# 10258392511/InverseProblemWithDiffusionModel

Measured on AMD Instinct MI355X. Metric: ALD reconstructions/sec (128x128 complex, R=40, 4-coil), higher is better.
Workload: dtype f32 (convolutions: operands as two fp16 pieces = 22 significand bits + 2 signs, three fp16 MFMAs per product, fp32 accumulate; every image scaled into fp16's range by an exact power of two from its producer's per-image maxima: any fp32 input, DESIGN.md 4.2); 1 GPU; ACDC-style 128x128 complex SENSE R=40 4-coil ALD reconstruction, NCSNv2Deepest ngf=128 (94.1M params, seeded random init), sigma 348->0.01 x 2311 levels x 3 steps, L2Penalty, denoise; 14 posterior samples = 14 on rank 0 + 13 per further rank (the 105-sample / 8-GPU partition of BASELINE config 3); samples_total=14, samples_this_rank=14, parallelism=sample-sharded x1, hip_graph=True, state_finite=True

## Files before the change

include/ipdm.h:

```cpp
#ifndef IPDM_H
#define IPDM_H

#include <stddef.h>
#include <stdint.h>

#ifdef __cplusplus
extern "C" {
#endif

#define IPDM_OK 0
#define IPDM_EINVAL (-1)
#define IPDM_EUNSUPPORTED (-2)

#define IPDM_ACT_NONE 0
#define IPDM_ACT_ELU 1
#define IPDM_ACT_RELU 2
#define IPDM_ACT_LRELU02 3
#define IPDM_ACT_SWISH 4
#define IPDM_ACT_COPY 5

#define IPDM_AMAX_WAYS 8
#define IPDM_AMAX_SLOT 128

#define IPDM_ABI_VERSION 4
// ... 106 lines not shown
                                   int32_t* iters_out, int B, int n_coils, int H, int W, void* stream);

int ipdm_sense_forward_sets_c64(const float* x, const float* sens, int sens_complex, int sens_sets, const uint8_t* mask,
                                int mask_t, float* y, int B, int n_coils, int H, int W, void* stream);
int ipdm_sense_adjoint_sets_c64(const float* s, const float* sens, int sens_complex, int sens_sets, const uint8_t* mask,
                                int mask_t, int apply_mask, float* x, float* workspace, int B, int n_coils, int H, int W,
                                void* stream);
int ipdm_sense_l2prox_sets_f32(const float* z_re, const float* z_im, const float* y, const float* sens, int sens_complex,
                               int sens_sets, const uint8_t* mask, int mask_t, float coef, float* out_re, float* out_im,
                               float* work, int B, int n_coils, int H, int W, void* stream);
int ipdm_ald_sense_step_sets_f32(float* x_re, float* x_im, const float* g_re, const float* g_im,
                                 const float* noise_re, const float* noise_im,
                                 float step, float noise_scale, uint64_t seed, int64_t sample_offset, int64_t step_id,
                                 const ipdm_sched_t* dev_sched, const float* y, const float* sens, int sens_complex,
                                 int sens_sets, const uint8_t* mask, int mask_t, float coef, float* work, int B, int n_coils,
                                 int H, int W, void* stream);
int ipdm_sense_cgprox_sets_f32(const float* z_re, const float* z_im, const float* y, const float* sens, int sens_complex,
                               int sens_sets, const uint8_t* mask, int mask_t, float a, const float* ahy, int max_iter,
                               float tol, float* out_re, float* out_im, float* work, int32_t* iters_out, int B, int n_coils,
                               int H, int W, void* stream);
int ipdm_ald_sense_cg_step_sets_f32(float* x_re, float* x_im, const float* g_re, const float* g_im,
                                    const float* noise_re, const float* noise_im,
                                    float step, float noise_scale, uint64_t seed, int64_t sample_offset, int64_t step_id,
                                    const ipdm_sched_t* dev_sched, const float* y, const float* sens, int sens_complex,
                                    int sens_sets, const uint8_t* mask, int mask_t, float coef, float* work,
                                    const float* ahy, int max_iter, float tol, int32_t* iters_out, int B, int n_coils,
                                    int H, int W, void* stream);

size_t ipdm_csm_workspace_bytes(int B, int n_coils, int H, int W);
int ipdm_csm_supported(int n_coils, int radius, int H, int W);
int ipdm_csm_calib_images_c64(const float* y, int ah, int aw, float* calib, int B, int n_coils, int H, int W, void* stream);
int ipdm_csm_walsh_c64(const float* y, int ah, int aw, int radius, int power_iters, float thresh,
                       float* maps , float* rss ,
                       float* rss_max , float* work , int B,
                       int n_coils, int H, int W, void* stream);

int ipdm_coilcomp_supported(int n_coils, int n_virtual);
size_t ipdm_coilcomp_workspace_bytes(int B, int n_coils);
int ipdm_coil_gram_c64(const float* y, int ah, int aw, float* gram, int B, int n_coils, int H, int W, void* stream);
int ipdm_coilcomp_matrix_c64(const float* gram, const float* noise_cov, int n_virtual, float* A, float* eig, int32_t* status,
                             int B, int n_coils, void* stream);
int ipdm_coil_apply_c64(const float* y, const float* A, int per_image, float* out, int B, int n_coils, int n_virtual,
                        int64_t P, void* stream);
int ipdm_coil_compress_c64(const float* y, int ah, int aw, int n_virtual, const float* noise_cov, float* A, float* eig,
                           int32_t* status, float* out, float* work, int B, int n_coils, int H, int W, void* stream);

int ipdm_gcc_supported(int n_coils, int n_virtual, int H, int W, int win);
size_t ipdm_gcc_workspace_bytes(int B, int n_coils, int n_virtual, int H, int W);
int ipdm_readout_fft_c64(const float* in, float* out, int inverse, int64_t planes, int H, int W, void* stream);
int ipdm_gcc_gram_c64(const float* h, int aw, int win, float* gram, int B, int n_coils, int H, int W, void* stream);
int ipdm_gcc_align_c64(const float* Ahat, const float* noise_cov, float* A, int32_t* status, int32_t* work, int B, int H,
                       int n_coils, int n_virtual, void* stream);
int ipdm_coil_apply_rows_c64(const float* y, const float* A, int per_image, float* out, int B, int n_coils, int n_virtual, int H,
                             int W, void* stream);
int ipdm_gcc_compress_c64(const float* y, int aw, int win, int n_virtual, const float* noise_cov, float* A, float* eig,
                          int32_t* status, float* out, float* work, int B, int n_coils, int H, int W, void* stream);

int ipdm_espirit_supported(int n_coils, int ksize, int H, int W);
size_t ipdm_espirit_workspace_bytes(int B, int n_coils, int ksize);
int ipdm_espirit_gram_c64(const float* y, int ah, int aw, int ksize, double* gram, int B, int n_coils, int H, int W, void* stream);
int ipdm_espirit_kernels_c64(const float* y, int ah, int aw, int ksize, double sv_thresh, float* K, double* lam, int32_t* rank,
                             int32_t* status, int32_t* sweeps, double* work, int B, int n_coils, int H, int W, void* stream);
int ipdm_espirit_pixel_c64(const float* K, const int32_t* status, int ksize, float crop, int power_iters, float* maps,
                           float* eigval, int B, int n_coils, int H, int W, void* stream);
int ipdm_espirit_c64(const float* y, int ah, int aw, int ksize, double sv_thresh, float crop, int power_iters, float* maps,
                     float* eigval, float* K, double* lam, int32_t* rank, int32_t* status, double* work, int B, int n_coils,
                     int H, int W, void* stream);

int ipdm_kspace_tavg_c64(const float* y, const uint8_t* mask, int mask_t, float* ybar, int32_t* count, int B, int T,
                         int n_coils, int H, int W, void* stream);

int ipdm_singlecoil_prox_f32(const float* z_re, const float* z_im, const float* y, const uint8_t* mask, int mask_t,
                             float coef, int mode, float* out_re, float* out_im,
                             float* workspace ,
                             int B, int H, int W, void* stream);

int ipdm_ald_singlecoil_step_f32(float* x_re, float* x_im, const float* g_re, const float* g_im,
                                 const float* noise_re, const float* noise_im,
                                 float step, float noise_scale, uint64_t seed, int64_t sample_offset, int64_t step_id,
                                 const ipdm_sched_t* dev_sched, const float* y, const uint8_t* mask, int mask_t,
                                 float coef, int mode, float* workspace , int B, int H,
                                 int W, void* stream);

int64_t ipdm_pc_langevin_coef_workspace_bytes(int B);
int ipdm_pc_langevin_coef_f32(const float* g_re, const float* g_im, const float* noise_re, const float* noise_im,
                              double snr, double alpha, uint64_t seed, int64_t sample_offset, int64_t step_id,
                              const ipdm_sched_t* dev_sched, float coef, float sigma, ipdm_sched_t* sample_sched,
                              double* work, int B, int64_t sample_elems, void* stream);
int ipdm_pc_sense_step_f32(float* x_re, float* x_im, const float* g_re, const float* g_im,
                           const float* noise_re, const float* noise_im,
                           float step, float noise_scale, uint64_t seed, int64_t sample_offset, int64_t step_id,
                           const ipdm_sched_t* dev_sched, int sched_stride, const float* y, const float* sens,
                           int sens_complex, int sens_sets, const uint8_t* mask, int mask_t, float coef, float* work, int B,
                           int n_coils, int H, int W, void* stream);
int ipdm_pc_sense_cg_step_f32(float* x_re, float* x_im, const float* g_re, const float* g_im,
                              const float* noise_re, const float* noise_im,
                              float step, float noise_scale, uint64_t seed, int64_t sample_offset, int64_t step_id,
                              const ipdm_sched_t* dev_sched, int sched_stride, const float* y, const float* sens,
                              int sens_complex, int sens_sets, const uint8_t* mask, int mask_t, float coef, float* work,
                              const float* ahy, int max_iter, float tol, int32_t* iters_out, int B, int n_coils, int H,
                              int W, void* stream);
int ipdm_pc_singlecoil_step_f32(float* x_re, float* x_im, const float* g_re, const float* g_im,
                                const float* noise_re, const float* noise_im,
                                float step, float noise_scale, uint64_t seed, int64_t sample_offset, int64_t step_id,
                                const ipdm_sched_t* dev_sched, int sched_stride, const float* y, const uint8_t* mask,
                                int mask_t, float coef, int mode, float* workspace, int B, int H, int W, void* stream);

int ipdm_nc_supported(int H, int W);
int64_t ipdm_ndft_workspace_bytes(int M, int H, int W);
int ipdm_ndft_forward_c64(const float* x, const float* sens, const double* traj, float* y,
                          float* work , int B, int n_coils, int M, int H, int W, void* stream);
int ipdm_ndft_adjoint_c64(const float* y, const float* sens, const double* traj, const float* weights, float* x,
                          float* work , int B, int n_coils, int M, int H, int W, void* stream);
int64_t ipdm_toeplitz_psf_workspace_bytes(int M, int H, int W);
int ipdm_toeplitz_psf_f32(const double* traj, const float* weights, float* psf,
                          float* work , int M, int H, int W, void* stream);
int64_t ipdm_toeplitz_workspace_bytes(int B, int n_coils, int H, int W);
int ipdm_toeplitz_normal_c64(const float* v, const float* sens, const float* psf, float* out,
                             float* work , int B, int n_coils, int H, int W, void* stream);
int64_t ipdm_nc_sense_cg_workspace_bytes(int B, int n_coils, int H, int W);
int ipdm_nc_sense_cgprox_f32(const float* z_re, const float* z_im, const float* sens, const float* psf, float a,
                             const float* ahy, int max_iter, float tol, float* out_re, float* out_im, float* work,
                             int32_t* iters_out, int B, int n_coils, int H, int W, void* stream);
int ipdm_ald_nc_sense_cg_step_f32(float* x_re, float* x_im, const float* g_re, const float* g_im,
                                  const float* noise_re, const float* noise_im,
                                  float step, float noise_scale, uint64_t seed, int64_t sample_offset, int64_t step_id,
                                  const ipdm_sched_t* dev_sched, int sched_stride, const float* sens, const float* psf,
                                  float coef, float* work, const float* ahy, int max_iter, float tol, int32_t* iters_out,
                                  int B, int n_coils, int H, int W, void* stream);
int ipdm_ndft_forward_sets_c64(const float* x, const float* sens, const double* traj, int traj_sets, float* y, float* work,
                               int B, int n_coils, int M, int H, int W, void* stream);
int ipdm_ndft_adjoint_sets_c64(const float* y, const float* sens, const double* traj, int traj_sets, const float* weights,
                               float* x, float* work, int B, int n_coils, int M, int H, int W, void* stream);
int ipdm_toeplitz_psf_sets_f32(const double* traj, int traj_sets, const float* weights, float* psf, float* work, int M, int H,
                               int W, void* stream);
int ipdm_toeplitz_normal_sets_c64(const float* v, const float* sens, const float* psf, int psf_sets, float* out, float* work,
                                  int B, int n_coils, int H, int W, void* stream);
int ipdm_nc_sense_cgprox_sets_f32(const float* z_re, const float* z_im, const float* sens, const float* psf, int psf_sets,
                                  float a, const float* ahy, int max_iter, float tol, float* out_re, float* out_im,
                                  float* work, int32_t* iters_out, int B, int n_coils, int H, int W, void* stream);
int ipdm_ald_nc_sense_cg_step_sets_f32(float* x_re, float* x_im, const float* g_re, const float* g_im,
                                       const float* noise_re, const float* noise_im,
                                       float step, float noise_scale, uint64_t seed, int64_t sample_offset, int64_t step_id,
                                       const ipdm_sched_t* dev_sched, int sched_stride, const float* sens, const float* psf,
                                       int psf_sets, float coef, float* work, const float* ahy, int max_iter, float tol,
                                       int32_t* iters_out, int B, int n_coils, int H, int W, void* stream);

size_t ipdm_nc_coil_gram_workspace_bytes(int B, int n_coils, int M);
int ipdm_nc_coil_gram_c64(const float* y, const float* weights, float* gram, float* work, int B, int n_coils, int M, void* stream);

int ipdm_langevin_step_f32(float* x, const float* g, const float* noise, float step, float noise_scale,
                           uint64_t seed, int64_t sample_offset, int64_t step_id, const ipdm_sched_t* dev_sched,
                           int64_t n_samples, int64_t sample_elems, void* stream);

int ipdm_philox_normal_f32(float* out, uint64_t seed, int64_t sample_offset, int64_t step_id, int plane,
                           int64_t n_samples, int64_t sample_elems, void* stream);

int ipdm_philox_block_host(uint64_t seed, int64_t sample, int64_t step_id, int plane, uint32_t quad, uint32_t* out4);


int ipdm_instnorm_plus_coef_f32(const float* x, const float* alpha, const float* gamma, const float* beta,
                                float* coef, int B, int C, int HW,
                                float* amax_bound ,
                                void* stream);
int ipdm_cond_instnorm_plus_coef_f32(const float* x, const float* embed, const int64_t* labels, int num_classes, int bias,
                                     float* coef, int B, int C, int HW, float* amax_bound, void* stream);
int ipdm_affine_act_f32(const float* x, const float* coef, float* y, int B, int C, int HW, int act, void* stream);
int ipdm_act_f32(const float* x, float* y, int64_t n, int act, void* stream);
int ipdm_scale_shift_f32(const float* x, float* y, int64_t n, float a, float b, void* stream);
int ipdm_add_f32(const float* x, const float* y, float* out, int64_t n, void* stream);
int ipdm_div_sigma_f32(const float* x, const float* sigmas, const int64_t* labels, float* out,
                       int B, int64_t sample_elems, void* stream);
int ipdm_conv3x3_thin_supported(int Cin, int Cout, int H, int W);
int ipdm_conv3x3_thin_f32(const float* x, const float* w, const float* bias,
                          const float* coef ,
                          float* out, int B, int Cin, int Cout, int H, int W, void* stream);
int ipdm_conv3x3_thin_stats_partials(int Cin, int Cout, int H, int W);
int ipdm_conv3x3_thin_stats_f32(const float* x, const float* w, const float* bias, const float* coef, float* out, float* part,
                                int B, int Cin, int Cout, int H, int W, void* stream);
int ipdm_conv3x3_fewout_fin_supported(int Cin, int Cout, int H, int W);
int ipdm_conv3x3_fewout_fin_f32(const float* x, const float* w, const float* bias, const float* coef, int act, float* out,
                                int B, int Cin, int Cout, int H, int W, void* stream);
int ipdm_maxpool5_f32(const float* x, float* y, int planes, int H, int W, void* stream);
int ipdm_affine_avgpool5_f32(const float* x, const float* coef, float* y, int planes, int H, int W, void* stream);
int ipdm_meanpool2_f32(const float* x, float* y, int planes, int H, int W, void* stream);
int ipdm_bilinear_f32(const float* x, float* out, int planes, int in_h, int in_w, int out_h, int out_w,
                      int accumulate, int act ,
                      int planes_per_image, float* amax_out ,
                      void* stream);
int ipdm_trilinear_f32(const float* x, float* out, int planes, int in_d, int in_h, int in_w, int out_d, int out_h,
                       int out_w, int accumulate, int act, int planes_per_image, float* amax_out, void* stream);

int ipdm_groupnorm_coef_f32(const float* x, const float* weight, const float* bias, float* coef,
                            int B, int C, int HW, int G, float eps,
                            float* plane_amax ,
                            void* stream);
int ipdm_groupnorm_coef_partials_f32(const float* part1, int C1, const float* part2, int C2, int P, const float* weight,
                                     const float* bias, float* coef , int B, int G, float eps, void* stream);
int ipdm_groupnorm_coef_cat_f32(const float* x1, int C1, const float* x2, int C2, const float* weight, const float* bias,
                                float* coef, int B, int HW, int G, float eps, float* plane_amax ,
                                void* stream);
int ipdm_affine_act_cat_f32(const float* x1, int C1, const float* x2, int C2, const float* coef, float* y, int B, int HW,
                            int act, void* stream);
int ipdm_linear_f32(const float* x, const float* W, const float* bias, float* y, int B, int In, int Out,
                    int act, void* stream);
int ipdm_attention_f32(const float* q, const float* k, const float* v, float* out, int B, int C, int N,
                       float scale, void* stream);
int ipdm_axpby_f32(const float* x, const float* y, float* out, int64_t n, float a, float b, void* stream);
int ipdm_sample_axpy2_f32(const float* x, const float* y, const float* z, const float* a, const float* c,
                          float* out, int n_samples, int64_t sample_elems, void* stream);
int ipdm_sample_norm_f32(const float* x, float* norms, int n_samples, int64_t sample_elems, void* stream);

int ipdm_conv_pack_weight_f32(const float* w , float* wt, int Cout, int Cin, int k, void* stream);
int ipdm_conv2d_f32(const float* x, const float* wt, const float* bias, const float* coef, int act,
                    const float* residual, float* out, float* out_act, int act_out,
                    int B, int Cin, int Cout, int H, int W, int k, int dilation, int pool2, void* stream);

int ipdm_conv_wino_weight_f32(const float* w , float* U, int Cout, int Cin, void* stream);
int ipdm_conv2d_wino_supported(int Cin, int Cout, int H, int W, int dilation);
int ipdm_conv2d_wino_f32(const float* x, const float* U, const float* bias, const float* residual, float* out,
                         float* out_act, int act_out, int B, int Cin, int Cout, int H, int W, int dilation,
                         void* stream);

int ipdm_debug_set_stamp_buffer(void* buf);
int64_t ipdm_debug_lds_optin_count(void);

int ipdm_conv3d_f32(const float* x, const float* wt, const float* bias, const float* coef, int act,
                    const float* residual, float* out, float* out_act, int act_out,
                    int B, int Cin, int Cout, int D, int H, int W, int k, int dilation, void* stream);

int ipdm_maxpool3d5_f32(const float* x, float* y, int planes, int D, int H, int W, void* stream);
int ipdm_temporal_taps_f32(const float* x, float* out, int planes, int S, int T_in, int T_out, int mode, void* stream);

typedef struct {
  const float* in_amax;
  int bias_bstride;
  float out_scale;
  int res_second;
  float* out_amax;
  float* act_amax;
} ipdm_conv_ext_t;

int64_t ipdm_conv_bx3_weight_bytes(int Cout, int Cin, int k);
int ipdm_conv_bx3_pack_weight(const float* w , void* packed, int Cout,
                              int Cin, int k, void* stream);
int ipdm_conv2d_bx3_f32(const float* x, const void* packed, const float* bias, const float* coef, int act,
                        const float* residual, float* out, float* out_act, int act_out,
                        int B, int Cin, int Cout, int H, int W, int k, int dilation, const ipdm_conv_ext_t* ext, void* stream);
int ipdm_conv3d_bx3_f32(const float* x, const void* packed, const float* bias, const float* coef, int act,
                        const float* residual, float* out, float* out_act, int act_out,
                        int B, int Cin, int Cout, int D, int H, int W, int k, int dilation, const ipdm_conv_ext_t* ext, void* stream);

int ipdm_conv_bx3_splitk(int B, int D, int Cin, int Cout, int H, int W, int k, int dilation);
int ipdm_conv_bx3_splitk_f32(const float* x, const void* packed, const float* bias, const float* coef, int act,
                             const float* residual, float* out, float* out_act, int act_out,
                             int B, int Cin, int Cout, int D, int H, int W, int k, int dilation, int volume, int ksplit,
                             float* work, const ipdm_conv_ext_t* ext, void* stream);

int ipdm_adam_ascent_f32(float* x, const float* g, float* m, float* v, int64_t n, float lr, float beta1, float beta2,
                         float eps, int step, void* stream);

int64_t ipdm_conv_wino_bx3_weight_bytes(int Cout, int Cin);
int ipdm_conv_wino_bx3_pack_weight(const float* w , void* U, int Cout, int Cin, void* stream);
int ipdm_conv2d_wino_bx3_supported(int Cin, int Cout, int H, int W, int dilation);
int ipdm_conv2d_wino_bx3_f32(const float* x, const void* U, const float* bias, const float* residual, float* out,
                             float* out_act, int act_out, int B, int Cin, int Cout, int H, int W, int dilation,
                             int pool2, const ipdm_conv_ext_t* ext, void* stream);
int ipdm_conv2d_wino_bx3_splitk(int Cin, int Cout, int H, int W, int dilation);
int ipdm_conv2d_wino_bx3_splitk_f32(const float* x, const void* U, const float* bias, const float* residual, float* out,
                                    float* out_act, int act_out, int B, int Cin, int Cout, int H, int W, int dilation,
                                    int ksplit, float* work, const ipdm_conv_ext_t* ext, void* stream);
int ipdm_conv2d_wino_bx3_stats_partials(int Cin, int Cout, int H, int W, int dilation, int pool2);
int ipdm_conv2d_wino_bx3_stats_f32(const float* x, const void* U, const float* bias, const float* residual, float* out,
                                   float* out_act, int act_out, int B, int Cin, int Cout, int H, int W, int dilation,
                                   int pool2, float* stats, const ipdm_conv_ext_t* ext, void* stream);
int ipdm_absmax_f32(const float* x, float* amax , int n_images,
                    int64_t per_image, void* stream);
int64_t ipdm_conv_hx2_weight_bytes(int Cout, int Cin, int k);
int ipdm_conv_hx2_pack_weight(const float* w , void* packed, int Cout,
                              int Cin, int k, void* stream);
int ipdm_conv2d_hx2_f32(const float* x, const void* packed, const float* bias, const float* coef, int act,
                        const float* residual, float* out, float* out_act, int act_out,
                        int B, int Cin, int Cout, int H, int W, int k, int dilation, const ipdm_conv_ext_t* ext, void* stream);
int ipdm_conv3d_hx2_f32(const float* x, const void* packed, const float* bias, const float* coef, int act,
                        const float* residual, float* out, float* out_act, int act_out,
                        int B, int Cin, int Cout, int D, int H, int W, int k, int dilation, const ipdm_conv_ext_t* ext, void* stream);
int ipdm_conv_hx2_splitk_f32(const float* x, const void* packed, const float* bias, const float* coef, int act,
                             const float* residual, float* out, float* out_act, int act_out,
                             int B, int Cin, int Cout, int D, int H, int W, int k, int dilation, int volume, int ksplit,
                             float* work, const ipdm_conv_ext_t* ext, void* stream);
int64_t ipdm_conv_wino_hx2_weight_bytes(int Cout, int Cin);
int ipdm_conv_wino_hx2_pack_weight(const float* w , void* U, int Cout, int Cin, void* stream);
int ipdm_conv2d_wino_hx2_f32(const float* x, const void* U, const float* bias, const float* residual, float* out,
                             float* out_act, int act_out, int B, int Cin, int Cout, int H, int W, int dilation,
                             int pool2, const ipdm_conv_ext_t* ext, void* stream);
#define IPDM_WINO_FORM_OTHER 0
#define IPDM_WINO_FORM_CO32 1
#define IPDM_WINO_FORM_HALF 2
#define IPDM_WINO_FORM_POLY 3
int ipdm_conv2d_wino_hx2_form(int Cin, int Cout, int H, int W, int dilation);
int64_t ipdm_conv_wino1d_weight_bytes(int Cout, int Cin);
int ipdm_conv_wino1d_pack_weight(const float* w , void* U, int Cout, int Cin, void* stream);
int ipdm_conv2d_wino1d_supported(int Cin, int Cout, int H, int W);
int64_t ipdm_conv_wino1d_weight_bytes3d(int Cout, int Cin);
int ipdm_conv_wino1d_pack_weight3d(const float* w, void* U, int Cout, int Cin, void* stream);
int ipdm_conv3d_wino1d_supported(int Cin, int Cout, int D, int H, int W);
int ipdm_conv3d_wino1d_f32(const float* x, const void* U, const float* bias, const float* residual, float* out,
                           float* out_act, int act_out, int B, int Cin, int Cout, int D, int H, int W,
                           const ipdm_conv_ext_t* ext, void* stream);
int ipdm_conv2d_wino1d_f32(const float* x, const void* U, const float* bias, const float* coef, int act,
                           const float* residual, float* out, float* out_act, int act_out, int B, int Cin, int Cout, int H,
                           int W, int pool2, const ipdm_conv_ext_t* ext, void* stream);
int ipdm_conv2d_wino1d_stats_partials(int Cin, int Cout, int H, int W);
int ipdm_conv2d_wino1d_stats_f32(const float* x, const void* U, const float* bias, const float* coef, int act,
                                 const float* residual, float* out, float* out_act, int act_out, int B, int Cin, int Cout,
                                 int H, int W, int pool2, float* stats, const ipdm_conv_ext_t* ext, void* stream);
int ipdm_conv2d_wino_hx2_splitk_f32(const float* x, const void* U, const float* bias, const float* residual, float* out,
                                    float* out_act, int act_out, int B, int Cin, int Cout, int H, int W, int dilation,
                                    int ksplit, float* work, const ipdm_conv_ext_t* ext, void* stream);
int ipdm_conv2d_wino_hx2_stats_f32(const float* x, const void* U, const float* bias, const float* residual, float* out,
                                   float* out_act, int act_out, int B, int Cin, int Cout, int H, int W, int dilation,
                                   int pool2, float* stats, const ipdm_conv_ext_t* ext, void* stream);
int ipdm_instnorm_plus_coef_partials_f32(const float* partials, int P, const float* alpha, const float* gamma,
                                         const float* beta , float* coef , int B, int C,
                                         int HW , float* amax_bound ,
                                         void* stream);

int ipdm_cond_instnorm_plus_coef_partials_f32(const float* partials, int P, const float* embed, const int64_t* labels,
                                              int num_classes, int bias, float* coef, int B, int C, int HW, float* amax_bound,
                                              void* stream);

int ipdm_conv1d_hx2_supported(int Cin, int Cout, int L, int k, int dilation);
int64_t ipdm_conv1d_hx2_weight_bytes(int Cout, int Cin, int k);
int ipdm_conv1d_hx2_pack_weight(const float* w , void* packed, int Cout, int Cin, int k, void* stream);
int ipdm_conv1d_hx2_f32(const float* x, const void* packed, const float* bias, const float* residual, float* out,
                        float* out_act, int act_out, int N, int Cin, int Cout, int L, int k, int dilation, int pool2,
                        const ipdm_conv_ext_t* ext, void* stream);
int ipdm_meanpool1d2_f32(const float* x, float* y, int rows, int L, void* stream);
int ipdm_scale_shift_amax_f32(const float* x, float* y, float* amax_out, int n_images, int64_t per_image, float a, float b,
                              void* stream);


int ipdm_zero_insert2_f32(const float* x, float* out, int planes, int H, int W, void* stream);
int ipdm_subsample2_f32(const float* x, float* out, int planes, int H, int W, int oy, int ox, int Ho, int Wo, void* stream);
int ipdm_in_prelu_fwd_f32(const float* x, const float* slope, float* xhat, float* y, float* rstd, int planes, int HW,
                          float eps, void* stream);
int ipdm_in_prelu_bwd_f32(const float* gy, const float* xhat, const float* rstd, const float* slope, float* gx, int planes,
                          int HW, void* stream);
int ipdm_in_prelu_bwd_eps_f32(const float* gy, const float* xhat, const float* rstd, const float* slope, float* gx, int planes,
                              int HW, float eps, void* stream);
int ipdm_seg_loglh_grad_f32(const float* logits, const int64_t* label, float* g, int B, int C, int64_t HW, void* stream);
int ipdm_axpy_sched_f32(float* y, const float* x, const int64_t* mask, int64_t mask_period, const ipdm_sched_t* dev_sched,
                        float scale, int64_t n, void* stream);


int ipdm_magnitude_c64(const float* x , float* out, int64_t n, void* stream);
int ipdm_posterior_moments_c64(const float* samples, double* planes, int n_samples, int64_t HW, void* stream);
int ipdm_nrmse_f32(const float* img, const float* ref, double* out, int n_images, int64_t elems, int ref_broadcast,
                   void* stream);
int ipdm_ssim_f32(const float* img, const float* ref, double* out, int n_images, int H, int W, int ref_broadcast,
                  double data_range, void* stream);

int ipdm_tv_c64(const float* x, double* out, int n_images, int H, int W, void* stream);
int ipdm_tv_grad_c64(const float* x, float* g, int n_images, int H, int W, void* stream);

#ifdef __cplusplus
}
#endif
#endif
```

inverseproblemwithdiffusionmodel_amd/_lib.py:

```python
import ctypes
import os

import torch
from ctypes import c_char_p, c_double, c_float, c_int, c_int64, c_uint64, c_void_p


class ConvExt(ctypes.Structure):
    _fields_ = [("in_amax", c_void_p), ("bias_bstride", c_int), ("out_scale", c_float), ("res_second", c_int),
                ("out_amax", c_void_p), ("act_amax", c_void_p)]


_HERE = os.path.dirname(os.path.abspath(__file__))
LIB_PATH = os.environ.get("IPDM_LIB") or os.path.join(_HERE, "libipdm.so")

P = c_void_p

SIGNATURES = {
    "ipdm_abi_version": [],
    "ipdm_build_arch": [],
    "ipdm_upfirdn2d_f32": [P, P, P] + [c_int] * 14 + [P],
    "ipdm_fused_bias_act_f32": [P, P, P, P, c_int64, c_int, c_int, c_int, c_int, c_float, c_float, P],
    "ipdm_upfirdn2d_f16": [P, P, P] + [c_int] * 14 + [P],
    "ipdm_upfirdn2d_f64": [P, P, P] + [c_int] * 14 + [P],
    "ipdm_fused_bias_act_f16": [P, P, P, P, c_int64, c_int, c_int, c_int, c_int, c_float, c_float, P],
    "ipdm_fused_bias_act_f64": [P, P, P, P, c_int64, c_int, c_int, c_int, c_int, c_float, c_float, P],
    "ipdm_fft2c_c64": [P, P, c_int, c_int, c_int, c_int, P, P],
    "ipdm_fft2c_workspace_bytes": [c_int, c_int, c_int],
    "ipdm_mask_layouts": [],
    "ipdm_kspace_size_class": [c_int, c_int],
    "ipdm_sense_forward_c64": [P, P, P, c_int, P, c_int, c_int, c_int, c_int, P],
    "ipdm_sense_workspace_bytes": [c_int, c_int, c_int, c_int],
    "ipdm_sense_adjoint_c64": [P, P, P, c_int, c_int, P, P, c_int, c_int, c_int, c_int, P],
    "ipdm_sense_ssos_c64": [P, P, P, c_int, c_int, c_int, c_int, P],
    "ipdm_sense_l2prox_f32": [P, P, P, P, P, c_int, c_float, P, P, P, c_int, c_int, c_int, c_int, P],
    "ipdm_ald_sense_step_f32": [P, P, P, P, P, P, c_float, c_float, c_uint64, c_int64, c_int64, P,
                                P, P, P, c_int, c_float, P, c_int, c_int, c_int, c_int, P],
    "ipdm_sense_forward_csm_c64": [P, P, P, c_int, P, c_int, c_int, c_int, c_int, P],
    "ipdm_sense_adjoint_csm_c64": [P, P, P, c_int, c_int, P, P, c_int, c_int, c_int, c_int, P],
    "ipdm_sense_l2prox_csm_f32": [P, P, P, P, P, c_int, c_float, P, P, P, c_int, c_int, c_int, c_int, P],
    "ipdm_ald_sense_step_csm_f32": [P, P, P, P, P, P, c_float, c_float, c_uint64, c_int64, c_int64, P,
                                    P, P, P, c_int, c_float, P, c_int, c_int, c_int, c_int, P],
    "ipdm_sense_cg_workspace_bytes": [c_int, c_int, c_int, c_int],
    "ipdm_sense_cgprox_f32": [P, P, P, P, P, c_int, c_float, P, c_int, c_float, P, P, P, P, c_int, c_int, c_int, c_int, P],
    "ipdm_sense_cgprox_csm_f32": [P, P, P, P, P, c_int, c_float, P, c_int, c_float, P, P, P, P, c_int, c_int, c_int, c_int, P],
    "ipdm_ald_sense_cg_step_f32": [P, P, P, P, P, P, c_float, c_float, c_uint64, c_int64, c_int64, P,
                                   P, P, P, c_int, c_float, P, P, c_int, c_float, P, c_int, c_int, c_int, c_int, P],
    "ipdm_ald_sense_cg_step_csm_f32": [P, P, P, P, P, P, c_float, c_float, c_uint64, c_int64, c_int64, P,
                                       P, P, P, c_int, c_float, P, P, c_int, c_float, P, c_int, c_int, c_int, c_int, P],
    "ipdm_sense_forward_sets_c64": [P, P, c_int, c_int, P, c_int, P, c_int, c_int, c_int, c_int, P],
    "ipdm_sense_adjoint_sets_c64": [P, P, c_int, c_int, P, c_int, c_int, P, P, c_int, c_int, c_int, c_int, P],
    "ipdm_sense_l2prox_sets_f32": [P, P, P, P, c_int, c_int, P, c_int, c_float, P, P, P, c_int, c_int, c_int, c_int, P],
    "ipdm_ald_sense_step_sets_f32": [P, P, P, P, P, P, c_float, c_float, c_uint64, c_int64, c_int64, P,
                                     P, P, c_int, c_int, P, c_int, c_float, P, c_int, c_int, c_int, c_int, P],
    "ipdm_sense_cgprox_sets_f32": [P, P, P, P, c_int, c_int, P, c_int, c_float, P, c_int, c_float, P, P, P, P,
                                   c_int, c_int, c_int, c_int, P],
    "ipdm_ald_sense_cg_step_sets_f32": [P, P, P, P, P, P, c_float, c_float, c_uint64, c_int64, c_int64, P,
                                        P, P, c_int, c_int, P, c_int, c_float, P, P, c_int, c_float, P,
                                        c_int, c_int, c_int, c_int, P],
    "ipdm_csm_workspace_bytes": [c_int, c_int, c_int, c_int],
    "ipdm_csm_supported": [c_int, c_int, c_int, c_int],
    "ipdm_csm_calib_images_c64": [P, c_int, c_int, P, c_int, c_int, c_int, c_int, P],
    "ipdm_csm_walsh_c64": [P, c_int, c_int, c_int, c_int, c_float, P, P, P, P, c_int, c_int, c_int, c_int, P],
    "ipdm_coilcomp_supported": [c_int, c_int],
    "ipdm_coilcomp_workspace_bytes": [c_int, c_int],
    "ipdm_coil_gram_c64": [P, c_int, c_int, P, c_int, c_int, c_int, c_int, P],
    "ipdm_coilcomp_matrix_c64": [P, P, c_int, P, P, P, c_int, c_int, P],
    "ipdm_coil_apply_c64": [P, P, c_int, P, c_int, c_int, c_int, c_int64, P],
    "ipdm_coil_compress_c64": [P, c_int, c_int, c_int, P, P, P, P, P, P, c_int, c_int, c_int, c_int, P],
    "ipdm_gcc_supported": [c_int, c_int, c_int, c_int, c_int],
    "ipdm_gcc_workspace_bytes": [c_int, c_int, c_int, c_int, c_int],
    "ipdm_readout_fft_c64": [P, P, c_int, c_int64, c_int, c_int, P],
    "ipdm_gcc_gram_c64": [P, c_int, c_int, P, c_int, c_int, c_int, c_int, P],
    "ipdm_gcc_align_c64": [P, P, P, P, P, c_int, c_int, c_int, c_int, P],
    "ipdm_coil_apply_rows_c64": [P, P, c_int, P, c_int, c_int, c_int, c_int, c_int, P],
    "ipdm_gcc_compress_c64": [P, c_int, c_int, c_int, P, P, P, P, P, P, c_int, c_int, c_int, c_int, P],
    "ipdm_espirit_supported": [c_int, c_int, c_int, c_int],
    "ipdm_espirit_workspace_bytes": [c_int, c_int, c_int],
    "ipdm_espirit_gram_c64": [P, c_int, c_int, c_int, P, c_int, c_int, c_int, c_int, P],
    "ipdm_espirit_kernels_c64": [P, c_int, c_int, c_int, c_double, P, P, P, P, P, P, c_int, c_int, c_int, c_int, P],
    "ipdm_espirit_pixel_c64": [P, P, c_int, c_float, c_int, P, P, c_int, c_int, c_int, c_int, P],
    "ipdm_espirit_c64": [P, c_int, c_int, c_int, c_double, c_float, c_int, P, P, P, P, P, P, P, c_int, c_int, c_int, c_int, P],
    "ipdm_kspace_tavg_c64": [P, P, c_int, P, P, c_int, c_int, c_int, c_int, c_int, P],
    "ipdm_singlecoil_prox_f32": [P, P, P, P, c_int, c_float, c_int, P, P, P, c_int, c_int, c_int, P],
    "ipdm_ald_singlecoil_step_f32": [P, P, P, P, P, P, c_float, c_float, c_uint64, c_int64, c_int64, P,
                                     P, P, c_int, c_float, c_int, P, c_int, c_int, c_int, P],
    "ipdm_pc_langevin_coef_workspace_bytes": [c_int],
    "ipdm_pc_langevin_coef_f32": [P, P, P, P, c_double, c_double, c_uint64, c_int64, c_int64, P, c_float, c_float, P, P,
                                  c_int, c_int64, P],
    "ipdm_pc_sense_step_f32": [P, P, P, P, P, P, c_float, c_float, c_uint64, c_int64, c_int64, P, c_int,
                               P, P, c_int, c_int, P, c_int, c_float, P, c_int, c_int, c_int, c_int, P],
    "ipdm_pc_sense_cg_step_f32": [P, P, P, P, P, P, c_float, c_float, c_uint64, c_int64, c_int64, P, c_int,
                                  P, P, c_int, c_int, P, c_int, c_float, P, P, c_int, c_float, P,
                                  c_int, c_int, c_int, c_int, P],
    "ipdm_pc_singlecoil_step_f32": [P, P, P, P, P, P, c_float, c_float, c_uint64, c_int64, c_int64, P, c_int,
                                    P, P, c_int, c_float, c_int, P, c_int, c_int, c_int, P],
    "ipdm_nc_supported": [c_int, c_int],
    "ipdm_ndft_workspace_bytes": [c_int, c_int, c_int],
    "ipdm_ndft_forward_c64": [P, P, P, P, P, c_int, c_int, c_int, c_int, c_int, P],
    "ipdm_ndft_adjoint_c64": [P, P, P, P, P, P, c_int, c_int, c_int, c_int, c_int, P],
    "ipdm_toeplitz_psf_workspace_bytes": [c_int, c_int, c_int],
    "ipdm_toeplitz_psf_f32": [P, P, P, P, c_int, c_int, c_int, P],
    "ipdm_toeplitz_workspace_bytes": [c_int, c_int, c_int, c_int],
    "ipdm_toeplitz_normal_c64": [P, P, P, P, P, c_int, c_int, c_int, c_int, P],
    "ipdm_nc_sense_cg_workspace_bytes": [c_int, c_int, c_int, c_int],
    "ipdm_nc_sense_cgprox_f32": [P, P, P, P, c_float, P, c_int, c_float, P, P, P, P, c_int, c_int, c_int, c_int, P],
    "ipdm_ald_nc_sense_cg_step_f32": [P, P, P, P, P, P, c_float, c_float, c_uint64, c_int64, c_int64, P, c_int,
                                      P, P, c_float, P, P, c_int, c_float, P, c_int, c_int, c_int, c_int, P],
    "ipdm_ndft_forward_sets_c64": [P, P, P, c_int, P, P, c_int, c_int, c_int, c_int, c_int, P],
    "ipdm_ndft_adjoint_sets_c64": [P, P, P, c_int, P, P, P, c_int, c_int, c_int, c_int, c_int, P],
    "ipdm_toeplitz_psf_sets_f32": [P, c_int, P, P, P, c_int, c_int, c_int, P],
    "ipdm_toeplitz_normal_sets_c64": [P, P, P, c_int, P, P, c_int, c_int, c_int, c_int, P],
    "ipdm_nc_sense_cgprox_sets_f32": [P, P, P, P, c_int, c_float, P, c_int, c_float, P, P, P, P, c_int, c_int, c_int, c_int, P],
    "ipdm_ald_nc_sense_cg_step_sets_f32": [P, P, P, P, P, P, c_float, c_float, c_uint64, c_int64, c_int64, P, c_int,
                                           P, P, c_int, c_float, P, P, c_int, c_float, P, c_int, c_int, c_int, c_int, P],
    "ipdm_nc_coil_gram_workspace_bytes": [c_int, c_int, c_int],
    "ipdm_nc_coil_gram_c64": [P, P, P, P, c_int, c_int, c_int, P],
    "ipdm_langevin_step_f32": [P, P, P, c_float, c_float, c_uint64, c_int64, c_int64, P, c_int64, c_int64, P],
    "ipdm_philox_normal_f32": [P, c_uint64, c_int64, c_int64, c_int, c_int64, c_int64, P],
    "ipdm_philox_block_host": [c_uint64, c_int64, c_int64, c_int, ctypes.c_uint32, P],
    "ipdm_instnorm_plus_coef_f32": [P, P, P, P, P, c_int, c_int, c_int, P, P],
    "ipdm_cond_instnorm_plus_coef_f32": [P, P, P, c_int, c_int, P, c_int, c_int, c_int, P, P],
    "ipdm_affine_act_f32": [P, P, P, c_int, c_int, c_int, c_int, P],
    "ipdm_act_f32": [P, P, c_int64, c_int, P],
    "ipdm_scale_shift_f32": [P, P, c_int64, c_float, c_float, P],
    "ipdm_add_f32": [P, P, P, c_int64, P],
    "ipdm_div_sigma_f32": [P, P, P, P, c_int, c_int64, P],
    "ipdm_maxpool5_f32": [P, P, c_int, c_int, c_int, P],
    "ipdm_affine_avgpool5_f32": [P, P, P, c_int, c_int, c_int, P],
    "ipdm_meanpool2_f32": [P, P, c_int, c_int, c_int, P],
    "ipdm_bilinear_f32": [P, P, c_int, c_int, c_int, c_int, c_int, c_int, c_int, c_int, P, P],
    "ipdm_conv3x3_thin_supported": [c_int, c_int, c_int, c_int],
    "ipdm_conv3x3_thin_f32": [P, P, P, P, P, c_int, c_int, c_int, c_int, c_int, P],
    "ipdm_conv3x3_thin_stats_partials": [c_int, c_int, c_int, c_int],
    "ipdm_conv3x3_thin_stats_f32": [P, P, P, P, P, P, c_int, c_int, c_int, c_int, c_int, P],
    "ipdm_conv3x3_fewout_fin_supported": [c_int, c_int, c_int, c_int],
    "ipdm_conv3x3_fewout_fin_f32": [P, P, P, P, c_int, P, c_int, c_int, c_int, c_int, c_int, P],
    "ipdm_trilinear_f32": [P, P, c_int, c_int, c_int, c_int, c_int, c_int, c_int, c_int, c_int, c_int, P, P],
    "ipdm_groupnorm_coef_f32": [P, P, P, P, c_int, c_int, c_int, c_int, c_float, P, P],
    "ipdm_groupnorm_coef_partials_f32": [P, c_int, P, c_int, c_int, P, P, P, c_int, c_int, c_float, P],
    "ipdm_groupnorm_coef_cat_f32": [P, c_int, P, c_int, P, P, P, c_int, c_int, c_int, c_float, P, P],
    "ipdm_affine_act_cat_f32": [P, c_int, P, c_int, P, P, c_int, c_int, c_int, P],
    "ipdm_linear_f32": [P, P, P, P, c_int, c_int, c_int, c_int, P],
    "ipdm_attention_f32": [P, P, P, P, c_int, c_int, c_int, c_float, P],
    "ipdm_axpby_f32": [P, P, P, c_int64, c_float, c_float, P],
    "ipdm_sample_axpy2_f32": [P, P, P, P, P, P, c_int, c_int64, P],
    "ipdm_sample_norm_f32": [P, P, c_int, c_int64, P],
    "ipdm_conv_pack_weight_f32": [P, P, c_int, c_int, c_int, P],
    "ipdm_conv2d_f32": [P, P, P, P, c_int, P, P, P, c_int] + [c_int] * 8 + [P],
    "ipdm_conv_wino_weight_f32": [P, P, c_int, c_int, P],
    "ipdm_conv2d_wino_supported": [c_int, c_int, c_int, c_int, c_int],
    "ipdm_conv2d_wino_f32": [P, P, P, P, P, P, c_int, c_int, c_int, c_int, c_int, c_int, c_int, P],
    "ipdm_debug_set_stamp_buffer": [P],
    "ipdm_debug_lds_optin_count": [],
    "ipdm_conv3d_f32": [P, P, P, P, c_int, P, P, P, c_int] + [c_int] * 8 + [P],
    "ipdm_maxpool3d5_f32": [P, P, c_int, c_int, c_int, c_int, P],
    "ipdm_temporal_taps_f32": [P, P, c_int, c_int, c_int, c_int, c_int, P],
    "ipdm_conv_bx3_weight_bytes": [c_int, c_int, c_int],
    "ipdm_conv_bx3_pack_weight": [P, P, c_int, c_int, c_int, P],
    "ipdm_conv2d_bx3_f32": [P, P, P, P, c_int, P, P, P, c_int] + [c_int] * 7 + [P, P],
    "ipdm_conv3d_bx3_f32": [P, P, P, P, c_int, P, P, P, c_int] + [c_int] * 8 + [P, P],
    "ipdm_conv_bx3_splitk": [c_int] * 8,
    "ipdm_conv_bx3_splitk_f32": [P, P, P, P, c_int, P, P, P, c_int] + [c_int] * 10 + [P, P, P],
    "ipdm_adam_ascent_f32": [P, P, P, P, c_int64, c_float, c_float, c_float, c_float, c_int, P],
    "ipdm_conv_wino_bx3_weight_bytes": [c_int, c_int],
    "ipdm_conv_wino_bx3_pack_weight": [P, P, c_int, c_int, P],
    "ipdm_conv2d_wino_bx3_supported": [c_int, c_int, c_int, c_int, c_int],
    "ipdm_conv2d_wino_bx3_f32": [P, P, P, P, P, P, c_int, c_int, c_int, c_int, c_int, c_int, c_int, c_int, P, P],
    "ipdm_conv2d_wino_bx3_stats_partials": [c_int, c_int, c_int, c_int, c_int, c_int],
    "ipdm_conv2d_wino_bx3_splitk": [c_int, c_int, c_int, c_int, c_int],
    "ipdm_conv2d_wino_bx3_splitk_f32": [P, P, P, P, P, P, c_int, c_int, c_int, c_int, c_int, c_int, c_int, c_int, P, P, P],
    "ipdm_conv2d_wino_bx3_stats_f32": [P, P, P, P, P, P, c_int, c_int, c_int, c_int, c_int, c_int, c_int, c_int, P, P, P],
    "ipdm_conv_hx2_weight_bytes": [c_int, c_int, c_int],
    "ipdm_conv_hx2_pack_weight": [P, P, c_int, c_int, c_int, P],
    "ipdm_absmax_f32": [P, P, c_int, c_int64, P],
    "ipdm_conv2d_hx2_f32": [P, P, P, P, c_int, P, P, P, c_int] + [c_int] * 7 + [P, P],
    "ipdm_conv3d_hx2_f32": [P, P, P, P, c_int, P, P, P, c_int] + [c_int] * 8 + [P, P],
    "ipdm_conv_hx2_splitk_f32": [P, P, P, P, c_int, P, P, P, c_int] + [c_int] * 10 + [P, P, P],
    "ipdm_conv_wino_hx2_weight_bytes": [c_int, c_int],
    "ipdm_conv_wino1d_weight_bytes": [c_int, c_int],
    "ipdm_conv_wino1d_pack_weight": [P, P, c_int, c_int, P],
    "ipdm_conv2d_wino1d_supported": [c_int, c_int, c_int, c_int],
    "ipdm_conv_wino1d_weight_bytes3d": [c_int, c_int],
    "ipdm_conv_wino1d_pack_weight3d": [P, P, c_int, c_int, P],
    "ipdm_conv3d_wino1d_supported": [c_int, c_int, c_int, c_int, c_int],
    "ipdm_conv3d_wino1d_f32": [P, P, P, P, P, P, c_int, c_int, c_int, c_int, c_int, c_int, c_int, P, P],
    "ipdm_conv2d_wino1d_f32": [P, P, P, P, c_int, P, P, P, c_int, c_int, c_int, c_int, c_int, c_int, c_int, P, P],
    "ipdm_conv2d_wino1d_stats_partials": [c_int, c_int, c_int, c_int],
    "ipdm_conv2d_wino1d_stats_f32": [P, P, P, P, c_int, P, P, P, c_int, c_int, c_int, c_int, c_int, c_int, c_int, P, P, P],
    "ipdm_conv_wino_hx2_pack_weight": [P, P, c_int, c_int, P],
    "ipdm_conv2d_wino_hx2_f32": [P, P, P, P, P, P, c_int, c_int, c_int, c_int, c_int, c_int, c_int, c_int, P, P],
    "ipdm_conv2d_wino_hx2_form": [c_int] * 5,
    "ipdm_conv2d_wino_hx2_splitk_f32": [P, P, P, P, P, P, c_int, c_int, c_int, c_int, c_int, c_int, c_int, c_int, P, P, P],
    "ipdm_conv2d_wino_hx2_stats_f32": [P, P, P, P, P, P, c_int, c_int, c_int, c_int, c_int, c_int, c_int, c_int, P, P, P],
    "ipdm_instnorm_plus_coef_partials_f32": [P, c_int, P, P, P, P, c_int, c_int, c_int, P, P],
    "ipdm_cond_instnorm_plus_coef_partials_f32": [P, c_int, P, P, c_int, c_int, P, c_int, c_int, c_int, P, P],
    "ipdm_conv1d_hx2_supported": [c_int] * 5,
    "ipdm_conv1d_hx2_weight_bytes": [c_int, c_int, c_int],
    "ipdm_conv1d_hx2_pack_weight": [P, P, c_int, c_int, c_int, P],
    "ipdm_conv1d_hx2_f32": [P, P, P, P, P, P, c_int] + [c_int] * 7 + [P, P],
    "ipdm_meanpool1d2_f32": [P, P, c_int, c_int, P],
    "ipdm_scale_shift_amax_f32": [P, P, P, c_int, c_int64, c_float, c_float, P],
    "ipdm_zero_insert2_f32": [P, P, c_int, c_int, c_int, P],
    "ipdm_subsample2_f32": [P, P, c_int, c_int, c_int, c_int, c_int, c_int, c_int, P],
    "ipdm_in_prelu_fwd_f32": [P, P, P, P, P, c_int, c_int, c_float, P],
    "ipdm_in_prelu_bwd_f32": [P, P, P, P, P, c_int, c_int, P],
    "ipdm_in_prelu_bwd_eps_f32": [P, P, P, P, P, c_int, c_int, c_float, P],
    "ipdm_seg_loglh_grad_f32": [P, P, P, c_int, c_int, c_int64, P],
    "ipdm_axpy_sched_f32": [P, P, P, c_int64, P, c_float, c_int64, P],
    "ipdm_magnitude_c64": [P, P, c_int64, P],
    "ipdm_posterior_moments_c64": [P, P, c_int, c_int64, P],
    "ipdm_tv_c64": [P, P, c_int, c_int, c_int, P],
    "ipdm_tv_grad_c64": [P, P, c_int, c_int, c_int, P],
    "ipdm_nrmse_f32": [P, P, P, c_int, c_int64, c_int, P],
    "ipdm_ssim_f32": [P, P, P, c_int, c_int, c_int, c_int, ctypes.c_double, P],
}
_RESTYPES = {"ipdm_build_arch": c_char_p, "ipdm_debug_lds_optin_count": c_int64, "ipdm_fft2c_workspace_bytes": c_int64, "ipdm_sense_workspace_bytes": c_int64, "ipdm_sense_cg_workspace_bytes": c_int64,
             "ipdm_pc_langevin_coef_workspace_bytes": c_int64,
             "ipdm_ndft_workspace_bytes": c_int64, "ipdm_toeplitz_psf_workspace_bytes": c_int64,
             "ipdm_toeplitz_workspace_bytes": c_int64, "ipdm_nc_sense_cg_workspace_bytes": c_int64,
             "ipdm_conv_bx3_weight_bytes": c_int64,
             "ipdm_conv_wino_bx3_weight_bytes": c_int64, "ipdm_conv_hx2_weight_bytes": c_int64,
             "ipdm_conv_wino_hx2_weight_bytes": c_int64, "ipdm_conv_wino1d_weight_bytes": c_int64, "ipdm_conv_wino1d_weight_bytes3d": c_int64,
             "ipdm_conv1d_hx2_weight_bytes": c_int64, "ipdm_csm_workspace_bytes": ctypes.c_size_t,
             "ipdm_coilcomp_workspace_bytes": ctypes.c_size_t, "ipdm_gcc_workspace_bytes": ctypes.c_size_t,
             "ipdm_espirit_workspace_bytes": ctypes.c_size_t, "ipdm_nc_coil_gram_workspace_bytes": ctypes.c_size_t}

IPDM_EINVAL = -1
IPDM_EUNSUPPORTED = -2


class IpdmError(RuntimeError):
    pass


class IpdmUnsupported(IpdmError, NotImplementedError):
    pass


def _load():
    if not os.path.exists(LIB_PATH):
        raise ImportError(
            f"{LIB_PATH} is missing: the HIP kernels are not built. Run `python -c 'import __graft_entry__ as g; "
            "g.build()'` (or inverseproblemwithdiffusionmodel_amd/csrc/build.py). There is no CPU fallback.")
    lib = ctypes.CDLL(LIB_PATH)
    for name, argtypes in SIGNATURES.items():
        fn = getattr(lib, name)
        fn.argtypes = argtypes
        fn.restype = _RESTYPES.get(name, c_int)
    return lib


lib = _load()


def check(rc, what):
    if rc == 0:
        return
    if rc == IPDM_EUNSUPPORTED:
        raise IpdmUnsupported(f"{what}: no gfx950 kernel for this size/combination (IPDM_EUNSUPPORTED)")
    if rc == IPDM_EINVAL:
        raise IpdmError(f"{what}: invalid argument (IPDM_EINVAL)")
    raise IpdmError(f"{what}: HIP error {rc}")


def call(name, *args):
    check(getattr(lib, name)(*args), name)
```

inverseproblemwithdiffusionmodel_amd/csrc/conv_wino1d.hip:

```cpp
#include "conv_kernel.h"

namespace ipdm_conv {

namespace {

constexpr int Y_KC = 16;
constexpr int Y_CO = 128;
constexpr int Y_ROWS = 8, Y_TX = 16;
constexpr int Y_VROWS = 12;
constexpr int Y_RS = 1040;
constexpr int Y_STAGE = Y_VROWS * Y_RS;
constexpr int Y_RAW = 8 * 1024;
constexpr int Y_M = 4 * 64 * 32;
constexpr int Y_S1 = Y_STAGE + Y_RAW;
constexpr size_t Y_LDS_BYTES = ((size_t)Y_S1 + 2 * Y_M + 2 * Y_CO) * 4;
static_assert(Y_STAGE <= 2 * Y_M && Y_LDS_BYTES <= 160 * 1024, "LDS budget");
constexpr float HX1_PRESCALE = 0.5f;
constexpr int Y_QC = 10, Y_RC4 = 40, Y_QN = 100;

__device__ __forceinline__ float wino1d_U(const float* g, int p) {
  g += (p / 12) * 9;
  p %= 12;
  const float G[4][3] = {{1.f, 0.f, 0.f}, {0.5f, 0.5f, 0.5f}, {0.5f, -0.5f, 0.5f}, {0.f, 0.f, 1.f}};
  const int ky = p >> 2, xi = p & 3;
  return G[xi][0] * g[ky * 3 + 0] + G[xi][1] * g[ky * 3 + 1] + G[xi][2] * g[ky * 3 + 2];
}

__global__ __launch_bounds__(256) void wino1d_scale_kernel(const float* __restrict__ w, float* __restrict__ inv_scale, int Cout,
                                                           int Cin, int n_co_pad, int npos) {
  __shared__ float red[256];
  const int co = blockIdx.x;
  float m = 0.f;
  if (co < Cout)
    for (int i = threadIdx.x; i < Cin * npos; i += 256)
      m = fmaxf(m, fabsf(wino1d_U(w + ((size_t)co * Cin + i / npos) * (npos / 12 * 9), i % npos)));
  red[threadIdx.x] = m;
  __syncthreads();
  for (int st = 128; st > 0; st >>= 1) {
    if ((int)threadIdx.x < st) red[threadIdx.x] = fmaxf(red[threadIdx.x], red[threadIdx.x + st]);
    __syncthreads();
  }
  if (threadIdx.x == 0 && co < n_co_pad) {
    int e = 0;
    const float mx = red[0];
    if (mx > 0.f && mx < INFINITY) (void)frexpf(mx, &e);
    inv_scale[co] = (mx > 0.f && mx < INFINITY ? ldexpf(1.f, e - 14) : 1.f) / HX1_PRESCALE;
  }
}

__global__ __launch_bounds__(256) void wino1d_weight_kernel(const float* __restrict__ w, unsigned short* __restrict__ out,
                                                            const float* __restrict__ inv_scale, int Cout, int Cin, int n_cc,
                                                            int n_ct, int npos) {
  const int64_t total = (int64_t)npos * n_cc * n_ct * 512;
  for (int64_t i = (int64_t)blockIdx.x * 256 + threadIdx.x; i < total; i += (int64_t)gridDim.x * 256) {
    const int q = (int)(i & 7), r = (int)((i >> 3) & 31), h = (int)((i >> 8) & 1);
    const int64_t rest = i >> 9;
    const int ct = (int)(rest % n_ct);
    const int cc = (int)((rest / n_ct) % n_cc);
    const int p = (int)(rest / ((int64_t)n_ct * n_cc));
    const int co = ct * 32 + r, ci = cc * 16 + 8 * h + q;
    float v = 0.f;
    if (co < Cout && ci < Cin) v = wino1d_U(w + ((size_t)co * Cin + ci) * (npos / 12 * 9), p) * (1.f / (inv_scale[co] * HX1_PRESCALE));
    const _Float16 hi = (_Float16)v;
    const _Float16 lo = (_Float16)(v - (float)hi);
    const int64_t base = rest * 2 * 512 + h * 256 + r * 8 + q;
    out[base] = __builtin_bit_cast(unsigned short, hi);
    out[base + 512] = __builtin_bit_cast(unsigned short, lo);
  }
}

template <int OUTS, bool STATS = false, bool POOL = false, bool FIN = false, bool VOL = false, int NBU = 4>
__global__ __launch_bounds__(512) void conv_wino1d_kernel(ConvArgs a, int total_tiles) {
  extern __shared__ __align__(16) float lds[];
  unsigned* const ldsw = reinterpret_cast<unsigned*>(lds);
  const int tid = threadIdx.x;
  const int lane = tid & 63;
  const int wave = __builtin_amdgcn_readfirstlane(tid >> 6);
  const int h = lane >> 5, j = lane & 31;
  const int xi = wave & 3, chh = wave >> 2;
  const int HW = a.H * a.W;
  const int n_cc = a.Cin / Y_KC, n_ct = a.Cout / 32;
  static_assert(!VOL || (!STATS && !POOL && !FIN), "VOL: plain epilogues");
  static_assert(NBU == 4 || (NBU == 3 && VOL), "compact columns: the volume form");
  const int n_chunks = VOL ? 3 * n_cc : n_cc;
  const int CS = VOL ? a.D * HW : HW;
  const bool pack = VOL && a.W <= 12;
  const int seam = a.W >> 1;
  unsigned long long t0 = 0, t1 = 0, t_loop = 0, t_epi = 0, tq = 0;
#ifdef IPDM_W1D_TRACE
  unsigned long long te[4] = {0, 0, 0, 0};
#endif
  if (a.dbg) t0 = __builtin_amdgcn_s_memtime();

  const int S = gridDim.x / 8;
  const int xcd = blockIdx.x % 8, slot = blockIdx.x / 8;
  const int q8 = total_tiles / 8, r8 = total_tiles % 8;
  const int x_start = xcd < r8 ? xcd * (q8 + 1) : r8 * (q8 + 1) + (xcd - r8) * q8;
  const int t_end = x_start + q8 + (xcd < r8 ? 1 : 0);
  int tile = x_start + slot;
  if (tile >= t_end) return;
  if (a.phase_step > 0) {
    const int g = slot & a.phase_mask;
    for (int i = 0; i < g * a.phase_step; ++i) __builtin_amdgcn_s_sleep(8);
  }

  struct Geo { int b, y0, x0, cob, z; };
  auto geo_of = [&](int L) {
    Geo g;
    g.cob = L % a.co_tiles;
    int t = L / a.co_tiles;
    const int tx = t % a.tiles_x;
    t /= a.tiles_x;
    g.y0 = (t % a.tiles_y) * Y_ROWS;
    g.x0 = tx * (2 * Y_TX);
    t /= a.tiles_y;
    g.z = 0;
    if constexpr (VOL) {
      const int nz = pack ? (a.D + 1) >> 1 : a.D;
      g.z = (t % nz) * (pack ? 2 : 1);
      t /= nz;
    }
    g.b = t;
    return g;
  };

  const __amdgpu_buffer_rsrc_t x_rsrc = __builtin_amdgcn_make_buffer_rsrc(
      const_cast<float*>(a.x), 0, (int)((size_t)a.B * a.Cin * CS * 4), 0x00020000);
  float* const rs = lds + Y_STAGE;

  int dma_off[4];
  int dma_b = 0;
  [[maybe_unused]] int dma_z = 0, dma_isb = 0;
  auto set_dma_geo = [&](const Geo& g) {
    dma_b = g.b;
    if constexpr (VOL) {
      dma_z = g.z;
      dma_isb = 0;
    }
#pragma unroll
    for (int k = 0; k < 4; ++k) {
      const int e = k * 64 + lane;
      const int cl = e / Y_QN, qq = e - cl * Y_QN;
      const int cin = 2 * wave + cl;
      const int rr = qq / Y_QC, qc = qq - rr * Y_QC;
      const int gy = g.y0 - 1 + rr;
      int gx0 = g.x0 - 4 + 4 * qc;
      bool okx = gx0 >= 0 && gx0 < a.W;
      if constexpr (VOL) {
        if (pack) {
          const bool in_b = gx0 >= a.W && gx0 < 2 * a.W;
          okx = okx || in_b;
          gx0 -= in_b ? a.W : 0;
          dma_isb |= in_b ? 1 << k : 0;
        }
      }
      const bool ok = e < 2 * Y_QN && gy >= 0 && gy < a.H && okx;
      dma_off[k] = ok ? (cin * CS + gy * a.W + gx0) * 4 : 0x40000000;
    }
  };
  auto issue_dma = [&](int chunk) {
    int cc = chunk;
    [[maybe_unused]] int off_a = 0, off_b = 0;
    [[maybe_unused]] bool ok_a = true, ok_b = false;
    if constexpr (VOL) {
      const int kz = chunk / n_cc;
      cc = chunk - kz * n_cc;
      const int za = dma_z + kz - 1, zb = za + 1;
      ok_a = (unsigned)za < (unsigned)a.D;
      ok_b = pack && (unsigned)zb < (unsigned)a.D && dma_z + 1 < a.D;
      off_a = za * HW * 4;
      off_b = zb * HW * 4;
    }
    [[maybe_unused]] const int soff = (int)(((size_t)dma_b * a.Cin + cc * Y_KC) * CS * 4);
#pragma unroll
    for (int k = 0; k < 4; ++k) {
      int off = dma_off[k];
      if constexpr (VOL) {
        const bool isb = (dma_isb >> k) & 1;
        const bool ok = off != 0x40000000 && (isb ? ok_b : ok_a);
        off = ok ? off + (isb ? off_b : off_a) : 0x40000000;
      }
#if defined(__HIP_DEVICE_COMPILE__)
      __builtin_amdgcn_raw_ptr_buffer_load_lds(x_rsrc, (__attribute__((address_space(3))) void*)(rs + (wave * 4 + k) * 256), 16,
                                               off, soff, 0, 0);
#endif
    }
  };

  const int pt = lane & 15, rsub = lane >> 4;
  const bool pfirst = pt == 0, plast = pt == Y_TX - 1;
  struct Raw { float2 qa, qb; float ea, eb; };
  Raw raw[3];
  auto read_items = [&]() {
    const float* rp = rs + wave * 1024 + rsub * Y_RC4 + 2 * pt + 2;
    const int edge = pfirst ? 1 : 4;
#pragma unroll
    for (int it = 0; it < 3; ++it) {
      raw[it].qa = *reinterpret_cast<const float2*>(rp + it * 4 * Y_RC4 + 2);
      raw[it].ea = rp[it * 4 * Y_RC4 + edge];
      raw[it].qb = *reinterpret_cast<const float2*>(rp + Y_QN * 4 + it * 4 * Y_RC4 + 2);
      raw[it].eb = rp[Y_QN * 4 + it * 4 * Y_RC4 + edge];
    }
  };
  [[maybe_unused]] float hx_in = HX1_PRESCALE, hx_out = 1.f;
  auto hx_scales_of = [&](int b, float& s_in, float& s_out) {
    s_in = HX1_PRESCALE;
    s_out = 1.f;
    if (a.in_amax) {
      float sd, si;
      hx_dynamic_scale(ipdm_amax_read(a.in_amax + (size_t)b * IPDM_AMAX_SLOT), sd, si);
      s_in = HX1_PRESCALE * sd;
      s_out = si;
    }
  };
  const int v_st = ((wave & 3) >> 1) * 64 + (wave >> 2) * 32 + (wave & 1) * 16 + pt;
  [[maybe_unused]] float fin_mu[2] = {0.f, 0.f}, fin_sc[2] = {1.f, 1.f}, fin_sh[2] = {0.f, 0.f};
  [[maybe_unused]] int fin_row = 0;
  [[maybe_unused]] bool fin_pair = true, fin_edge = true;
  [[maybe_unused]] auto set_fin = [&](int b, int chunk, int y0, int x0) {
    if constexpr (FIN) {
      const float* cf = a.coef + ((size_t)b * a.Cin + chunk * Y_KC + 2 * wave) * 3;
#pragma unroll
      for (int cl = 0; cl < 2; ++cl) {
        fin_mu[cl] = cf[cl * 3];
        fin_sc[cl] = cf[cl * 3 + 1];
        fin_sh[cl] = cf[cl * 3 + 2];
      }
      fin_row = y0 - 1 + rsub;
      fin_pair = x0 + 2 * pt < a.W;
      fin_edge = pfirst ? x0 > 0 : x0 + 2 * Y_TX < a.W;
    }
  };
  auto xform_item = [&](auto itc, float (&va)[4], float (&vb)[4]) {
    constexpr int it = decltype(itc)::value;
    Raw r = raw[it];
    if constexpr (FIN) {
      const bool rok = (unsigned)(fin_row + 4 * it) < (unsigned)a.H;
      const bool pok = rok && fin_pair, eok = rok && fin_edge;
      auto fin = [&](float v, int cl, bool ok) {
        const float t = fast_elu((v - fin_mu[cl]) * fin_sc[cl] + fin_sh[cl]);
        return ok ? t : 0.f;
      };
      r.qa.x = fin(r.qa.x, 0, pok); r.qa.y = fin(r.qa.y, 0, pok); r.ea = fin(r.ea, 0, eok);
      r.qb.x = fin(r.qb.x, 1, pok); r.qb.y = fin(r.qb.y, 1, pok); r.eb = fin(r.eb, 1, eok);
    }
    const float la = __builtin_bit_cast(float, __builtin_amdgcn_mov_dpp(__builtin_bit_cast(int, r.qa.y), 0x111, 0xf, 0xf, true));
    const float ra = __builtin_bit_cast(float, __builtin_amdgcn_mov_dpp(__builtin_bit_cast(int, r.qa.x), 0x101, 0xf, 0xf, true));
    const float lb = __builtin_bit_cast(float, __builtin_amdgcn_mov_dpp(__builtin_bit_cast(int, r.qb.y), 0x111, 0xf, 0xf, true));
    const float rb = __builtin_bit_cast(float, __builtin_amdgcn_mov_dpp(__builtin_bit_cast(int, r.qb.x), 0x101, 0xf, 0xf, true));
    float a0 = pfirst ? r.ea : la, a3 = plast ? r.ea : ra;
    float b0 = pfirst ? r.eb : lb, b3 = plast ? r.eb : rb;
    if constexpr (VOL) {
      if (pack) {
        const bool s_l = pt == seam, s_r = pt == seam - 1;
        a0 = s_l ? 0.f : a0; b0 = s_l ? 0.f : b0;
        a3 = s_r ? 0.f : a3; b3 = s_r ? 0.f : b3;
      }
    }
    va[0] = a0 - r.qa.y; va[1] = r.qa.x + r.qa.y; va[2] = r.qa.y - r.qa.x; va[3] = r.qa.x - a3;
    vb[0] = b0 - r.qb.y; vb[1] = r.qb.x + r.qb.y; vb[2] = r.qb.y - r.qb.x; vb[3] = r.qb.x - b3;
  };
  auto store_item = [&](unsigned* st, auto itc, const float (&va)[4], const float (&vb)[4], auto lo_c, auto hi_c) {
    constexpr int it = decltype(itc)::value;
    unsigned* vs = st + (it * 4 + rsub) * Y_RS + v_st;
#pragma unroll
    for (int x = decltype(lo_c)::value; x < decltype(hi_c)::value; ++x) {
      unsigned hp, lp;
      split2_pk_scaled(va[x], vb[x], hx_in, hp, lp);
      vs[(x * 2 + 0) * 128] = hp;
      vs[(x * 2 + 1) * 128] = lp;
    }
  };

  const uint4* wq = reinterpret_cast<const uint4*>(a.wt);
  const size_t pos_stride = (size_t)n_cc * n_ct * 128;
  auto load_A = [&](uint4 (&fr)[2][2], int ky, int chunk, int cob) {
    int cc = chunk, kz = 0;
    if constexpr (VOL) {
      kz = chunk / n_cc;
      cc = chunk - kz * n_cc;
    }
    const uint4* base = wq + (size_t)((kz * 3 + ky) * 4 + xi) * pos_stride + ((size_t)cc * n_ct + cob * 4 + chh * 2) * 128 + lane;
#pragma unroll
    for (int c = 0; c < 2; ++c)
#pragma unroll
      for (int s = 0; s < 2; ++s) fr[c][s] = base[c * 128 + s * 64];
  };
  const int b_lane = (j >> 4) * Y_RS + xi * 256 + h * 32 + (j & 15);
  [[maybe_unused]] int b_cmp[3] = {0, 0, 0};
  if constexpr (NBU == 3) {
#pragma unroll
    for (int nb = 0; nb < 3; ++nb) {
      const int n = 32 * nb + j;
      b_cmp[nb] = (n / 12) * Y_RS + xi * 256 + h * 32 + n % 12;
    }
  }
  auto load_B = [&](uint4 (&fr)[2], const unsigned* cur, auto kyc, auto nbc) {
    constexpr int ky = decltype(kyc)::value, nb = decltype(nbc)::value;
    const unsigned* bp = NBU == 3 ? cur + ky * Y_RS + b_cmp[nb < 3 ? nb : 0] : cur + (2 * nb + ky) * Y_RS + b_lane;
#pragma unroll
    for (int s = 0; s < 2; ++s) fr[s] = make_uint4(bp[s * 128], bp[s * 128 + 16], bp[s * 128 + 64], bp[s * 128 + 80]);
  };

  f32x16 acc[2][NBU];
#pragma unroll
  for (int i = 0; i < 2 * NBU; ++i)
#pragma unroll
    for (int rr = 0; rr < 16; ++rr) acc[i / NBU][i % NBU][rr] = 0.f;

  auto lds_barrier = [&]() {
    __builtin_amdgcn_sched_barrier(0);
    __builtin_amdgcn_s_waitcnt(0xC07F);
    __builtin_amdgcn_s_barrier();
    asm volatile("" ::: "memory");
    __builtin_amdgcn_sched_barrier(0);
  };

  Geo cur_g = geo_of(tile);
  uint4 afr[2][2][2];
  load_A(afr[0], 0, 0, cur_g.cob);
  load_A(afr[1], 1, 0, cur_g.cob);
  hx_scales_of(cur_g.b, hx_in, hx_out);
  set_dma_geo(cur_g);
  issue_dma(0);
  __builtin_amdgcn_s_waitcnt(0);
  set_fin(cur_g.b, 0, cur_g.y0, cur_g.x0);
  read_items();
  __builtin_amdgcn_sched_barrier(0);
  __builtin_amdgcn_s_waitcnt(0xC07F);
  issue_dma(1);
  __builtin_amdgcn_sched_barrier(0);
  static_for<3>([&](auto itc) {
    float va[4], vb[4];
    xform_item(itc, va, vb);
    store_item(ldsw, itc, va, vb, std::integral_constant<int, 0>{}, std::integral_constant<int, 4>{});
  });
  __builtin_amdgcn_s_waitcnt(0);
  __syncthreads();

  if (a.dbg) t1 = tq = __builtin_amdgcn_s_memtime();
  [[maybe_unused]] int pend_b = cur_g.b;
  [[maybe_unused]] unsigned pend_o = 0u, pend_a = 0u;
  auto flush_amax = [&]() {
    if (lane == 0) {
      if (a.amax_out) ipdm_amax_atomic(a.amax_out + (size_t)pend_b * IPDM_AMAX_SLOT, wave, __builtin_bit_cast(float, pend_o));
      if (a.amax_act) ipdm_amax_atomic(a.amax_act + (size_t)pend_b * IPDM_AMAX_SLOT, wave, __builtin_bit_cast(float, pend_a));
    }
  };

  while (true) {
    const int next_tile = tile + S;
    const bool has_next = next_tile < t_end;
    const Geo next_g = geo_of(has_next ? next_tile : tile);
    for (int ch2 = 0; ch2 < n_chunks; ch2 += 2) {
      static_for<2>([&](auto cpc) {
        constexpr int cpar = decltype(cpc)::value;
        const int ch = ch2 + cpar;
        const unsigned* cur = ldsw + cpar * Y_S1;
        unsigned* nxt = ldsw + (1 - cpar) * Y_S1;
        const bool dma_next = ch + 2 >= n_chunks;
        const int dma_chunk = dma_next ? ch + 2 - n_chunks : ch + 2;
        if (ch + 2 == n_chunks) set_dma_geo(next_g);
        const bool a_next = ch + 1 >= n_chunks;
        const int a_chunk = a_next ? 0 : ch + 1;
        const int a_cob = a_next ? next_g.cob : cur_g.cob;
        if (a_next && next_g.b != cur_g.b) {
          [[maybe_unused]] float unused_out;
          hx_scales_of(next_g.b, hx_in, unused_out);
        }
        if constexpr (FIN) {
          if (a_next) set_fin(next_g.b, 0, next_g.y0, next_g.x0);
          else set_fin(cur_g.b, ch + 1, cur_g.y0, cur_g.x0);
        }
        uint4 bsh[2][2];
        __builtin_amdgcn_s_waitcnt(0x0F78);
        read_items();
        load_B(bsh[0], cur, std::integral_constant<int, 0>{}, std::integral_constant<int, 0>{});
        __builtin_amdgcn_sched_barrier(0);
        __builtin_amdgcn_s_waitcnt(0xC07F);
        issue_dma(dma_chunk);
        __builtin_amdgcn_sched_barrier(0);
        float va[4], vb[4];
        static_for<3 * NBU>([&](auto ssc) {
          constexpr int ss = decltype(ssc)::value;
          constexpr int ky = ss / NBU, nb = ss % NBU;
          constexpr int aslot = (cpar * 3 + ky) & 1;
          if constexpr (ss < 3 * NBU - 1)
            load_B(bsh[(ss + 1) & 1], cur, std::integral_constant<int, (ss + 1) / NBU>{}, std::integral_constant<int, (ss + 1) % NBU>{});
          constexpr int it = ky;
          if constexpr (nb == 0) xform_item(std::integral_constant<int, it>{}, va, vb);
          if constexpr (nb == 1) store_item(nxt, std::integral_constant<int, it>{}, va, vb, std::integral_constant<int, 0>{}, std::integral_constant<int, 2>{});
          if constexpr (nb == 2) store_item(nxt, std::integral_constant<int, it>{}, va, vb, std::integral_constant<int, 2>{}, std::integral_constant<int, 4>{});
          const f16x8 bh = __builtin_bit_cast(f16x8, bsh[ss & 1][0]), bl = __builtin_bit_cast(f16x8, bsh[ss & 1][1]);
#pragma unroll
          for (int c = 0; c < 2; ++c) {
            f32x16 v = acc[c][nb];
            v = __builtin_amdgcn_mfma_f32_32x32x16_f16(__builtin_bit_cast(f16x8, afr[aslot][c][1]), bh, v, 0, 0, 0);
            v = __builtin_amdgcn_mfma_f32_32x32x16_f16(__builtin_bit_cast(f16x8, afr[aslot][c][0]), bl, v, 0, 0, 0);
            v = __builtin_amdgcn_mfma_f32_32x32x16_f16(__builtin_bit_cast(f16x8, afr[aslot][c][0]), bh, v, 0, 0, 0);
            acc[c][nb] = v;
          }
          if constexpr (nb == NBU - 1) {
            if constexpr (ky == 0) load_A(afr[aslot], 2, ch, cur_g.cob);
            if constexpr (ky == 1) load_A(afr[aslot], 0, a_chunk, a_cob);
            if constexpr (ky == 2) load_A(afr[aslot], 1, a_chunk, a_cob);
          }
          if constexpr (ss < 3 * NBU - 1) __builtin_amdgcn_sched_group_barrier(0x100, 8, 0);
#pragma unroll
          for (int i = 0; i < 6; ++i) {
            __builtin_amdgcn_sched_group_barrier(0x008, 1, 0);
            __builtin_amdgcn_sched_group_barrier(0x006, 4, 0);
            if constexpr (nb == 1 || nb == 2) __builtin_amdgcn_sched_group_barrier(0x200, 1, 0);
          }
          __builtin_amdgcn_sched_barrier(0);
        });
        lds_barrier();
      });
    }

    if (a.dbg) {
      const unsigned long long t = __builtin_amdgcn_s_memtime();
      t_loop += t - tq;
      tq = t;
    }
    constexpr bool W_OUT = (OUTS & 1) != 0, W_ACT = (OUTS & 2) != 0;
    float* const ms = lds + Y_S1;
    const int ecol = tid & 31, ecg = tid >> 5;
    const int co0 = cur_g.cob * Y_CO;
    const float* const scale_p = reinterpret_cast<const float*>(wq + (VOL ? 36 : 12) * pos_stride);
    const int oHW = POOL ? HW >> 2 : (VOL ? CS : HW), oW = POOL ? a.W >> 1 : a.W;
    const size_t tile_base = (((size_t)cur_g.b * a.Cout + co0) * oHW + (size_t)cur_g.z * HW + (size_t)(POOL ? cur_g.y0 >> 1 : cur_g.y0) * oW +
                              (POOL ? cur_g.x0 >> 1 : cur_g.x0)) * 4;
    const bool e_isb = pack && (ecol & 15) >= seam;
    const int e_pair = e_isb ? (ecol & 15) - seam : (ecol & 15);
    unsigned eoff4 = 4u * (unsigned)(ecg * oHW + (POOL ? (ecol & 15) : (ecol >> 4) * oW + 2 * e_pair + (e_isb ? HW : 0)));
    asm volatile("" : "+v"(eoff4));
    [[maybe_unused]] auto cmp_off = [&](int nb) -> unsigned {
      const int n = 32 * nb + ecol, row = n / 12, pr = n % 12;
      const bool isb = pack && pr >= 6;
      return 4u * (unsigned)(ecg * oHW + row * oW + 2 * (isb ? pr - 6 : pr) + (isb ? HW : 0));
    };
    auto boff = [&](int c, int nb, int k) -> unsigned {
      if constexpr (NBU == 3) return 4u * (unsigned)((((k >> 1) * 2 + c) * 32 + (k & 1) * 16) * oHW) + cmp_off(nb);
      return 4u * (unsigned)((((k >> 1) * 2 + c) * 32 + (k & 1) * 16) * oHW + (POOL ? nb : 2 * nb) * oW) + eoff4;
    };
    auto in_range = [&](int nb) {
      if constexpr (NBU == 3) return !(pack && (32 * nb + ecol) % 12 >= 6) || cur_g.z + 1 < a.D;
      const bool row_ok = cur_g.y0 + 2 * nb + (ecol >> 4) < a.H;
      if constexpr (VOL) {
        if (pack) return row_ok && (ecol & 15) < 2 * seam && (!e_isb || cur_g.z + 1 < a.D);
      }
      return row_ok && cur_g.x0 + 2 * (ecol & 15) < a.W;
    };
    const bool has_res = a.residual != nullptr, has_bias = a.bias != nullptr;
    const bool elu = a.act_out == IPDM_ACT_ELU;
    const float* const res_p = has_res ? a.residual : a.wt;
    const float* const bias_p = has_bias ? a.bias : a.wt;
    const char* const res_b = reinterpret_cast<const char*>(res_p) + (has_res ? tile_base : 0);
    [[maybe_unused]] char* const out_b = reinterpret_cast<char*>(a.out) + tile_base;
    [[maybe_unused]] char* const act_b = reinterpret_cast<char*>(a.out_act) + tile_base;
    constexpr int NV = POOL ? 1 : 2;
    typedef float vecv __attribute__((ext_vector_type(NV)));
    vecv resv[2][4];
    auto prefetch = [&](auto rc) {
      constexpr int rnd = decltype(rc)::value;
      constexpr int c = rnd / NBU, nb = rnd % NBU, bf = rnd & 1;
      const bool res_ok = has_res && in_range(nb) && (!POOL || (ecol >> 4) == 0);
#pragma unroll
      for (int k = 0; k < 4; ++k) {
        const unsigned ob = res_ok ? boff(c, nb, k) : 0u;
        resv[bf][k] = *reinterpret_cast<const vecv*>(res_b + ob);
      }
    };
    if (cur_g.b != pend_b) {
      flush_amax();
      pend_b = cur_g.b;
      pend_o = pend_a = 0u;
    }
    float* const es = lds + Y_S1 + 2 * Y_M;
    if (tid < Y_CO) {
      es[tid] = scale_p[co0 + tid] * hx_out;
      es[Y_CO + tid] = has_bias ? bias_p[cur_g.b * a.bias_bstride + co0 + tid] : 0.f;
    }
    prefetch(std::integral_constant<int, 0>{});
    float amx_o = 0.f, amx_a = 0.f;
    [[maybe_unused]] float st_k[4], st_s1[4], st_s2[4];
    [[maybe_unused]] int st_c0 = 0, st_c1 = 0;
#ifdef IPDM_W1D_TRACE
#define W1D_TE(k) if (a.dbg) { const unsigned long long t_ = __builtin_amdgcn_s_memtime(); te[k] += t_ - tl; tl = t_; }
    unsigned long long tl = a.dbg ? __builtin_amdgcn_s_memtime() : 0;
#else
#define W1D_TE(k)
#endif
    static_for<2 * NBU>([&](auto rc) {
      constexpr int rnd = decltype(rc)::value;
      constexpr int c = rnd / NBU, nb = rnd % NBU, bf = rnd & 1;
      float* const mw = ms + (rnd & 1) * Y_M;
#pragma unroll
      for (int rr = 0; rr < 16; ++rr) {
        const int col = (rr & 3) + 8 * (rr >> 2) + 4 * h;
        mw[(xi * 64 + chh * 32 + col) * 32 + j] = acc[c][nb][rr];
        acc[c][nb][rr] = 0.f;
      }
      W1D_TE(0);
      __syncthreads();
      W1D_TE(1);
      if constexpr (rnd < 2 * NBU - 1) prefetch(std::integral_constant<int, rnd + 1>{});
      const bool inr = in_range(nb) && (!POOL || (ecol >> 4) == 0);
#pragma unroll
      for (int half = 0; half < 2; ++half) {
        float m[2][4], sc[2], bi[2];
#pragma unroll
        for (int kk = 0; kk < 2; ++kk) {
          const int k = half * 2 + kk;
          const int cidx = ((k >> 1) * 2 + c) * 32 + (k & 1) * 16 + ecg;
          sc[kk] = es[cidx];
          bi[kk] = es[Y_CO + cidx];
#pragma unroll
          for (int x = 0; x < 4; ++x) m[kk][x] = mw[(x * 64 + k * 16 + ecg) * 32 + ecol];
        }
        vecv ov[2], ev[2];
#pragma unroll
        for (int kk = 0; kk < 2; ++kk) {
          const int k = half * 2 + kk;
          float yv[2];
          yv[0] = __builtin_fmaf(m[kk][0] + m[kk][1] + m[kk][2], sc[kk], bi[kk]);
          yv[1] = __builtin_fmaf(m[kk][1] - m[kk][2] - m[kk][3], sc[kk], bi[kk]);
          if constexpr (POOL) {
            const float p0 = __shfl_xor(yv[0], 16, 64), p1 = __shfl_xor(yv[1], 16, 64);
            yv[0] = (((yv[0] + p0) + yv[1]) + p1) * 0.25f;
          }
#pragma unroll
          for (int v = 0; v < NV; ++v) {
            float y = yv[v], rv = yv[v];
            y += has_res ? resv[bf][k][v] : 0.f;
            rv = a.res_second ? rv : y;
            y *= a.out_scale;
            rv *= a.out_scale;
            ov[kk][v] = rv;
            if constexpr (STATS) {
              if constexpr (nb == 0) {
                if (v == 0) {
                  const float k0 = __builtin_bit_cast(float, __builtin_amdgcn_readlane(__builtin_bit_cast(int, rv), 0));
                  const float k1 = __builtin_bit_cast(float, __builtin_amdgcn_readlane(__builtin_bit_cast(int, rv), 32));
                  st_k[k] = h ? k1 : k0;
                  st_s1[k] = st_s2[k] = 0.f;
                }
              }
              const float d = inr ? rv - st_k[k] : 0.f;
              st_s1[k] += d;
              st_s2[k] = __builtin_fmaf(d, d, st_s2[k]);
            }
            if constexpr (W_OUT) amx_o = fmaxf(amx_o, inr ? fabsf(rv) : 0.f);
            if constexpr (W_ACT) {
              const float e = elu ? fast_elu(y) : y;
              ev[kk][v] = e;
              amx_a = fmaxf(amx_a, inr ? fabsf(e) : 0.f);
            }
          }
        }
        if (inr) {
#pragma unroll
          for (int kk = 0; kk < 2; ++kk) {
            const unsigned ob = boff(c, nb, half * 2 + kk);
#if defined(IPDM_W1D_NO_NT)
            if constexpr (W_OUT) *reinterpret_cast<vecv*>(out_b + ob) = ov[kk];
#elif defined(IPDM_W1D_NT_BIG)
            if constexpr (W_OUT) {
              if ((size_t)a.B * a.Cout * HW > (size_t)IPDM_W1D_NT_BIG * 262144) __builtin_nontemporal_store(ov[kk], reinterpret_cast<vecv*>(out_b + ob));
              else *reinterpret_cast<vecv*>(out_b + ob) = ov[kk];
            }
#else
            if constexpr (W_OUT) __builtin_nontemporal_store(ov[kk], reinterpret_cast<vecv*>(out_b + ob));
#endif
#ifdef IPDM_W1D_ACT_NT
            if constexpr (W_ACT) __builtin_nontemporal_store(ev[kk], reinterpret_cast<vecv*>(act_b + ob));
#else
            if constexpr (W_ACT) *reinterpret_cast<vecv*>(act_b + ob) = ev[kk];
#endif
          }
        }
      }
      if constexpr (STATS) {
        const unsigned long long bal = __ballot(inr);
        if constexpr (nb == 0) st_c0 = st_c1 = 0;
        st_c0 += NV * __popcll(bal & 0xffffffffull);
        st_c1 += NV * __popcll(bal >> 32);
        if constexpr (nb == NBU - 1) {
          const float cnt = (float)(h ? st_c1 : st_c0);
          const int tb = (cur_g.y0 / Y_ROWS) * a.tiles_x + cur_g.x0 / (2 * Y_TX);
          const int n_tb = a.tiles_x * a.tiles_y;
#pragma unroll
          for (int k = 0; k < 4; ++k) {
            const float s1 = half_wave_sum(st_s1[k]), s2 = half_wave_sum(st_s2[k]);
            if (ecol == 0) {
              const int co = co0 + ((k >> 1) * 2 + c) * 32 + (k & 1) * 16 + ecg;
              float* sp = a.stats + (((size_t)cur_g.b * a.Cout + co) * n_tb + tb) * 3;
              const float dm = cnt > 0.f ? s1 / cnt : 0.f;
              sp[0] = cnt; sp[1] = st_k[k] + dm; sp[2] = fmaxf(s2 - s1 * dm, 0.f);
            }
          }
        }
      }
      W1D_TE(2);
    });
    __syncthreads();
    W1D_TE(3);
    if (a.amax_out || a.amax_act) {
      const unsigned mo = __builtin_bit_cast(unsigned, ipdm_wave_max(amx_o)), ma = __builtin_bit_cast(unsigned, ipdm_wave_max(amx_a));
      const unsigned uo = __builtin_amdgcn_readfirstlane(mo), ua = __builtin_amdgcn_readfirstlane(ma);
      pend_o = pend_o > uo ? pend_o : uo;
      pend_a = pend_a > ua ? pend_a : ua;
    }
    if (a.dbg) {
      const unsigned long long t = __builtin_amdgcn_s_memtime();
      t_epi += t - tq;
      tq = t;
    }
    if (!has_next) break;
    tile = next_tile;
    if (next_g.b != cur_g.b) hx_scales_of(next_g.b, hx_in, hx_out);
    cur_g = next_g;
  }
  flush_amax();
  if (a.dbg && tid == 0) {
    unsigned long long* d4 = a.dbg + (size_t)blockIdx.x * 4;
    d4[0] = tq - t0; d4[1] = t1 - t0; d4[2] = t_loop; d4[3] = t_epi;
#ifdef IPDM_W1D_TRACE
    unsigned long long* d8 = a.dbg + (size_t)gridDim.x * 4 + (size_t)blockIdx.x * 4;
    d8[0] = te[0]; d8[1] = te[1]; d8[2] = te[2]; d8[3] = te[3];
#endif
  }
}

}

bool wino1d_ok(const ConvArgs& a) {
  if (!(a.D == 1 && a.dil == 1 && a.Cin % (2 * Y_KC) == 0 && a.Cout % Y_CO == 0)) return false;
  if (a.coef ? a.act != IPDM_ACT_ELU : a.act != IPDM_ACT_NONE) return false;
  if (a.out_act && a.act_out != IPDM_ACT_ELU && a.act_out != IPDM_ACT_COPY) return false;
  if ((size_t)a.B * a.Cin * a.H * a.W * 4 >= 0x3fffffffull) return false;
  if (a.stats && !a.out) return false;
  return a.H % 2 == 0 && a.W % 4 == 0 && a.H >= 8 && a.W >= 32 && (reinterpret_cast<uintptr_t>(a.x) & 15) == 0;
}

struct W1dStagger {
  int step = 0, groups = 4, minpass = 0;
};
static W1dStagger w1d_stagger_parse(const char* e) {
  W1dStagger st;
  if (e) {
    int c = 0, g = 4, m = 0;
    const int n = sscanf(e, "%d:%d:%d", &c, &g, &m);
    if (n >= 1) st.step = c / 512;
    if (n >= 2 && (g == 2 || g == 4 || g == 8)) st.groups = g;
    if (n >= 3) st.minpass = m;
  }
  return st;
}

int conv_wino1d_launch(ConvArgs a, hipStream_t s) {
  static const W1dStagger st = w1d_stagger_parse(getenv("IPDM_W1D_STAGGER"));
  a.tiles_x = (a.W + 2 * Y_TX - 1) / (2 * Y_TX);
  a.tiles_y = (a.H + Y_ROWS - 1) / Y_ROWS;
  a.co_tiles = a.Cout / Y_CO;
  const int64_t nblk = (int64_t)a.B * a.tiles_x * a.tiles_y * a.co_tiles;
  if (nblk > 0x7fffffff) return IPDM_EUNSUPPORTED;
  a.phase_step = st.step > 0 && nblk >= (int64_t)st.minpass * 256 ? st.step : 0;
  a.phase_mask = st.groups - 1;
  const dim3 grid(ipdm_persistent_grid(nblk));
  const int outs = (a.out ? 1 : 0) | (a.out_act ? 2 : 0);
#define W1D_LAUNCH(O, S_, P_)                                                                                            \
  return a.coef ? ipdm_launch_lds(conv_wino1d_kernel<O, S_, P_, true>, grid, dim3(512), Y_LDS_BYTES, s, a, (int)nblk)   \
                : ipdm_launch_lds(conv_wino1d_kernel<O, S_, P_, false>, grid, dim3(512), Y_LDS_BYTES, s, a, (int)nblk)
  if (a.pool2) {
    if (a.stats) { if (outs == 3) W1D_LAUNCH(3, true, true); else W1D_LAUNCH(1, true, true); }
    else if (outs == 3) W1D_LAUNCH(3, false, true);
    else if (outs == 1) W1D_LAUNCH(1, false, true);
    else W1D_LAUNCH(2, false, true);
  } else if (a.stats) {
    if (outs == 3) W1D_LAUNCH(3, true, false); else W1D_LAUNCH(1, true, false);
  } else if (outs == 3) W1D_LAUNCH(3, false, false);
  else if (outs == 1) W1D_LAUNCH(1, false, false);
  else W1D_LAUNCH(2, false, false);
#undef W1D_LAUNCH
}

int conv_wino1d_weights(const float* w, void* U, int Cout, int Cin, int npos, hipStream_t s) {
  const int n_cc = (Cin + 15) / 16, n_ct = (Cout + 31) / 32;
  const int64_t total = (int64_t)npos * n_cc * n_ct * 512;
  float* inv_scale = reinterpret_cast<float*>(static_cast<char*>(U) + total * 2 * 2);
  hipLaunchKernelGGL(wino1d_scale_kernel, dim3(n_ct * 32), dim3(256), 0, s, w, inv_scale, Cout, Cin, n_ct * 32, npos);
  hipLaunchKernelGGL(wino1d_weight_kernel, dim3(ipdm_ew_grid(total, 256)), dim3(256), 0, s, w, (unsigned short*)U, inv_scale, Cout,
                     Cin, n_cc, n_ct, npos);
  return ipdm_launch_status();
}

}

using namespace ipdm_conv;

extern "C" int64_t ipdm_conv_wino1d_weight_bytes(int Cout, int Cin) {
  if (Cout <= 0 || Cin <= 0) return -1;
  return (int64_t)12 * ((Cin + 15) / 16) * ((Cout + 31) / 32) * 2048 + (int64_t)((Cout + 31) / 32) * 32 * 4;
}

extern "C" int ipdm_conv_wino1d_pack_weight(const float* w, void* U, int Cout, int Cin, void* stream) {
  IPDM_REQUIRE(w && U && Cout > 0 && Cin > 0);
  return conv_wino1d_weights(w, U, Cout, Cin, 12, ipdm_stream(stream));
}

extern "C" int ipdm_conv2d_wino1d_supported(int Cin, int Cout, int H, int W) {
  return wino1d_ok(conv_query_args(Cin, Cout, 1, H, W, 1)) ? 1 : 0;
}

static int wino1d_entry(const float* x, const void* U, const float* bias, const float* coef, int act, const float* residual,
                        float* out, float* out_act, int act_out, int B, int Cin, int Cout, int H, int W, int pool2, float* stats, const ipdm_conv_ext_t* ext,
                        void* stream) {
  IPDM_REQUIRE(B >= 0 && Cin > 0 && Cout > 0 && H > 0 && W > 0);
  if (B == 0) return IPDM_OK;
  IPDM_REQUIRE(x && U && (out || out_act) && x != out && x != out_act);
  ConvArgs a = conv_launch_args(x, U, bias, residual, out, out_act, act_out, B, Cin, Cout, 1, H, W, 3, 1, 1, ext, conv_debug_stamps());
  a.coef = coef; a.act = coef ? act : IPDM_ACT_NONE;
  a.stats = stats;
  a.pool2 = pool2 ? 1 : 0;
  if (!wino1d_ok(a) || !wino_pairs_aligned(a)) return IPDM_EUNSUPPORTED;
  return conv_wino1d_launch(a, ipdm_stream(stream));
}

extern "C" int ipdm_conv2d_wino1d_f32(const float* x, const void* U, const float* bias, const float* coef, int act,
                                      const float* residual, float* out, float* out_act, int act_out, int B, int Cin, int Cout,
                                      int H, int W, int pool2, const ipdm_conv_ext_t* ext, void* stream) {
  IPDM_REQUIRE(coef || act == IPDM_ACT_NONE);
  return wino1d_entry(x, U, bias, coef, act, residual, out, out_act, act_out, B, Cin, Cout, H, W, pool2, nullptr, ext, stream);
}

extern "C" int ipdm_conv2d_wino1d_stats_partials(int Cin, int Cout, int H, int W) {
  if (!ipdm_conv2d_wino1d_supported(Cin, Cout, H, W)) return 0;
  return ((W + 2 * Y_TX - 1) / (2 * Y_TX)) * ((H + Y_ROWS - 1) / Y_ROWS);
}

extern "C" int ipdm_conv2d_wino1d_stats_f32(const float* x, const void* U, const float* bias, const float* coef, int act,
                                            const float* residual, float* out, float* out_act, int act_out, int B, int Cin,
                                            int Cout, int H, int W, int pool2, float* stats, const ipdm_conv_ext_t* ext,
                                            void* stream) {
  IPDM_REQUIRE(stats != nullptr && out != nullptr && (coef || act == IPDM_ACT_NONE));
  return wino1d_entry(x, U, bias, coef, act, residual, out, out_act, act_out, B, Cin, Cout, H, W, pool2, stats, ext, stream);
}

namespace ipdm_conv {
bool wino1d_vol_ok(const ConvArgs& a) {
  if (!(a.D >= 1 && a.dil == 1 && a.Cin % (2 * Y_KC) == 0 && a.Cout % Y_CO == 0 && !a.coef && a.act == IPDM_ACT_NONE)) return false;
  if (a.out_act && a.act_out != IPDM_ACT_ELU && a.act_out != IPDM_ACT_COPY) return false;
  if (a.pool2 || a.stats) return false;
  if ((size_t)a.B * a.Cin * a.D * a.H * a.W * 4 >= 0x3fffffffull) return false;
  if ((size_t)a.D * a.H * a.W * Y_CO * 4 >= 0xffffffffull) return false;
  return a.H >= 2 && a.W % 4 == 0 && (a.W <= 12 || a.W >= 16) && (reinterpret_cast<uintptr_t>(a.x) & 15) == 0;
}

int conv_wino1d_vol_launch(ConvArgs a, hipStream_t s) {
  const bool pack = a.W <= 12;
  a.tiles_x = pack ? 1 : (a.W + 2 * Y_TX - 1) / (2 * Y_TX);
  a.tiles_y = (a.H + Y_ROWS - 1) / Y_ROWS;
  a.co_tiles = a.Cout / Y_CO;
  const int64_t nblk = (int64_t)a.B * (pack ? (a.D + 1) / 2 : a.D) * a.tiles_x * a.tiles_y * a.co_tiles;
  if (nblk > 0x7fffffff) return IPDM_EUNSUPPORTED;
  static const int compact = ipdm_env_int("IPDM_W1D_COMPACT", 1);
  const bool nbu3 = compact && a.H % Y_ROWS == 0 && (pack ? a.W == 12 : a.W == 24);
  const dim3 grid(ipdm_persistent_grid(nblk));
  const int outs = (a.out ? 1 : 0) | (a.out_act ? 2 : 0);
  if (nbu3) {
    if (outs == 3) return ipdm_launch_lds(conv_wino1d_kernel<3, false, false, false, true, 3>, grid, dim3(512), Y_LDS_BYTES, s, a, (int)nblk);
    if (outs == 1) return ipdm_launch_lds(conv_wino1d_kernel<1, false, false, false, true, 3>, grid, dim3(512), Y_LDS_BYTES, s, a, (int)nblk);
    return ipdm_launch_lds(conv_wino1d_kernel<2, false, false, false, true, 3>, grid, dim3(512), Y_LDS_BYTES, s, a, (int)nblk);
  }
  if (outs == 3) return ipdm_launch_lds(conv_wino1d_kernel<3, false, false, false, true>, grid, dim3(512), Y_LDS_BYTES, s, a, (int)nblk);
  if (outs == 1) return ipdm_launch_lds(conv_wino1d_kernel<1, false, false, false, true>, grid, dim3(512), Y_LDS_BYTES, s, a, (int)nblk);
  return ipdm_launch_lds(conv_wino1d_kernel<2, false, false, false, true>, grid, dim3(512), Y_LDS_BYTES, s, a, (int)nblk);
}
}

extern "C" int64_t ipdm_conv_wino1d_weight_bytes3d(int Cout, int Cin) {
  if (Cout <= 0 || Cin <= 0) return -1;
  return (int64_t)36 * ((Cin + 15) / 16) * ((Cout + 31) / 32) * 2048 + (int64_t)((Cout + 31) / 32) * 32 * 4;
}

extern "C" int ipdm_conv_wino1d_pack_weight3d(const float* w, void* U, int Cout, int Cin, void* stream) {
  IPDM_REQUIRE(w && U && Cout > 0 && Cin > 0);
  return conv_wino1d_weights(w, U, Cout, Cin, 36, ipdm_stream(stream));
}

extern "C" int ipdm_conv3d_wino1d_supported(int Cin, int Cout, int D, int H, int W) {
  return wino1d_vol_ok(conv_query_args(Cin, Cout, D, H, W, 1)) ? 1 : 0;
}

extern "C" int ipdm_conv3d_wino1d_f32(const float* x, const void* U, const float* bias, const float* residual, float* out,
                                      float* out_act, int act_out, int B, int Cin, int Cout, int D, int H, int W,
                                      const ipdm_conv_ext_t* ext, void* stream) {
  IPDM_REQUIRE(B >= 0 && Cin > 0 && Cout > 0 && D > 0 && H > 0 && W > 0);
  if (B == 0) return IPDM_OK;
  IPDM_REQUIRE(x && U && (out || out_act) && x != out && x != out_act);
  ConvArgs a = conv_launch_args(x, U, bias, residual, out, out_act, act_out, B, Cin, Cout, D, H, W, 3, 1, 1, ext, conv_debug_stamps());
  a.kd = 3;
  if (!wino1d_vol_ok(a) || !wino_pairs_aligned(a)) return IPDM_EUNSUPPORTED;
  return conv_wino1d_vol_launch(a, ipdm_stream(stream));
}
```

inverseproblemwithdiffusionmodel_amd/ncsn/models/layers.py:

```python
import os
from functools import partial

import torch
import torch.nn as nn

from ... import ops, _lib
from .normalization import InstanceNorm2dPlus, ConditionalInstanceNorm2dPlus, get_normalization


class _Act:

    def __init__(self, name):
        self.name = name
        self.code = ops.ACT_CODES[name]

    def __call__(self, x):
        return ops.act(x, self.code)


USE_WINOGRAD = os.environ.get("IPDM_WINOGRAD", "1") != "0"
FUSE_POOL = os.environ.get("IPDM_FUSE_POOL", "1") != "0"


def get_act(config):
    name = config.model.nonlinearity.lower()
    if name not in ("elu", "relu", "lrelu", "swish"):
        raise NotImplementedError("activation function does not exist!")
    return _Act(name)


def _act_code(act):
    if act is None:
        return ops.ACT_NONE
    if isinstance(act, _Act):
        return act.code
    if isinstance(act, nn.ELU):
        return ops.ACT_ELU
    if isinstance(act, nn.ReLU):
        return ops.ACT_RELU
    raise NotImplementedError(f"no kernel code for activation {act!r}")


class Conv2d(ops.PackedWeightMixin, nn.Module):

    def __init__(self, in_planes, out_planes, kernel_size=3, dilation=1, bias=True, ndim=2, full_range=False):
        super().__init__()
        assert kernel_size in (1, 3) and ndim in (1, 2, 3)
        self.in_planes, self.out_planes, self.kernel_size, self.dilation = in_planes, out_planes, kernel_size, dilation
        self.ndim = ndim
        self.full_range = full_range
        self.weight = nn.Parameter(torch.empty(out_planes, in_planes, *([kernel_size] * ndim)))
        self.bias = nn.Parameter(torch.empty(out_planes)) if bias else None
        bound = 1.0 / (in_planes * kernel_size ** ndim) ** 0.5
        nn.init.uniform_(self.weight, -bound, bound)
        if bias:
            nn.init.uniform_(self.bias, -bound, bound)
        self._cache = ops.PackedWeightCache()

    def _cached(self, kind, build):
        return self._cache.get(self.weight, kind, build)

    def packed_wino(self):
        return self._cached("wino_f32", ops.conv_wino_weight)

    def packed_wino_bx3(self):
        return self._cached("wino_" + ops.CONV_IMPL, ops.conv_wino_split_weight)

    def packed_wino1d(self):
        return self._cached("wino1d", ops.conv_wino1d_weight)

    def route(self, x, site="ncsn", coef=None, **call):
        return ops.conv_route(site, self.ndim, self.kernel_size, self.dilation, self.in_planes, self.out_planes, tuple(x.shape[2:]),
                              x.data_ptr() % 16 == 0, ops.CONV_IMPL, winograd=USE_WINOGRAD, fuse_pool=FUSE_POOL,
                              full_range=self.full_range, coef=coef is not None,
                              coef_bound=getattr(coef, "_ipdm_amax_bound", None) is not None, **call)

    def fuses_input(self, x, coef):
        return self.route(x, coef=coef, act=ops.ACT_ELU) == ops.ROUTE_WINO1D

    def streams_norm_input(self, x, act):
        return (self.ndim == 2 and self.kernel_size == 3 and self.dilation == 1 and x.dim() == 4
                and ops.conv3x3_fewout_fin_ok(self.in_planes, self.out_planes, x.shape[2], x.shape[3], x, act))

    def stream_norm_input(self, x, coef, act):
        return ops.conv3x3_fewout_fin(x, self.weight.data, None if self.bias is None else self.bias.data, coef, act)

    def packed_conv1d(self):
        return self._cached("conv1d", ops.conv1d_weight)

    def packed_rows(self):
        if self.full_range and ops.CONV_IMPL == "hx2":
            return self._cached("rows_bx3", lambda w: ops.conv1d_rows_weight(w, impl="bx3"))
        return self._cached("rows_" + ops.CONV_IMPL, ops.conv1d_rows_weight)

    def conv1d_ok(self, x):
        return self.ndim == 1 and self.route(x) == ops.ROUTE_SEQ

    def packed(self):
        if self.full_range and ops.CONV_IMPL == "hx2":
            return self._cached("direct_bx3", lambda w: ops.conv_weight(w, impl="bx3"))
        return self._cached("direct_" + ops.CONV_IMPL, ops.conv_weight)

    def forward(self, x, coef=None, act=ops.ACT_NONE, residual=None, out=None, act_out=ops.ACT_NONE, raw=True,
                want_stats=False, in_amax=None, feeds_conv=True, res_second=False, thin_stats=False):
        bias = None if self.bias is None else self.bias.data
        dyn = ops.dynamic_range()
        produce = dyn and feeds_conv
        if in_amax is None and dyn and coef is None and act == ops.ACT_NONE:
            in_amax = ops.in_amax_for(x)
        if self.ndim == 1 and out is not None:
            raise NotImplementedError("Conv2d(ndim=1): no `out=` form")
        route = self.route(x, coef=coef, act=act, residual=residual is not None, out=out is not None, act_out=act_out, raw=raw,
                           want_stats=want_stats)
        tail = dict(act_out=act_out, raw=raw, in_amax=in_amax, want_amax=produce, res_second=res_second)
        if route == ops.ROUTE_SEQ:
            return ops.conv1d(x, self.packed_conv1d(), bias, residual, self.dilation, **tail)
        if route == ops.ROUTE_ROWS:
            return ops.conv1d_rows(x, self.packed_rows(), bias, coef, act, residual, self.dilation, **tail)
        if route == ops.ROUTE_WINO1D and coef is not None:
            return ops.conv2d_wino_bx3(x, self.packed_wino1d(), bias, residual, act_out=act_out, raw=raw, want_stats=want_stats,
                                       in_amax=getattr(coef, "_ipdm_amax_bound", None) if dyn else None, want_amax=produce,
                                       res_second=res_second, coef=coef, act=act)
        if route == ops.ROUTE_THIN:
            if thin_stats:
                return ops.conv3x3_thin(x, self.weight.data, bias, coef, want_stats=True)
            return ops.conv3x3_thin(x, self.weight.data, bias, coef)
        if route == ops.ROUTE_WINO_F32:
            return ops.conv2d_wino(x, self.packed_wino(), bias, residual, act_out=act_out, raw=raw,
                                   dilation=self.dilation)
        if route in (ops.ROUTE_WINO1D, ops.ROUTE_WINO_SPLIT):
            return ops.conv2d_wino_bx3(x, self.packed_wino1d() if route == ops.ROUTE_WINO1D else self.packed_wino_bx3(), bias, residual,
                                       act_out=act_out, raw=raw, dilation=self.dilation, want_stats=want_stats, in_amax=in_amax,
                                       want_amax=produce, res_second=res_second)
        if route == ops.ROUTE_WINO1D_VOL:
            return ops.conv3d(x, self._cached("wino1d_vol", ops.conv_wino1d_weight3d), bias, residual=residual, **tail)
        if route == ops.ROUTE_DIRECT3D:
            return ops.conv3d(x, self.packed(), bias, coef, act, residual, self.dilation, **tail)
        return ops.conv2d(x, self.packed(), bias, coef, act, residual, self.dilation, out=out, **tail)


def conv1x1(in_planes, out_planes, stride=1, bias=True, spec_norm=False, ndim=2):
    assert stride == 1 and not spec_norm
    return Conv2d(in_planes, out_planes, 1, bias=bias, ndim=ndim)


def conv3x3(in_planes, out_planes, stride=1, bias=True, spec_norm=False, ndim=2):
    assert stride == 1 and not spec_norm
    return Conv2d(in_planes, out_planes, 3, bias=bias, ndim=ndim)


def dilated_conv3x3(in_planes, out_planes, dilation, bias=True, spec_norm=False, ndim=2):
    assert not spec_norm
    return Conv2d(in_planes, out_planes, 3, dilation=dilation, bias=bias, ndim=ndim)


def _maxpool(x):
    if x.dim() == 3:
        return ops.maxpool1d5(x)
    return ops.maxpool3d5(x) if x.dim() == 5 else ops.maxpool5(x)


class ConvMeanPool(nn.Module):
    def __init__(self, input_dim, output_dim, kernel_size=3, biases=True, adjust_padding=False, spec_norm=False, ndim=2):
        super().__init__()
        if adjust_padding or spec_norm:
            raise NotImplementedError("adjust_padding / spec_norm are unused by every shipped config")
        if ndim == 3:
            raise NotImplementedError("the 8-way 3-D ConvMeanPool is unused by NCSN3DShallow (all its stages are dilated)")
        self.conv = Conv2d(input_dim, output_dim, kernel_size, bias=biases, ndim=ndim)

    def forward(self, inputs, feeds_conv=True):
        if self.conv.ndim == 1:
            if self.conv.kernel_size == 1:
                return self.conv(ops.meanpool1d2(inputs), feeds_conv=feeds_conv)
            return ops.meanpool1d2(self.conv(inputs, feeds_conv=feeds_conv))
        if self.conv.kernel_size == 1:
            return self.conv(ops.meanpool2(inputs), feeds_conv=feeds_conv)
        return ops.meanpool2(self.conv(inputs, feeds_conv=feeds_conv))

    def fused(self, inputs, residual=None, act_out=ops.ACT_NONE, feeds_conv=True, coef=None, act=ops.ACT_NONE):
        c = self.conv
        route = c.route(inputs, site="pool", coef=coef, act=act, act_out=act_out)
        bias, dyn = None if c.bias is None else c.bias.data, ops.dynamic_range()
        if route is None:
            return None
        if route == ops.ROUTE_SEQ:
            return ops.conv1d(inputs, c.packed_conv1d(), bias, residual, c.dilation,
                              act_out=act_out, in_amax=ops.in_amax_for(inputs) if dyn else None, want_amax=dyn and feeds_conv,
                              pool2=True)
        try:
            if coef is not None:
                return ops.conv2d_wino_bx3(inputs, c.packed_wino1d(), bias, residual,
                                           act_out=act_out, pool2=True, want_stats=True,
                                           in_amax=getattr(coef, "_ipdm_amax_bound", None) if dyn else None,
                                           want_amax=dyn and feeds_conv, coef=coef, act=act)
            return ops.conv2d_wino_bx3(inputs, c.packed_wino1d() if route == ops.ROUTE_WINO1D else c.packed_wino_bx3(), bias, residual,
                                       act_out=act_out, pool2=True, want_stats=True,
                                       in_amax=ops.in_amax_for(inputs), want_amax=dyn and feeds_conv)
        except _lib.IpdmUnsupported:
            return None


class CRPBlock(nn.Module):
    def __init__(self, features, n_stages, act=None, maxpool=True, spec_norm=False, ndim=2):
        super().__init__()
        if not maxpool:
            raise NotImplementedError("average-pool CRP is unused by every shipped config")
        self.convs = nn.ModuleList([conv3x3(features, features, bias=False, spec_norm=spec_norm, ndim=ndim)
                                    for _ in range(n_stages)])
        self.n_stages = n_stages
        self.act = act

    def forward(self, x, x_act=None, want_act=False):
        code = _act_code(self.act)
        x = x_act if x_act is not None else ops.act(x, code)
        path, out_act = x, None
        for i in range(self.n_stages):
            pooled = _maxpool(path)
            if i == self.n_stages - 1:
                if want_act:
                    x, out_act = self.convs[i](pooled, residual=x, act_out=code)
                else:
                    x = self.convs[i](pooled, residual=x)
            elif ops.split_impl():
                path, x = self.convs[i](pooled, residual=x, res_second=True, act_out=ops.ACT_COPY)
            else:
                path = self.convs[i](pooled)
                x = ops.add(path, x)
        return x, out_act


class RCUBlock(nn.Module):
    def __init__(self, features, n_blocks, n_stages, act=None, spec_norm=False, ndim=2):
        super().__init__()
        for i in range(n_blocks):
            for j in range(n_stages):
                setattr(self, '{}_{}_conv'.format(i + 1, j + 1), conv3x3(features, features, bias=False,
                                                                         spec_norm=spec_norm, ndim=ndim))
        self.stride = 1
        self.n_blocks = n_blocks
        self.n_stages = n_stages
        self.act = act

    def forward(self, x, x_act=None, want_act=False, feeds_conv=True, want_stats=False):
        code = _act_code(self.act)
        for i in range(self.n_blocks):
            residual = x
            a = x_act if x_act is not None else ops.act(x, code)
            for j in range(self.n_stages):
                conv = getattr(self, '{}_{}_conv'.format(i + 1, j + 1))
                if j < self.n_stages - 1:
                    _, a = conv(a, act_out=code, raw=False)
                elif i < self.n_blocks - 1 or want_act:
                    x, x_act = conv(a, residual=residual, act_out=code)
                elif want_stats:
                    x, x_act = conv(a, residual=residual, feeds_conv=feeds_conv, want_stats=True), None
                else:
                    x, x_act = conv(a, residual=residual, feeds_conv=feeds_conv), None
        return x, x_act


class MSFBlock(nn.Module):
    def __init__(self, in_planes, features, spec_norm=False, ndim=2):
        super().__init__()
        assert isinstance(in_planes, (list, tuple))
        self.convs = nn.ModuleList([conv3x3(p, features, bias=True, spec_norm=spec_norm, ndim=ndim) for p in in_planes])
        self.features = features

    def forward(self, xs, shape, act_out=ops.ACT_NONE):
        shape = tuple(int(s) for s in shape)
        sums = None
        n = len(self.convs)
        for i, conv in enumerate(self.convs):
            last_act = act_out if i == n - 1 else ops.ACT_NONE
            if tuple(xs[i].shape[2:]) == shape:
                if last_act != ops.ACT_NONE:
                    _, sums = conv(xs[i], residual=sums, act_out=last_act, raw=False)
                else:
                    sums = conv(xs[i], residual=sums, feeds_conv=False)
            else:
                h = conv(xs[i], feeds_conv=False)
                resize = ops.trilinear if h.dim() == 5 else ops.bilinear
                size = shape
                if h.dim() == 3:
                    resize, size = ops.linear1d, shape[0]
                sums = resize(h, size, out=sums, accumulate=sums is not None, act=last_act,
                              want_amax=i == n - 1 and ops.dynamic_range())
        return sums


class RefineBlock(nn.Module):
    def __init__(self, in_planes, features, act=None, start=False, end=False, maxpool=True, spec_norm=False, ndim=2):
        super().__init__()
        assert isinstance(in_planes, (tuple, list))
        self.n_blocks = n_blocks = len(in_planes)
        self.adapt_convs = nn.ModuleList([RCUBlock(in_planes[i], 2, 2, act, spec_norm=spec_norm, ndim=ndim)
                                          for i in range(n_blocks)])
        self.output_convs = RCUBlock(features, 3 if end else 1, 2, act, spec_norm=spec_norm, ndim=ndim)
        if not start:
            self.msf = MSFBlock(in_planes, features, spec_norm=spec_norm, ndim=ndim)
        self.crp = CRPBlock(features, 2, act, maxpool=maxpool, spec_norm=spec_norm, ndim=ndim)
        self.act = act

    def forward(self, xs, output_shape, xs_act=None, want_act=False, feeds_conv=None, want_stats=False):
        assert isinstance(xs, (tuple, list))
        code = _act_code(self.act)
        xs_act = [None] * len(xs) if xs_act is None else xs_act
        single = self.n_blocks == 1
        hs = [self.adapt_convs[i](xs[i], xs_act[i], want_act=single) for i in range(len(xs))]
        if single:
            h, h_act = self.crp(hs[0][0], hs[0][1], want_act=True)
        else:
            a = self.msf([h[0] for h in hs], output_shape, act_out=code)
            h, h_act = self.crp(None, a, want_act=True)
        out, out_act = self.output_convs(h, h_act, want_act=want_act, feeds_conv=want_act if feeds_conv is None else feeds_conv,
                                         want_stats=want_stats and not want_act)
        return (out, out_act) if want_act else out


class ResidualBlock(nn.Module):
    def __init__(self, input_dim, output_dim, resample=None, act=None, normalization=InstanceNorm2dPlus,
                 adjust_padding=False, dilation=None, spec_norm=False, ndim=2):
        super().__init__()
        conv3x3_ = partial(conv3x3, ndim=ndim)
        conv1x1_ = partial(conv1x1, ndim=ndim)
        dilated_conv3x3_ = partial(dilated_conv3x3, ndim=ndim)
        ConvMeanPool_ = partial(ConvMeanPool, ndim=ndim)
        self.non_linearity = act
        self.input_dim = input_dim
        self.output_dim = output_dim
        self.resample = resample
        self.normalization = normalization
        if resample == 'down':
            if dilation is not None:
                self.conv1 = dilated_conv3x3_(input_dim, input_dim, dilation=dilation, spec_norm=spec_norm)
                self.normalize2 = normalization(input_dim)
                self.conv2 = dilated_conv3x3_(input_dim, output_dim, dilation=dilation, spec_norm=spec_norm)
                conv_shortcut = partial(dilated_conv3x3_, dilation=dilation, spec_norm=spec_norm)
            else:
                self.conv1 = conv3x3_(input_dim, input_dim, spec_norm=spec_norm)
                self.normalize2 = normalization(input_dim)
                self.conv2 = ConvMeanPool_(input_dim, output_dim, 3, adjust_padding=adjust_padding, spec_norm=spec_norm)
                conv_shortcut = partial(ConvMeanPool_, kernel_size=1, adjust_padding=adjust_padding,
                                        spec_norm=spec_norm)
        elif resample is None:
            if dilation is not None:
                conv_shortcut = partial(dilated_conv3x3_, dilation=dilation, spec_norm=spec_norm)
                self.conv1 = dilated_conv3x3_(input_dim, output_dim, dilation=dilation, spec_norm=spec_norm)
                self.normalize2 = normalization(output_dim)
                self.conv2 = dilated_conv3x3_(output_dim, output_dim, dilation=dilation, spec_norm=spec_norm)
            else:
                conv_shortcut = partial(conv1x1_, spec_norm=spec_norm)
                self.conv1 = conv3x3_(input_dim, output_dim, spec_norm=spec_norm)
                self.normalize2 = normalization(output_dim)
                self.conv2 = conv3x3_(output_dim, output_dim, spec_norm=spec_norm)
        else:
            raise Exception('invalid resample value')
        if output_dim != input_dim or resample is not None:
            self.shortcut = conv_shortcut(input_dim, output_dim)
        self.normalize1 = normalization(input_dim)

    def forward(self, x, want_act=False):
        code = _act_code(self.non_linearity)
        h = self._norm_act_conv(self.normalize1, self.conv1, x, code, want_stats=True, feeds_conv=False)
        a2 = None
        if self.output_dim == self.input_dim and self.resample is None:
            shortcut = x
        else:
            shortcut = self.shortcut(x, feeds_conv=False)
        if isinstance(self.conv2, ConvMeanPool):
            plain_norm = isinstance(self.normalize2, InstanceNorm2dPlus) and self.conv2.conv.ndim == 2
            coef2 = self.normalize2.coef(h) if plain_norm else None
            fin = plain_norm and code == ops.ACT_ELU and self.conv2.conv.fuses_input(h, coef2)
            a2 = h if fin else (ops.affine_act(h, coef2, code) if plain_norm else self.normalize2(h, code))
            fused = self.conv2.fused(a2, residual=shortcut, act_out=code if want_act else ops.ACT_NONE, feeds_conv=want_act,
                                     coef=coef2 if fin else None, act=code if fin else ops.ACT_NONE)
            if fused is not None:
                return fused
            if fin:
                a2 = ops.affine_act(h, coef2, code)
            out = ops.add(shortcut, self.conv2(a2))
            return (out, ops.act(out, code)) if want_act else out
        if want_act:
            return self._norm_act_conv(self.normalize2, self.conv2, h, code, residual=shortcut, act_out=code, want_stats=True)
        return self._norm_act_conv(self.normalize2, self.conv2, h, code, residual=shortcut, want_stats=True, feeds_conv=False)

    @staticmethod
    def _norm_act_conv(norm, conv, x, code, **kw):
        if code == ops.ACT_ELU and isinstance(conv, Conv2d) and conv.ndim == 2 and isinstance(norm, InstanceNorm2dPlus):
            coef = norm.coef(x)
            if conv.fuses_input(x, coef):
                return conv(x, coef=coef, act=code, **kw)
            return conv(ops.affine_act(x, coef, code), **kw)
        return conv(norm(x, code), **kw)



def _cond_norm_act_conv(coef, conv, x, code, **kw):
    if code == ops.ACT_ELU and isinstance(conv, Conv2d) and conv.fuses_input(x, coef):
        return conv(x, coef=coef, act=code, **kw)
    return conv(ops.affine_act(x, coef, code), **kw)


class ConditionalResidualBlock(nn.Module):
    def __init__(self, input_dim, output_dim, num_classes, resample=None, act=None,
                 normalization=ConditionalInstanceNorm2dPlus, adjust_padding=False, dilation=None, spec_norm=False):
        super().__init__()
        self.non_linearity = act
        self.input_dim = input_dim
        self.output_dim = output_dim
        self.resample = resample
        self.normalization = normalization
        if resample == 'down':
            if dilation is not None:
                self.conv1 = dilated_conv3x3(input_dim, input_dim, dilation=dilation, spec_norm=spec_norm)
                self.normalize2 = normalization(input_dim, num_classes)
                self.conv2 = dilated_conv3x3(input_dim, output_dim, dilation=dilation, spec_norm=spec_norm)
                conv_shortcut = partial(dilated_conv3x3, dilation=dilation, spec_norm=spec_norm)
            else:
                self.conv1 = conv3x3(input_dim, input_dim, spec_norm=spec_norm)
                self.normalize2 = normalization(input_dim, num_classes)
                self.conv2 = ConvMeanPool(input_dim, output_dim, 3, adjust_padding=adjust_padding, spec_norm=spec_norm)
                conv_shortcut = partial(ConvMeanPool, kernel_size=1, adjust_padding=adjust_padding, spec_norm=spec_norm)
        elif resample is None:
            if dilation is not None:
                conv_shortcut = partial(dilated_conv3x3, dilation=dilation, spec_norm=spec_norm)
                self.conv1 = dilated_conv3x3(input_dim, output_dim, dilation=dilation, spec_norm=spec_norm)
                self.normalize2 = normalization(output_dim, num_classes)
                self.conv2 = dilated_conv3x3(output_dim, output_dim, dilation=dilation, spec_norm=spec_norm)
            else:
                conv_shortcut = nn.Conv2d
                self.conv1 = conv3x3(input_dim, output_dim, spec_norm=spec_norm)
                self.normalize2 = normalization(output_dim, num_classes)
                self.conv2 = conv3x3(output_dim, output_dim, spec_norm=spec_norm)
        else:
            raise Exception('invalid resample value')
        if output_dim != input_dim or resample is not None:
            self.shortcut = conv_shortcut(input_dim, output_dim)
        self.normalize1 = normalization(input_dim, num_classes)

    def forward(self, x, y, feeds_conv=False):
        code = _act_code(self.non_linearity)
        h = _cond_norm_act_conv(self.normalize1.coef(x, y), self.conv1, x, code, want_stats=True, feeds_conv=False)
        if self.output_dim == self.input_dim and self.resample is None:
            shortcut = x
        else:
            shortcut = self.shortcut(x, feeds_conv=False)
        coef2 = self.normalize2.coef(h, y)
        if isinstance(self.conv2, ConvMeanPool):
            fin = code == ops.ACT_ELU and self.conv2.conv.fuses_input(h, coef2)
            a2 = h if fin else ops.affine_act(h, coef2, code)
            fused = self.conv2.fused(a2, residual=shortcut, feeds_conv=feeds_conv, coef=coef2 if fin else None,
                                     act=code if fin else ops.ACT_NONE)
            if fused is not None:
                return fused
            if fin:
                a2 = ops.affine_act(h, coef2, code)
            return ops.add(shortcut, self.conv2(a2))
        return _cond_norm_act_conv(coef2, self.conv2, h, code, residual=shortcut, want_stats=True, feeds_conv=feeds_conv)


class CondRCUBlock(nn.Module):
    def __init__(self, features, n_blocks, n_stages, num_classes, normalizer, act=None, spec_norm=False):
        super().__init__()
        for i in range(n_blocks):
            for j in range(n_stages):
                setattr(self, '{}_{}_norm'.format(i + 1, j + 1), normalizer(features, num_classes, bias=True))
                setattr(self, '{}_{}_conv'.format(i + 1, j + 1), conv3x3(features, features, bias=False, spec_norm=spec_norm))
        self.stride = 1
        self.n_blocks = n_blocks
        self.n_stages = n_stages
        self.act = act
        self.normalizer = normalizer

    def forward(self, x, y, want_act=False):
        code = _act_code(self.act)
        x_act = None
        for i in range(self.n_blocks):
            residual = x
            for j in range(self.n_stages):
                norm = getattr(self, '{}_{}_norm'.format(i + 1, j + 1))
                conv = getattr(self, '{}_{}_conv'.format(i + 1, j + 1))
                kw = dict(want_stats=True, feeds_conv=False)
                if j == self.n_stages - 1:
                    kw["residual"] = residual
                    if want_act and i == self.n_blocks - 1:
                        kw["act_out"] = code
                out = _cond_norm_act_conv(norm.coef(x, y), conv, x, code, **kw)
                x, x_act = out if "act_out" in kw else (out, None)
        return (x, x_act) if want_act else x


class CondMSFBlock(nn.Module):
    def __init__(self, in_planes, features, num_classes, normalizer, spec_norm=False):
        super().__init__()
        assert isinstance(in_planes, (list, tuple))
        self.convs = nn.ModuleList()
        self.norms = nn.ModuleList()
        self.features = features
        self.normalizer = normalizer
        for i in range(len(in_planes)):
# ... 74 lines not shown
```

inverseproblemwithdiffusionmodel_amd/ops.py:

```python
import ctypes
import os

import torch

from . import _lib
from ._lib import call, P

ACT_NONE, ACT_ELU, ACT_RELU, ACT_LRELU02, ACT_SWISH = 0, 1, 2, 3, 4
ACT_COPY = 5
CONV_TRACE = None

ACT_CODES = {"none": ACT_NONE, None: ACT_NONE, "elu": ACT_ELU, "relu": ACT_RELU, "lrelu": ACT_LRELU02,
             "swish": ACT_SWISH}


def _gpu(t, dtype=None, name="tensor"):
    if not isinstance(t, torch.Tensor) or not t.is_cuda:
        raise RuntimeError(f"ipdm: {name} must be a GPU tensor (the HIP path has no CPU fallback); got "
                           f"{getattr(t, 'device', type(t))}")
    if dtype is not None and t.dtype != dtype:
        raise TypeError(f"ipdm: {name} must be {dtype}, got {t.dtype}")
    return t if t.is_contiguous() else t.contiguous()


def _ptr(t):
    return P(t.data_ptr()) if t is not None else P(0)


def _inplace_operand(t, dtype, name):
    if not isinstance(t, torch.Tensor) or not t.is_cuda:
        raise RuntimeError(f"ipdm: {name} must be a GPU tensor (the HIP path has no CPU fallback)")
    if t.dtype != dtype:
        raise TypeError(f"ipdm: {name} must be {dtype}, got {t.dtype}")
    if not t.is_contiguous():
        raise ValueError(f"ipdm: {name} must be contiguous (in-place kernel operand; call .contiguous() yourself and "
                         "keep the result)")
    return t


_STREAM_OF_DEVICE = {}


def _written(*tensors):
    for t in tensors:
        if t is not None:
            torch.autograd.graph.increment_version(t)


def _stream():
    st = torch.cuda.current_stream()
    h = st.cuda_stream
    if _STREAM_OF_DEVICE.get(st.device_index, h) != h or st.device_index not in _STREAM_OF_DEVICE:
        _note_stream(st.device_index, h)
    return P(h)


def _note_stream(dev, h):
    if torch.cuda.is_current_stream_capturing():
        return
    first = _STREAM_OF_DEVICE.setdefault(dev, h)
    if first != h and os.environ.get("IPDM_ALLOW_MULTI_STREAM", "0") != "1":
        raise RuntimeError(
            f"ipdm: kernels were launched on stream {first:#x} of cuda:{dev} and now on stream {h:#x}: this library runs on ONE "
            "stream per device (two queues on one MI355X silently corrupt packed-fp32 results, "
            "profiles/r03_shared_card_probe.txt). Use one stream, or set IPDM_ALLOW_MULTI_STREAM=1 to take the risk.")


def _c64_as_f32(t):
    return torch.view_as_real(t)


_FLOAT_SUFFIX = {torch.float32: "f32", torch.float16: "f16", torch.float64: "f64"}


def _float_suffix(t, what):
    try:
        return _FLOAT_SUFFIX[t.dtype]
    except KeyError:
        raise TypeError(f"ipdm {what}: dtype {t.dtype} (float32 / float16 / float64, as the reference's "
                        "AT_DISPATCH_FLOATING_TYPES_AND_HALF)") from None


def upfirdn2d_raw(x, kernel, up_x, up_y, down_x, down_y, pad_x0, pad_x1, pad_y0, pad_y1):
    sfx = _float_suffix(x, "upfirdn2d")
    x = _gpu(x, x.dtype, "input")
    kernel = _gpu(kernel.to(x.dtype), x.dtype, "kernel")
    major, in_h, in_w, minor = x.shape
    kh, kw = kernel.shape
    out_h = (in_h * up_y + pad_y0 + pad_y1 - kh) // down_y + 1
    out_w = (in_w * up_x + pad_x0 + pad_x1 - kw) // down_x + 1
    out = torch.empty((major, out_h, out_w, minor), dtype=x.dtype, device=x.device)
    call(f"ipdm_upfirdn2d_{sfx}", _ptr(x), _ptr(kernel), _ptr(out), major, in_h, in_w, minor, kh, kw,
         up_x, up_y, down_x, down_y, pad_x0, pad_x1, pad_y0, pad_y1, _stream())
    return out


def fused_bias_act_raw(x, bias, ref, act, grad, alpha, scale):
    sfx = _float_suffix(x, "fused_bias_act")
    x = _gpu(x, x.dtype, "input")
    bias = None if bias is None or bias.numel() == 0 else _gpu(bias.to(x.dtype), x.dtype, "bias")
    ref = None if ref is None or ref.numel() == 0 else _gpu(ref, x.dtype, "refer")
    step_b = 1
    for s in x.shape[2:]:
        step_b *= s
    y = torch.empty_like(x)
    call(f"ipdm_fused_bias_act_{sfx}", _ptr(x), _ptr(bias), _ptr(ref), _ptr(y), x.numel(), step_b,
         0 if bias is None else bias.numel(), act, grad, float(alpha), float(scale), _stream())
    return y


KSPACE_NONE, KSPACE_LDS, KSPACE_STRIPS = 0, 1, 2
KSPACE_SIZE_RULE = ("each side a power of two from 4, or a multiple of 16 of the form 2^a 3^b 5^c between 16 and 2048 "
                    "(e.g. 48, 80, 96, 144, 160, 192, 240, 288, 320, 384)")


def kspace_size_class(H, W):
    return int(_lib.lib.ipdm_kspace_size_class(int(H), int(W)))


def fft2c(x, inverse=False):
    x = _gpu(x, name="input")
    if x.dtype != torch.complex64:
        x = x.to(torch.complex64)
    H, W = x.shape[-2:]
    batch = x.numel() // (H * W) if H * W else 0
    out = torch.empty_like(x)
    ws_bytes = _lib.lib.ipdm_fft2c_workspace_bytes(batch, H, W)
    ws = torch.empty(ws_bytes // 4, dtype=torch.float32, device=x.device) if ws_bytes else None
    call("ipdm_fft2c_c64", _ptr(x), _ptr(out), batch, H, W, int(bool(inverse)), _ptr(ws), _stream())
    return out


def _mask_u8(mask, H, W, device):
    m = torch.as_tensor(mask)
    if m.is_complex():
        raise TypeError(f"mask: bool, integer or real floating dtype, got {m.dtype}")
    shape = tuple(m.shape)
    if not 1 <= len(shape) <= 4:
        raise ValueError(f"mask {shape}: 1 to 4 dims, broadcastable against (B, 1, {H}, {W})")
    T, C, h, w = (1,) * (4 - len(shape)) + shape
    if w != W:
        raise ValueError(f"mask {shape}: last dim {w} != W {W}")
    if h not in (1, H):
        raise ValueError(f"mask {shape}: dim -2 is {h}; 1 (a line mask) or H = {H} (a 2-D mask)")
    if C != 1:
        raise ValueError(f"mask {shape}: channel dim {C} != 1")
    if T < 1:
        raise ValueError(f"mask {shape}: no planes")
    m = m.to(device=device).reshape((T, W) if h == 1 and H != 1 else (T, H, W))
    return (m != 0).to(torch.uint8).contiguous()


def _mask_t(mask_u8, H, W, what):
    if not isinstance(mask_u8, torch.Tensor) or not mask_u8.is_cuda:
        raise RuntimeError(f"ipdm {what}: mask must be a GPU tensor (the HIP path has no CPU fallback)")
    if mask_u8.dtype != torch.uint8:
        raise TypeError(f"ipdm {what}: mask must be uint8 (ops._mask_u8 converts a host mask), got {mask_u8.dtype}")
    if not mask_u8.is_contiguous():
        raise ValueError(f"ipdm {what}: mask must be contiguous")
    shape = tuple(mask_u8.shape)
    if len(shape) == 2 and shape[0] >= 1 and shape[1] == W:
        return shape[0]
    if len(shape) == 3 and shape[0] >= 1 and shape[1:] == (H, W):
        return -shape[0]
    raise ValueError(f"ipdm {what}: mask {shape} is neither a line mask [mask_t, {W}] nor a 2-D mask [T, {H}, {W}]")


def _sens_entry(sens, real_name, csm_name, H, W, sets_name=None, B=None):
    if not isinstance(sens, torch.Tensor) or not sens.is_cuda:
        raise RuntimeError("ipdm: coil maps must be a GPU tensor (the HIP path has no CPU fallback)")
    if sens.dtype not in (torch.float32, torch.complex64):
        raise TypeError(f"ipdm: coil maps must be float32 or complex64, got {sens.dtype}")
    if not sens.is_contiguous():
        raise TypeError("ipdm: coil maps must be contiguous (call .contiguous() and keep the result)")
    if sets_name is not None and sens.dim() == 4:
        if tuple(sens.shape[-2:]) != (H, W) or sens.shape[0] < 1 or sens.shape[1] < 1:
            raise ValueError(f"ipdm: coil maps {tuple(sens.shape)} do not match [S, n_coils, {H}, {W}]")
        if B is not None and B % sens.shape[0]:
            raise ValueError(f"ipdm: a batch of {B} images is not a whole number of samples of {sens.shape[0]} map sets")
        return sets_name
    if sens.dim() != 3 or tuple(sens.shape[-2:]) != (H, W):
        raise ValueError(f"ipdm: coil maps {tuple(sens.shape)} do not match [n_coils, {H}, {W}]")
    return csm_name if sens.dtype == torch.complex64 else real_name


def _sens_tail(sens):
    return (int(sens.dtype == torch.complex64), sens.shape[0]) if sens.dim() == 4 else ()


def sense_forward(x, sens_f32, mask_u8):
    x = _gpu(x, torch.complex64, "x")
    B = x.numel() // (x.shape[-1] * x.shape[-2])
    H, W = x.shape[-2:]
    fn = "ipdm_sense_forward_c64" if sens_f32 is None else _sens_entry(sens_f32, "ipdm_sense_forward_c64",
                                                                        "ipdm_sense_forward_csm_c64", H, W,
                                                                        "ipdm_sense_forward_sets_c64", B)
    n = 1 if sens_f32 is None else sens_f32.shape[-3]
    tail = () if sens_f32 is None else _sens_tail(sens_f32)
    y = torch.empty((n,) + tuple(x.shape), dtype=torch.complex64, device=x.device)
    mask_t = _mask_t(mask_u8, H, W, "sense_forward")
    call(fn, _ptr(x), _ptr(sens_f32), *tail, _ptr(mask_u8), mask_t, _ptr(y), B, n, H, W,
         _stream())
    return y


def sense_workspace(B, n_coils, H, W, device):
    nbytes = _lib.lib.ipdm_sense_workspace_bytes(B, n_coils, H, W)
    return torch.empty(nbytes // 4, dtype=torch.float32, device=device) if nbytes else None


def _check_work(work, B, n_coils, H, W, what):
    need = _lib.lib.ipdm_sense_workspace_bytes(B, n_coils, H, W)
    if need == 0:
        return
    if (not isinstance(work, torch.Tensor) or not work.is_cuda or work.dtype != torch.float32 or not work.is_contiguous()
            or work.numel() * 4 < need):
        raise ValueError(f"{what}: `work` must be a contiguous float32 GPU tensor of >= {need} bytes "
                         f"(ops.sense_workspace({B}, {n_coils}, {H}, {W}, device))")


def _large_image(H, W):
    return H * W > 16384


def sense_adjoint(s, sens_f32, mask_u8=None, apply_mask=False):
    s = _gpu(s, torch.complex64, "s")
    n = s.shape[0]
    H, W = s.shape[-2:]
    B = s[0].numel() // (H * W)
    fn = _sens_entry(sens_f32, "ipdm_sense_adjoint_c64", "ipdm_sense_adjoint_csm_c64", H, W,
                     "ipdm_sense_adjoint_sets_c64", B)
    if sens_f32.shape[-3] != n:
        raise ValueError(f"sense_adjoint: {n} coil images, {sens_f32.shape[-3]} coil maps")
    x = torch.empty(tuple(s.shape[1:]), dtype=torch.complex64, device=s.device)
    ws = sense_workspace(B, n, H, W, s.device) if _large_image(H, W) else None
    call(fn, _ptr(s), _ptr(sens_f32), *_sens_tail(sens_f32), _ptr(mask_u8),
         1 if mask_u8 is None else _mask_t(mask_u8, H, W, "sense_adjoint"), int(bool(apply_mask)), _ptr(x), _ptr(ws), B, n, H, W, _stream())
    return x


def sense_ssos(s):
    s = _gpu(s, torch.complex64, "s")
    n = s.shape[0]
    H, W = s.shape[-2:]
    B = s[0].numel() // (H * W)
    out = torch.empty(tuple(s.shape[1:]), dtype=torch.float32, device=s.device)
    ws = sense_workspace(B, n, H, W, s.device) if _large_image(H, W) else None
    call("ipdm_sense_ssos_c64", _ptr(s), _ptr(out), _ptr(ws), B, n, H, W, _stream())
    return out


def sense_l2prox(z_re, z_im, y, sens_f32, mask_u8, coef, out_re=None, out_im=None, work=None):
    z_re, z_im = _gpu(z_re, torch.float32, "z_re"), _gpu(z_im, torch.float32, "z_im")
    y = _gpu(y, torch.complex64, "y")
    H, W = z_re.shape[-2:]
    B = z_re.numel() // (H * W)
    fn = _sens_entry(sens_f32, "ipdm_sense_l2prox_f32", "ipdm_sense_l2prox_csm_f32", H, W, "ipdm_sense_l2prox_sets_f32", B)
    n = sens_f32.shape[-3]
    if y.numel() != n * B * H * W:
        raise ValueError("sense_l2prox: measurement does not match [n_coils, B, H, W]")
    out_re = torch.empty_like(z_re) if out_re is None else out_re
    out_im = torch.empty_like(z_im) if out_im is None else out_im
    work = sense_workspace(B, n, H, W, z_re.device) if work is None else work
    _check_work(work, B, n, H, W, "sense_l2prox")
    mask_t = _mask_t(mask_u8, H, W, "sense_l2prox")
    call(fn, _ptr(z_re), _ptr(z_im), _ptr(y), _ptr(sens_f32), *_sens_tail(sens_f32), _ptr(mask_u8), mask_t,
         float(coef), _ptr(out_re), _ptr(out_im), _ptr(work), B, n, H, W, _stream())
    _written(out_re, out_im)
    return out_re, out_im


def _fused_step(what, x_re, x_im, g_re, g_im, y, noise_re, noise_im, step, noise_scale, seed, sample_offset, step_id,
                dev_sched, sens=None, entries=None):
    for t, n in ((x_re, "x_re"), (x_im, "x_im"), (g_re, "g_re"), (g_im, "g_im")):
        _inplace_operand(t, torch.float32, n)
    H, W = x_re.shape[-2:]
    B = x_re.numel() // (H * W) if H * W else 0
    fn = _sens_entry(sens, entries[0], entries[1], H, W, entries[2], B) if entries else None
    _inplace_operand(y, torch.complex64, "y")
    if entries:
        for t, n in ((noise_re, "noise_re"), (noise_im, "noise_im")):
            if t is not None:
                _inplace_operand(t, torch.float32, n)
        if g_re.numel() != x_re.numel() or g_im.numel() != x_im.numel() or y.numel() != sens.shape[-3] * B * H * W:
            raise ValueError(f"{what}: operand sizes do not match the state")
    head = (_ptr(x_re), _ptr(x_im), _ptr(g_re), _ptr(g_im), _ptr(noise_re), _ptr(noise_im), float(step), float(noise_scale),
            int(seed), int(sample_offset), int(step_id), _ptr(dev_sched))
    return fn, B, H, W, head


def ald_sense_step(x_re, x_im, g_re, g_im, y, sens_f32, mask_u8, work, step=0.0, noise_scale=0.0, coef=0.0,
                   noise_re=None, noise_im=None, seed=0, sample_offset=0, step_id=0, dev_sched=None):
    fn, B, H, W, head = _fused_step("ald_sense_step", x_re, x_im, g_re, g_im, y, noise_re, noise_im, step, noise_scale, seed,
                                    sample_offset, step_id, dev_sched, sens_f32,
                                    ("ipdm_ald_sense_step_f32", "ipdm_ald_sense_step_csm_f32",
                                     "ipdm_ald_sense_step_sets_f32"))
    n = sens_f32.shape[-3]
    _check_work(work, B, n, H, W, "ald_sense_step")
    mask_t = _mask_t(mask_u8, H, W, "ald_sense_step")
    call(fn, *head, _ptr(y), _ptr(sens_f32), *_sens_tail(sens_f32), _ptr(mask_u8), mask_t, float(coef), _ptr(work), B, n,
         H, W, _stream())
    _written(x_re, x_im)
# ... 1623 lines not shown
        return conv_bx3(x, wt, bias, coef, act, residual, dilation, act_out=act_out, raw=raw, in_amax=in_amax,
                        want_amax=want_amax, res_second=res_second)
    if res_second:
        raise _lib.IpdmUnsupported("conv3d: res_second exists on the split-operand kernels only")
    x = _gpu(x, torch.float32, "x")
    B, Cin, D, H, W = x.shape
    kk, Cin_w, Cout = wt.shape
    if Cin_w != Cin:
        raise ValueError(f"conv3d: weight Cin {Cin_w} != input Cin {Cin}")
    k = {1: 1, 27: 3}[kk]
    out, out_act, _, _ = _conv_outputs(x, (B, Cout, D, H, W), raw, act_out)
    e0 = _trace_open()
    call("ipdm_conv3d_f32", _ptr(x), _ptr(wt), _ptr(bias), _ptr(coef), act, _ptr(residual), _ptr(out), _ptr(out_act),
         act_out, B, Cin, Cout, D, H, W, k, dilation, _stream())
    return _conv_done(e0, out, out_act, B=B * D, Cin=Cin, Cout=Cout, H=H, W=W, k=k, dil=dilation, taps3d=kk, res=residual is not None)


def maxpool3d5(x):
    x = _gpu(x, torch.float32, "x")
    B, C, D, H, W = x.shape
    out = torch.empty_like(x)
    call("ipdm_maxpool3d5_f32", _ptr(x), _ptr(out), B * C, D, H, W, _stream())
    return carry_amax(x, out)


def temporal_taps(x, mode):
    x = _gpu(x, torch.float32, "x")
    B, C, D, H, T = x.shape
    T_out = T // 2 if mode == 0 else T * 2
    out = torch.empty((B, 4 * C, D, H, T_out), dtype=torch.float32, device=x.device)
    call("ipdm_temporal_taps_f32", _ptr(x), _ptr(out), B * C, D * H, T, T_out, mode, _stream())
    return carry_amax(x, out)


def conv2d(x, wt, bias=None, coef=None, act=ACT_NONE, residual=None, dilation=1, pool2=False, out=None,
           act_out=ACT_NONE, raw=True, in_amax=None, out_scale=1.0, want_amax=False, res_second=False):
    if isinstance(wt, PackedBx3):
        if pool2:
            raise _lib.IpdmUnsupported("conv2d: pool2 epilogue is not fused")
        return conv_bx3(x, wt, bias, coef, act, residual, dilation, out=out, act_out=act_out, raw=raw, in_amax=in_amax,
                        out_scale=out_scale, want_amax=want_amax, res_second=res_second)
    if out_scale != 1.0 or (bias is not None and bias.dim() == 2) or res_second:
        raise _lib.IpdmUnsupported("conv2d: per-image bias / out_scale exist on the split-operand kernels only")
    x = _gpu(x, torch.float32, "x")
    B, Cin, H, W = x.shape
    kk, Cin_w, Cout = wt.shape
    if Cin_w != Cin:
        raise ValueError(f"conv2d: weight Cin {Cin_w} != input Cin {Cin}")
    k = {1: 1, 9: 3}[kk]
    oh, ow = (H // 2, W // 2) if pool2 else (H, W)
    out, out_act, _, _ = _conv_outputs(x, (B, Cout, oh, ow), raw, act_out, "conv2d", out)
    e0 = _trace_open()
    call("ipdm_conv2d_f32", _ptr(x), _ptr(wt), _ptr(bias), _ptr(coef), act, _ptr(residual), _ptr(out), _ptr(out_act),
         act_out, B, Cin, Cout, H, W, k, dilation, int(bool(pool2)), _stream())
    _written(out)
    return _conv_done(e0, out, out_act, B=B, Cin=Cin, Cout=Cout, H=H, W=W, k=k, dil=dilation, res=residual is not None)


USE_THIN_CONV = os.environ.get("IPDM_THIN_CONV", "1") != "0"


def conv3x3_thin_ok(Cin, Cout, H, W, x=None):
    if x is not None and x.data_ptr() % 16:
        return False
    return USE_THIN_CONV and bool(_lib.lib.ipdm_conv3x3_thin_supported(int(Cin), int(Cout), int(H), int(W)))


THIN_STATS = os.environ.get("IPDM_THIN_STATS", "1") != "0"
THIN_FIN = os.environ.get("IPDM_THIN_FIN", "1") != "0"
END_STATS = os.environ.get("IPDM_END_STATS", "1") != "0"


def conv3x3_thin_stats_ok(Cin, Cout, H, W, x=None):
    return (THIN_STATS and USE_STATS_EPILOGUE and conv3x3_thin_ok(Cin, Cout, H, W, x)
            and int(_lib.lib.ipdm_conv3x3_thin_stats_partials(int(Cin), int(Cout), int(H), int(W))) > 0)


def conv3x3_fewout_fin_ok(Cin, Cout, H, W, x, act=ACT_ELU):
    return (THIN_FIN and act == ACT_ELU and x.dim() == 4 and Cout <= 3 < Cin and conv3x3_thin_ok(Cin, Cout, H, W, x)
            and bool(_lib.lib.ipdm_conv3x3_fewout_fin_supported(int(Cin), int(Cout), int(H), int(W))))


def conv3x3_fewout_fin(x, weight, bias, coef, act=ACT_ELU):
    x = _gpu(x, torch.float32, "x")
    weight = _gpu(weight, torch.float32, "weight")
    coef = _gpu(coef, torch.float32, "coef")
    B, Cin, H, W = x.shape
    Cout = weight.shape[0]
    if tuple(weight.shape) != (Cout, Cin, 3, 3):
        raise ValueError(f"conv3x3_fewout_fin: weight {tuple(weight.shape)} does not match input channels {Cin}")
    if tuple(coef.shape) != (B, Cin, 3):
        raise ValueError(f"conv3x3_fewout_fin: coef {tuple(coef.shape)} != {(B, Cin, 3)}")
    out = torch.empty((B, Cout, H, W), dtype=torch.float32, device=x.device)
    e0 = _trace_open()
    call("ipdm_conv3x3_fewout_fin_f32", _ptr(x), _ptr(weight), _ptr(bias), _ptr(coef), act, _ptr(out), B, Cin, Cout, H, W, _stream())
    return _conv_done(e0, out, None, B=B, Cin=Cin, Cout=Cout, H=H, W=W, k=3, dil=1, res=False, thin=True, fin=True)


def conv3x3_thin(x, weight, bias=None, coef=None, want_stats=False):
    x = _gpu(x, torch.float32, "x")
    weight = _gpu(weight, torch.float32, "weight")
    B, Cin, H, W = x.shape
    Cout = weight.shape[0]
    if tuple(weight.shape) != (Cout, Cin, 3, 3):
        raise ValueError(f"conv3x3_thin: weight {tuple(weight.shape)} does not match input channels {Cin}")
    out = torch.empty((B, Cout, H, W), dtype=torch.float32, device=x.device)
    e0 = _trace_open()
    if coef is not None:
        coef = _gpu(coef, torch.float32, "coef")
        if tuple(coef.shape) != (B, Cin, 3):
            raise ValueError(f"conv3x3_thin: coef {tuple(coef.shape)} != {(B, Cin, 3)}")
    if want_stats and conv3x3_thin_stats_ok(Cin, Cout, H, W, x):
        P = int(_lib.lib.ipdm_conv3x3_thin_stats_partials(Cin, Cout, H, W))
        part = torch.empty((B, Cout, P, 3), dtype=torch.float32, device=x.device)
        call("ipdm_conv3x3_thin_stats_f32", _ptr(x), _ptr(weight), _ptr(bias), _ptr(coef), _ptr(out), _ptr(part), B, Cin, Cout, H, W,
             _stream())
        out._ipdm_partials = (part, (out._version, out.data_ptr()))
        return _conv_done(e0, out, None, B=B, Cin=Cin, Cout=Cout, H=H, W=W, k=3, dil=1, res=False, thin=True, stats=True)
    call("ipdm_conv3x3_thin_f32", _ptr(x), _ptr(weight), _ptr(bias), _ptr(coef), _ptr(out), B, Cin, Cout, H, W, _stream())
    return _conv_done(e0, out, None, B=B, Cin=Cin, Cout=Cout, H=H, W=W, k=3, dil=1, res=False, thin=True)


CONV_IMPL = os.environ.get("IPDM_CONV_IMPL", "hx2")
SPLIT_IMPLS = ("hx2", "bx3")
if CONV_IMPL not in SPLIT_IMPLS + ("f32",):
    raise ValueError(f"IPDM_CONV_IMPL={CONV_IMPL!r}: expected 'hx2', 'bx3' or 'f32'")


def split_impl():
    return CONV_IMPL in SPLIT_IMPLS


def impl_unbounded():
    env = os.environ.get("IPDM_CONV_IMPL_UNBOUNDED")
    if env:
        if env not in SPLIT_IMPLS + ("f32",):
            raise ValueError(f"IPDM_CONV_IMPL_UNBOUNDED={env!r}")
        return env
    return CONV_IMPL


def unbounded_amax():
    return True if impl_unbounded() == "hx2" else None


class PackedWeightCache:

    def __init__(self):
        self._entries = {}

    def clear(self):
        self._entries.clear()

    def get(self, weight, kind, build):
        tag = (weight._version, weight.data_ptr(), str(weight.device))
        hit = self._entries.get(kind)
        if hit is None or hit[0] != tag:
            hit = (tag, build(weight.data))
            self._entries[kind] = hit
        return hit[1]


class PackedWeightMixin:

    def invalidate(self):
        self._cache.clear()

    def _load_from_state_dict(self, *args, **kwargs):
        self._cache.clear()
        return super()._load_from_state_dict(*args, **kwargs)


def conv_weight(w, impl=None):
    impl = CONV_IMPL if impl is None else impl
    return conv_bx3_weight(w, fmt=impl) if impl in SPLIT_IMPLS else conv_pack_weight(w)


class PackedBx3:
    __slots__ = ("blob", "Cout", "Cin", "kk", "fmt")

    def __init__(self, blob, Cout, Cin, kk, fmt="bx3"):
        self.blob, self.Cout, self.Cin, self.kk, self.fmt = blob, Cout, Cin, kk, fmt


def absmax_per_image(x):
    x = _gpu(x, torch.float32, "x")
    B = x.shape[0]
    out = torch.empty((B, AMAX_SLOT), dtype=torch.float32, device=x.device)
    call("ipdm_absmax_f32", _ptr(x), _ptr(out), B, x.numel() // max(B, 1), _stream())
    return out


def _conv_ext(fmt, in_amax, x, fused_input, bias_per_image=False, out_scale=1.0, Cout=0, out_amax=None, act_amax=None,
              res_second=False):
    amax_ptr = None
    if fmt == "hx2" and in_amax is not None and not fused_input:
        if in_amax is True:
            in_amax = absmax_per_image(x)
        if (tuple(in_amax.shape) != (x.shape[0], AMAX_SLOT) or in_amax.dtype != torch.float32 or not in_amax.is_cuda
                or not in_amax.is_contiguous()):
            raise ValueError(f"in_amax: expected a maxima vector -- contiguous float32 GPU tensor [{x.shape[0]}, {AMAX_SLOT}] "
                             "(ops.absmax_per_image / a producer's tag)")
        amax_ptr = in_amax.data_ptr()
        _KEEP.append(in_amax)
    if (amax_ptr is None and not bias_per_image and out_scale == 1.0 and out_amax is None and act_amax is None
            and not res_second):
        return P(0)
    ext = _lib.ConvExt(amax_ptr, int(Cout) if bias_per_image else 0, float(out_scale), int(bool(res_second)),
                       None if out_amax is None else out_amax.data_ptr(), None if act_amax is None else act_amax.data_ptr())
    _KEEP.append(ext)
    del _KEEP[:-8]
    return ctypes.byref(ext)


_KEEP = []


def conv_hx2_weight(w):
    return conv_bx3_weight(w, fmt="hx2")


def conv_bx3_weight(w, fmt="bx3"):
    if fmt not in SPLIT_IMPLS:
        raise ValueError(f"conv_bx3_weight: fmt {fmt!r}")
    w = _gpu(w, torch.float32, "weight")
    Cout, Cin = w.shape[:2]
    kk = 1
    for n in w.shape[2:]:
        kk *= int(n)
    if w.dim() == 5:
        if kk not in (1, 27):
            raise ValueError("3-D kernels must be 1x1x1 or 3x3x3")
        k = 27 if kk == 27 else 1
    else:
        k = {1: 1, 9: 3}[kk]
    nbytes = getattr(_lib.lib, f"ipdm_conv_{fmt}_weight_bytes")(Cout, Cin, k)
    blob = torch.empty(nbytes, dtype=torch.uint8, device=w.device)
    call(f"ipdm_conv_{fmt}_pack_weight", _ptr(w), _ptr(blob), Cout, Cin, k, _stream())
    return PackedBx3(blob, Cout, Cin, kk, fmt)


def conv_bx3(x, wq, bias=None, coef=None, act=ACT_NONE, residual=None, dilation=1, out=None, act_out=ACT_NONE, raw=True,
             in_amax=None, out_scale=1.0, want_amax=False, res_second=False):
    x = _gpu(x, torch.float32, "x")
    bias_per_image = bias is not None and bias.dim() == 2
    if bias_per_image and (tuple(bias.shape) != (x.shape[0], wq.Cout) or bias.stride(1) != 1):
        raise ValueError(f"conv_bx3: per-image bias {tuple(bias.shape)} != {(x.shape[0], wq.Cout)} (rows may be strided, not columns)")
    _need_both("conv_bx3", res_second, residual, act_out, raw)
    if wq.Cin != x.shape[1]:
        raise ValueError(f"conv_bx3: weight Cin {wq.Cin} != input Cin {x.shape[1]}")
    vol = x.dim() == 5
    k = {1: 1, 9: 3, 27: 3}[wq.kk]
    if (wq.kk == 27) != (vol and k == 3):
        raise ValueError("conv_bx3: kernel / input rank mismatch")
    shape = (x.shape[0], wq.Cout) + tuple(x.shape[2:])
    out, out_act, slot_o, slot_a = _conv_outputs(x, shape, raw, act_out, "conv_bx3", out, want_amax)
    ext = _conv_ext(wq.fmt, in_amax, x, coef is not None or act != ACT_NONE, bias_per_image, out_scale,
                    bias.stride(0) if bias_per_image else 0, slot_o, slot_a, res_second)
    e0 = _trace_open()
    if vol:
        B, Cin, D, H, W = x.shape
    else:
        B, Cin, H, W = x.shape
        D = 1
    ksplit = _lib.lib.ipdm_conv_bx3_splitk(B, D, Cin, wq.Cout, H, W, k, dilation) if B else 1
    if ksplit > 1:
        work = torch.empty((ksplit,) + shape, dtype=torch.float32, device=x.device)
        call(f"ipdm_conv_{wq.fmt}_splitk_f32", _ptr(x), _ptr(wq.blob), _ptr(bias), _ptr(coef), act, _ptr(residual), _ptr(out),
             _ptr(out_act), act_out, B, Cin, wq.Cout, D, H, W, k, dilation, int(vol), ksplit, _ptr(work), ext, _stream())
    elif vol:
        call(f"ipdm_conv3d_{wq.fmt}_f32", _ptr(x), _ptr(wq.blob), _ptr(bias), _ptr(coef), act, _ptr(residual), _ptr(out),
             _ptr(out_act), act_out, B, Cin, wq.Cout, D, H, W, k, dilation, ext, _stream())
    else:
        call(f"ipdm_conv2d_{wq.fmt}_f32", _ptr(x), _ptr(wq.blob), _ptr(bias), _ptr(coef), act, _ptr(residual), _ptr(out),
             _ptr(out_act), act_out, B, Cin, wq.Cout, H, W, k, dilation, ext, _stream())
    _written(out)
    return _conv_done(e0, out, out_act, slot_o, slot_a, B=B * D, Cin=Cin, Cout=wq.Cout, H=H, W=W, k=k, dil=dilation, bx3=True,
                      fmt=wq.fmt, res=residual is not None, taps3d=wq.kk if vol else None)


def conv_wino_bx3_weight(w, fmt="bx3"):
    if fmt not in SPLIT_IMPLS:
        raise ValueError(f"conv_wino_bx3_weight: fmt {fmt!r}")
    w = _gpu(w, torch.float32, "weight")
    Cout, Cin = w.shape[:2]
    nbytes = getattr(_lib.lib, f"ipdm_conv_wino_{fmt}_weight_bytes")(Cout, Cin)
    blob = torch.empty(nbytes, dtype=torch.uint8, device=w.device)
    call(f"ipdm_conv_wino_{fmt}_pack_weight", _ptr(w), _ptr(blob), Cout, Cin, _stream())
    return PackedBx3(blob, Cout, Cin, 16, fmt)


def conv_wino_hx2_weight(w):
    return conv_wino_bx3_weight(w, fmt="hx2")


def conv_wino1d_weight(w):
    w = _gpu(w, torch.float32, "weight")
    Cout, Cin = w.shape[:2]
    blob = torch.empty(_lib.lib.ipdm_conv_wino1d_weight_bytes(Cout, Cin), dtype=torch.uint8, device=w.device)
    call("ipdm_conv_wino1d_pack_weight", _ptr(w), _ptr(blob), Cout, Cin, _stream())
    return PackedBx3(blob, Cout, Cin, 12, "hx2")


def conv_wino1d_weight3d(w):
    w = _gpu(w, torch.float32, "weight")
    Cout, Cin = w.shape[:2]
    if tuple(w.shape[2:]) != (3, 3, 3):
        raise ValueError(f"conv_wino1d_weight3d: weight {tuple(w.shape)}")
    blob = torch.empty(_lib.lib.ipdm_conv_wino1d_weight_bytes3d(Cout, Cin), dtype=torch.uint8, device=w.device)
    call("ipdm_conv_wino1d_pack_weight3d", _ptr(w), _ptr(blob), Cout, Cin, _stream())
    return PackedBx3(blob, Cout, Cin, 36, "hx2")


def conv3d_wino1d(x, U, bias=None, residual=None, act_out=ACT_NONE, raw=True, in_amax=None, want_amax=False, res_second=False):
    x = _gpu(x, torch.float32, "x")
    B, Cin, D, H, W = x.shape
    if U.kk != 36 or U.Cin != Cin:
        raise ValueError("conv3d_wino1d: weight blob does not match the input")
    _need_both("conv3d_wino1d", res_second, residual, act_out, raw, how="")
    Cout = U.Cout
    if residual is not None and tuple(residual.shape) != (B, Cout, D, H, W):
        raise ValueError(f"conv3d_wino1d: residual {tuple(residual.shape)} != output {(B, Cout, D, H, W)}")
    residual = _wino_residual(residual)
    amax_t = None
    if in_amax is not None:
        amax_t = absmax_per_image(x) if in_amax is True else in_amax
    out, out_act, slot_o, slot_a = _conv_outputs(x, (B, Cout, D, H, W), raw, act_out, want_amax=want_amax)
    e0 = _trace_open()
    nb = max(1, (0x3fffffff - 1) // (Cin * D * H * W * 4))
    for n, cut in _chunks(B, nb):
        ext = _conv_ext("hx2", cut(amax_t), cut(x), False, False, 1.0, 0, cut(slot_o), cut(slot_a), res_second)
        call("ipdm_conv3d_wino1d_f32", _ptr(cut(x)), _ptr(U.blob), _ptr(bias), _ptr(cut(residual)), _ptr(cut(out)), _ptr(cut(out_act)),
             act_out, n, Cin, Cout, D, H, W, ext, _stream())
    return _conv_done(e0, out, out_act, slot_o, slot_a, B=B * D, Cin=Cin, Cout=Cout, H=H, W=W, k=3, dil=1, wino=True, bx3=True,
                      fmt="hx2", wino1d=True, res=residual is not None, taps3d=27)


def wino1d_vol_pays(Cin, Cout, D, H, W, dilation=1):
    return (WINO1D and WINO1D_VOL and CONV_IMPL == "hx2" and dilation == 1
            and bool(_lib.lib.ipdm_conv3d_wino1d_supported(int(Cin), int(Cout), int(D), int(H), int(W))))


WINO1D_VOL = os.environ.get("IPDM_WINO1D_VOL", "1") != "0"
WINO1D = os.environ.get("IPDM_WINO1D", "1") != "0"
WINO1D_STATS = os.environ.get("IPDM_WINO1D_STATS", "1") != "0"
WINO1D_FIN = os.environ.get("IPDM_WINO1D_FIN", "0") != "0"


def wino1d_pays(Cin, Cout, H, W, dilation=1):
    return (WINO1D and CONV_IMPL == "hx2" and dilation == 1
            and bool(_lib.lib.ipdm_conv2d_wino1d_supported(int(Cin), int(Cout), int(H), int(W))))


def conv_wino_split_weight(w, impl=None):
    impl = CONV_IMPL if impl is None else impl
    return conv_wino_bx3_weight(w, fmt=impl if impl in SPLIT_IMPLS else "bx3")


def conv_wino_bx3_supported(Cin, Cout, H, W, dilation=1):
    return bool(_lib.lib.ipdm_conv2d_wino_bx3_supported(Cin, Cout, H, W, dilation))


def conv2d_wino_bx3(x, U, bias=None, residual=None, act_out=ACT_NONE, raw=True, dilation=1, pool2=False, want_stats=False,
                    in_amax=None, out_scale=1.0, want_amax=False, res_second=False, coef=None, act=ACT_NONE):
    x = _gpu(x, torch.float32, "x")
    B, Cin, H, W = x.shape
    amax_t = None
    if U.fmt == "hx2" and in_amax is not None:
        if in_amax is True and coef is not None:
            raise ValueError("conv2d_wino_bx3: with a fused input the maxima are the coefficient kernel's bound, not max |x|")
        amax_t = absmax_per_image(x) if in_amax is True else in_amax
    bias_per_image = bias is not None and bias.dim() == 2
    if bias_per_image and (tuple(bias.shape) != (B, U.Cout) or bias.stride(1) != 1):
        raise ValueError(f"conv2d_wino_bx3: per-image bias {tuple(bias.shape)} != {(B, U.Cout)} (rows may be strided, not columns)")
    one_d = U.kk == 12
    if U.kk not in (12, 16) or U.Cin != Cin:
        raise ValueError("conv2d_wino_bx3: weight blob does not match the input")
    if one_d and (dilation != 1 or U.fmt != "hx2"):
        raise ValueError("conv2d_wino_bx3: the 1-D Winograd blob serves undilated f16x2 launches only")
    if coef is not None or act != ACT_NONE:
        if not one_d or coef is None or act != ACT_ELU:
            raise ValueError("conv2d_wino_bx3: a fused input (coef + ACT_ELU) is the 1-D Winograd kernel's only")
        coef = _gpu(coef, torch.float32, "coef")
        if tuple(coef.shape) != (B, Cin, 3):
            raise ValueError(f"conv2d_wino_bx3: coef {tuple(coef.shape)} != {(B, Cin, 3)}")
    _need_both("conv2d_wino_bx3", res_second, residual, act_out, raw)
    Cout = U.Cout
    oh, ow = (H // 2, W // 2) if pool2 else (H, W)
    if residual is not None and tuple(residual.shape) != (B, Cout, oh, ow):
        raise ValueError(f"conv2d_wino_bx3: residual {tuple(residual.shape)} != output {(B, Cout, oh, ow)}")
    residual = _wino_residual(residual)
    out, out_act, slot_o, slot_a = _conv_outputs(x, (B, Cout, oh, ow), raw, act_out, want_amax=want_amax)
    e0 = _trace_open()
    nb = wino_bx3_max_batch(Cin, H, W, dilation)
    ksplit = 1 if one_d or pool2 or x.data_ptr() % 16 or (WBX3_CO32 and U.fmt == "hx2") else wino_bx3_splitk(Cin, Cout, H, W, dilation)
    part = None
    if ksplit == 1 and want_stats and raw and USE_STATS_EPILOGUE and x.data_ptr() % 16 == 0:
        P = (int(_lib.lib.ipdm_conv2d_wino1d_stats_partials(Cin, Cout, H, W)) if one_d else
             int(_lib.lib.ipdm_conv2d_wino_bx3_stats_partials(Cin, Cout, H, W, dilation, int(bool(pool2)))))
        if P > 0:
            part = torch.empty((B, Cout, P, 3), dtype=torch.float32, device=x.device)
    for n, cut in _chunks(B, nb):
        head = (_ptr(cut(x)), _ptr(U.blob), _ptr(cut(bias) if bias_per_image else bias))
        outs = (_ptr(cut(residual)), _ptr(cut(out)), _ptr(cut(out_act)), act_out, n, Cin, Cout, H, W)
        ext = _conv_ext(U.fmt, cut(amax_t), cut(x), False, bias_per_image, out_scale, bias.stride(0) if bias_per_image else 0,
                        cut(slot_o), cut(slot_a), res_second)
        if ksplit > 1:
            work = torch.empty((ksplit, n, Cout, H, W), dtype=torch.float32, device=x.device)
            call(f"ipdm_conv2d_wino_{U.fmt}_splitk_f32", *head, *outs, dilation, ksplit, _ptr(work), ext, _stream())
        elif one_d:
            stats = () if part is None else (_ptr(cut(part)),)
            call("ipdm_conv2d_wino1d_f32" if part is None else "ipdm_conv2d_wino1d_stats_f32", *head, _ptr(cut(coef)), act, *outs,
                 int(bool(pool2)), *stats, ext, _stream())
        else:
            args = head + outs + (dilation, int(bool(pool2)))
            if part is not None:
                try:
                    call(f"ipdm_conv2d_wino_{U.fmt}_stats_f32", *args, _ptr(cut(part)), ext, _stream())
                    continue
                except _lib.IpdmUnsupported:
                    part = None
            call(f"ipdm_conv2d_wino_{U.fmt}_f32", *args, ext, _stream())
    if part is not None:
        out._ipdm_partials = (part, (out._version, out.data_ptr()))
    form = dict(pool2=False, ksplit=ksplit) if ksplit > 1 else dict(pool2=bool(pool2), wino1d=one_d, stats=part is not None)
    return _conv_done(e0, out, out_act, slot_o, slot_a, B=B, Cin=Cin, Cout=Cout, H=H, W=W, k=3, dil=dilation, wino=True, bx3=True,
                      fmt=U.fmt, res=residual is not None, **form)


WBX3_CO32 = os.environ.get("IPDM_WBX3_CO32", "1") != "0"


def wino_bx3_pays(Cin, Cout, H, W, dilation=1, B=None):
    if W <= 16 and dilation == 1:
        if wino_bx3_splitk(Cin, Cout, H, W, dilation) > 1:
            return True
        if H > 16 or Cout < 512 or Cin < 32:
            return False
    return conv_wino_bx3_supported(Cin, Cout, H, W, dilation)


def wino_bx3_splitk(Cin, Cout, H, W, dilation=1):
    return int(_lib.lib.ipdm_conv2d_wino_bx3_splitk(int(Cin), int(Cout), int(H), int(W), int(dilation)))


WINO_FORM_OTHER, WINO_FORM_CO32, WINO_FORM_HALF, WINO_FORM_POLY = 0, 1, 2, 3


def wino_hx2_form(Cin, Cout, H, W, dilation=1):
    f = int(_lib.lib.ipdm_conv2d_wino_hx2_form(int(Cin), int(Cout), int(H), int(W), int(dilation)))
    return None if f < 0 else f


def wino_bx3_max_batch(Cin, H, W, dilation=1):
    reach = 0x1fffffff if (W < 32 or dilation > 1) else 0x3fffffff
    return max(1, (reach - 1) // (Cin * H * W * 4))


def adam_ascent(x, g, m, v, lr, step, betas=(0.9, 0.999), eps=1e-8):
    for t, n in ((x, "x"), (g, "g"), (m, "m"), (v, "v")):
        _inplace_operand(t, torch.float32, n)
        if t.numel() != x.numel():
            raise ValueError(f"adam_ascent: {n} does not match x")
    call("ipdm_adam_ascent_f32", _ptr(x), _ptr(g), _ptr(m), _ptr(v), x.numel(), float(lr), float(betas[0]), float(betas[1]),
         float(eps), int(step), _stream())
    _written(x, m, v)
    return x


USE_CONV1D = os.environ.get("IPDM_CONV1D", "1") != "0"
CONV1D_LAUNCHES = 0
CONV1D_FALLBACKS = 0


def conv1d_pays(Cin, Cout, L, k, dilation=1):
    return (USE_CONV1D and CONV_IMPL == "hx2"
            and bool(_lib.lib.ipdm_conv1d_hx2_supported(int(Cin), int(Cout), int(L), int(k), int(dilation))))


ROUTE_THIN, ROUTE_WINO_F32, ROUTE_WINO1D, ROUTE_WINO_SPLIT = "thin", "wino_f32", "wino1d", "wino_split"
ROUTE_WINO1D_VOL, ROUTE_SEQ, ROUTE_ROWS, ROUTE_DIRECT2D, ROUTE_DIRECT3D = "wino1d_vol", "conv1d", "rows", "direct2d", "direct3d"


def conv_route(site, ndim, k, dilation, Cin, Cout, size, aligned, impl, winograd=True, fuse_pool=True, full_range=False,
               coef=False, coef_bound=False, act=ACT_NONE, residual=False, out=False, act_out=ACT_NONE, raw=True, want_stats=False):
    plain_in = not coef and act == ACT_NONE
    if ndim == 1:
        seq = plain_in and not full_range and conv1d_pays(Cin, Cout, size[0], k, dilation)
        if site == "pool":
            return ROUTE_SEQ if fuse_pool and k == 3 and size[0] % 2 == 0 and seq else None
        return ROUTE_SEQ if seq else ROUTE_ROWS
    H, W = size[0], size[1]
    wino = winograd and impl in SPLIT_IMPLS and ndim == 2 and k == 3

    def one_d():
        return (impl == "hx2" and aligned and act_out in (ACT_NONE, ACT_ELU, ACT_COPY) and wino1d_pays(Cin, Cout, H, W, dilation))
    if site == "pool":
        if not (fuse_pool and wino and dilation == 1 and H % 2 == 0 and W % 2 == 0 and wino_bx3_pays(Cin, Cout, H, W, 1)):
            return None
        if one_d() and WINO1D_STATS:
            return ROUTE_WINO1D
        return None if coef else ROUTE_WINO_SPLIT
    if (site == "ncsn" and coef and act == ACT_ELU and not out and WINO1D_FIN and wino and len(size) == 2 and aligned
            and (not dynamic_range(impl) or coef_bound) and wino1d_pays(Cin, Cout, H, W, dilation)):
        return ROUTE_WINO1D
    if (ndim == 2 and k == 3 and dilation == 1 and act == ACT_NONE and not residual and not out and act_out == ACT_NONE and raw
            and len(size) == 2 and (Cin <= 3 or (Cout <= 3 and not coef)) and aligned and conv3x3_thin_ok(Cin, Cout, H, W)):
        return ROUTE_THIN
    if (site == "ncsn" and winograd and impl == "f32" and ndim == 2 and k == 3 and plain_in and not out
            and conv_wino_supported(Cin, Cout, H, W, dilation)):
        return ROUTE_WINO_F32
    if wino and plain_in and not out and wino_bx3_pays(Cin, Cout, H, W, dilation):
        stats_ok = site == "sde" or WINO1D_STATS or not (want_stats and raw and USE_STATS_EPILOGUE)
        return ROUTE_WINO1D if one_d() and stats_ok else ROUTE_WINO_SPLIT
    if (ndim == 3 and k == 3 and dilation == 1 and plain_in and not out and len(size) == 3 and aligned
            and act_out in (ACT_NONE, ACT_ELU, ACT_COPY) and wino1d_vol_pays(Cin, Cout, *size)):
        return ROUTE_WINO1D_VOL
    return ROUTE_DIRECT3D if ndim == 3 else ROUTE_DIRECT2D


class PackedConv1d:
    __slots__ = ("blob", "Cout", "Cin", "k")

    def __init__(self, blob, Cout, Cin, k):
        self.blob, self.Cout, self.Cin, self.k = blob, Cout, Cin, k


def conv1d_weight(w):
    w = _gpu(w, torch.float32, "weight")
    if w.dim() != 3:
        raise ValueError(f"conv1d_weight: expected [Cout, Cin, k], got {tuple(w.shape)}")
    Cout, Cin, k = (int(v) for v in w.shape)
    nbytes = _lib.lib.ipdm_conv1d_hx2_weight_bytes(Cout, Cin, k)
    if nbytes < 0:
        raise _lib.IpdmUnsupported(f"conv1d_weight: no 1-D kernel for a [{Cout}, {Cin}, {k}] filter")
    blob = torch.empty(nbytes, dtype=torch.uint8, device=w.device)
    call("ipdm_conv1d_hx2_pack_weight", _ptr(w), _ptr(blob), Cout, Cin, k, _stream())
    return PackedConv1d(blob, Cout, Cin, k)


def conv1d_rows_weight(w, impl=None):
    w = _gpu(w, torch.float32, "weight")
    Cout, Cin, k = (int(v) for v in w.shape)
    if k == 1:
        return conv_weight(w.reshape(Cout, Cin, 1, 1), impl=impl)
    w2 = torch.zeros((Cout, Cin, 3, 3), dtype=torch.float32, device=w.device)
    w2[:, :, 1, :] = w
    return conv_weight(w2, impl=impl)


def as_rows(x):
    return carry_amax(x, x.view(x.shape[0], x.shape[1], 1, x.shape[2]))


def as_seq(x):
    return carry_amax(x, x.view(x.shape[0], x.shape[1], x.shape[3]))


def conv1d_rows(x, wt, bias=None, coef=None, act=ACT_NONE, residual=None, dilation=1, act_out=ACT_NONE, raw=True, in_amax=None,
                want_amax=False, res_second=False):
    global CONV1D_FALLBACKS
    CONV1D_FALLBACKS += 1
    x = _gpu(x, torch.float32, "x")
    res = None if residual is None else as_rows(_gpu(residual, torch.float32, "residual"))
    y = conv2d(as_rows(x), wt, bias, coef, act, res, dilation, act_out=act_out, raw=raw, in_amax=in_amax, want_amax=want_amax,
               res_second=res_second)
    if act_out != ACT_NONE:
        return (None if y[0] is None else as_seq(y[0])), as_seq(y[1])
    return as_seq(y)


def conv1d(x, wq, bias=None, residual=None, dilation=1, act_out=ACT_NONE, raw=True, in_amax=None, want_amax=False,
           res_second=False, pool2=False):
    global CONV1D_LAUNCHES
    x = _gpu(x, torch.float32, "x")
    if x.dim() != 3 or x.shape[1] != wq.Cin:
        raise ValueError(f"conv1d: input {tuple(x.shape)} for a filter with Cin {wq.Cin}")
    N, Cin, L = (int(v) for v in x.shape)
    if pool2 and L % 2:
        raise ValueError("conv1d: the pair mean needs an even length")
    shape = (N, wq.Cout, L // 2 if pool2 else L)
    out, out_act, slot_o, slot_a = _conv_outputs(x, shape, raw, act_out, "conv1d", None, want_amax, amax_cap=None)
    _need_both("conv1d", res_second, residual, act_out, raw)
    if residual is not None:
        residual = _gpu(residual, torch.float32, "residual")
        if tuple(residual.shape) != shape:
            raise ValueError(f"conv1d: residual {tuple(residual.shape)} != {shape}")
    ext = _conv_ext("hx2", in_amax, x, False, False, 1.0, 0, slot_o, slot_a, res_second)
    e0 = _trace_open()
    call("ipdm_conv1d_hx2_f32", _ptr(x), _ptr(wq.blob), _ptr(bias), _ptr(residual), _ptr(out), _ptr(out_act), act_out, N, Cin,
         wq.Cout, L, wq.k, int(dilation), int(bool(pool2)), ext, _stream())
    CONV1D_LAUNCHES += 1
    return _conv_done(e0, out, out_act, slot_o, slot_a, B=N, Cin=Cin, Cout=wq.Cout, H=1, W=L, k=wq.k, dil=dilation, conv1d=True,
                      res=residual is not None)


def meanpool1d2(x):
    x = _gpu(x, torch.float32, "x")
    L = int(x.shape[-1])
    if L % 2:
        raise ValueError("meanpool1d2: the length must be even")
    out = torch.empty(tuple(x.shape[:-1]) + (L // 2,), dtype=torch.float32, device=x.device)
    call("ipdm_meanpool1d2_f32", _ptr(x), _ptr(out), x.numel() // L, L, _stream())
    return carry_amax(x, out)


def scale_shift_amax(x, a, b):
    x = _gpu(x, torch.float32, "x")
    B = int(x.shape[0])
    out = torch.empty_like(x)
    slot = amax_slot(B, x.device)
    call("ipdm_scale_shift_amax_f32", _ptr(x), _ptr(out), _ptr(slot), B, x.numel() // max(B, 1), float(a), float(b), _stream())
    return tag_amax(out, slot)


def maxpool1d5(x):
    return as_seq(maxpool5(as_rows(x)))


def linear1d(x, size, out=None, accumulate=False, act=ACT_NONE, want_amax=False):
    x = _gpu(x, torch.float32, "x")
    out4 = None if out is None else out.view(out.shape[0], out.shape[1], 1, out.shape[2])
    return as_seq(bilinear(as_rows(x), (1, int(size)), out=out4, accumulate=accumulate, act=act, want_amax=want_amax))
```

Before: 0.1317 reconstructions/s.

## Fold 2x2 average pool into 1-D Winograd conv weights for pooled convolutions

Adds a folded weight form for the 1-D Winograd kernel on pooled layers. The vertical 2-tap pool sum is folded into a 4-row kernel and the horizontal pooling is folded into the output transform, so each tile computes only the pooled output. This halves the accumulator tiles and skips the cross-lane shuffle averaging, at the cost of a fourth kernel row (more B loads and MFMAs per row pair) and a second cached weight blob per layer. It is enabled by default through an environment flag and a context manager that offers the pooled blob to the launcher.

```diff
diff --git a/include/ipdm.h b/include/ipdm.h
--- a/include/ipdm.h
+++ b/include/ipdm.h
@@ -432,6 +432,8 @@
 int64_t ipdm_conv_wino1d_weight_bytes(int Cout, int Cin);
 int ipdm_conv_wino1d_pack_weight(const float* w , void* U, int Cout, int Cin, void* stream);
 int ipdm_conv2d_wino1d_supported(int Cin, int Cout, int H, int W);
+int64_t ipdm_conv_wino1d_pool_weight_bytes(int Cout, int Cin);
+int ipdm_conv_wino1d_pack_weight_pool(const float* w , void* U, int Cout, int Cin, void* stream);
 int64_t ipdm_conv_wino1d_weight_bytes3d(int Cout, int Cin);
 int ipdm_conv_wino1d_pack_weight3d(const float* w, void* U, int Cout, int Cin, void* stream);
 int ipdm_conv3d_wino1d_supported(int Cin, int Cout, int D, int H, int W);
diff --git a/inverseproblemwithdiffusionmodel_amd/_lib.py b/inverseproblemwithdiffusionmodel_amd/_lib.py
--- a/inverseproblemwithdiffusionmodel_amd/_lib.py
+++ b/inverseproblemwithdiffusionmodel_amd/_lib.py
@@ -179,6 +179,8 @@
     "ipdm_conv_wino_hx2_weight_bytes": [c_int, c_int],
     "ipdm_conv_wino1d_weight_bytes": [c_int, c_int],
     "ipdm_conv_wino1d_pack_weight": [P, P, c_int, c_int, P],
+    "ipdm_conv_wino1d_pool_weight_bytes": [c_int, c_int],
+    "ipdm_conv_wino1d_pack_weight_pool": [P, P, c_int, c_int, P],
     "ipdm_conv2d_wino1d_supported": [c_int, c_int, c_int, c_int],
     "ipdm_conv_wino1d_weight_bytes3d": [c_int, c_int],
     "ipdm_conv_wino1d_pack_weight3d": [P, P, c_int, c_int, P],
@@ -221,6 +223,7 @@
              "ipdm_conv_bx3_weight_bytes": c_int64,
              "ipdm_conv_wino_bx3_weight_bytes": c_int64, "ipdm_conv_hx2_weight_bytes": c_int64,
              "ipdm_conv_wino_hx2_weight_bytes": c_int64, "ipdm_conv_wino1d_weight_bytes": c_int64, "ipdm_conv_wino1d_weight_bytes3d": c_int64,
+             "ipdm_conv_wino1d_pool_weight_bytes": c_int64,
              "ipdm_conv1d_hx2_weight_bytes": c_int64, "ipdm_csm_workspace_bytes": ctypes.c_size_t,
              "ipdm_coilcomp_workspace_bytes": ctypes.c_size_t, "ipdm_gcc_workspace_bytes": ctypes.c_size_t,
              "ipdm_espirit_workspace_bytes": ctypes.c_size_t, "ipdm_nc_coil_gram_workspace_bytes": ctypes.c_size_t}
diff --git a/inverseproblemwithdiffusionmodel_amd/csrc/conv_wino1d.hip b/inverseproblemwithdiffusionmodel_amd/csrc/conv_wino1d.hip
--- a/inverseproblemwithdiffusionmodel_amd/csrc/conv_wino1d.hip
+++ b/inverseproblemwithdiffusionmodel_amd/csrc/conv_wino1d.hip
@@ -18,22 +18,32 @@
 constexpr float HX1_PRESCALE = 0.5f;
 constexpr int Y_QC = 10, Y_RC4 = 40, Y_QN = 100;
 
-__device__ __forceinline__ float wino1d_U(const float* g, int p) {
-  g += (p / 12) * 9;
-  p %= 12;
+__device__ __forceinline__ float wino1d_U(const float* g, int p, bool fold) {
   const float G[4][3] = {{1.f, 0.f, 0.f}, {0.5f, 0.5f, 0.5f}, {0.5f, -0.5f, 0.5f}, {0.f, 0.f, 1.f}};
-  const int ky = p >> 2, xi = p & 3;
-  return G[xi][0] * g[ky * 3 + 0] + G[xi][1] * g[ky * 3 + 1] + G[xi][2] * g[ky * 3 + 2];
+  float t[3];
+  const int xi = p & 3;
+  if (fold) {
+    const int r = p >> 2;
+#pragma unroll
+    for (int k = 0; k < 3; ++k) t[k] = (r < 3 ? g[r * 3 + k] : 0.f) + (r > 0 ? g[(r - 1) * 3 + k] : 0.f);
+  } else {
+    g += (p / 12) * 9;
+    p %= 12;
+    const int ky = p >> 2;
+#pragma unroll
+    for (int k = 0; k < 3; ++k) t[k] = g[ky * 3 + k];
+  }
+  return G[xi][0] * t[0] + G[xi][1] * t[1] + G[xi][2] * t[2];
 }
 
 __global__ __launch_bounds__(256) void wino1d_scale_kernel(const float* __restrict__ w, float* __restrict__ inv_scale, int Cout,
-                                                           int Cin, int n_co_pad, int npos) {
+                                                           int Cin, int n_co_pad, int npos, bool fold) {
   __shared__ float red[256];
   const int co = blockIdx.x;
   float m = 0.f;
   if (co < Cout)
     for (int i = threadIdx.x; i < Cin * npos; i += 256)
-      m = fmaxf(m, fabsf(wino1d_U(w + ((size_t)co * Cin + i / npos) * (npos / 12 * 9), i % npos)));
+      m = fmaxf(m, fabsf(wino1d_U(w + ((size_t)co * Cin + i / npos) * (npos / 12 * 9), i % npos, fold)));
   red[threadIdx.x] = m;
   __syncthreads();
   for (int st = 128; st > 0; st >>= 1) {
@@ -50,7 +60,7 @@
 
 __global__ __launch_bounds__(256) void wino1d_weight_kernel(const float* __restrict__ w, unsigned short* __restrict__ out,
                                                             const float* __restrict__ inv_scale, int Cout, int Cin, int n_cc,
-                                                            int n_ct, int npos) {
+                                                            int n_ct, int npos, bool fold) {
   const int64_t total = (int64_t)npos * n_cc * n_ct * 512;
   for (int64_t i = (int64_t)blockIdx.x * 256 + threadIdx.x; i < total; i += (int64_t)gridDim.x * 256) {
     const int q = (int)(i & 7), r = (int)((i >> 3) & 31), h = (int)((i >> 8) & 1);
@@ -60,7 +70,7 @@
     const int p = (int)(rest / ((int64_t)n_ct * n_cc));
     const int co = ct * 32 + r, ci = cc * 16 + 8 * h + q;
     float v = 0.f;
-    if (co < Cout && ci < Cin) v = wino1d_U(w + ((size_t)co * Cin + ci) * (npos / 12 * 9), p) * (1.f / (inv_scale[co] * HX1_PRESCALE));
+    if (co < Cout && ci < Cin) v = wino1d_U(w + ((size_t)co * Cin + ci) * (npos / 12 * 9), p, fold) * (1.f / (inv_scale[co] * HX1_PRESCALE));
     const _Float16 hi = (_Float16)v;
     const _Float16 lo = (_Float16)(v - (float)hi);
     const int64_t base = rest * 2 * 512 + h * 256 + r * 8 + q;
@@ -69,8 +79,11 @@
   }
 }
 
-template <int OUTS, bool STATS = false, bool POOL = false, bool FIN = false, bool VOL = false, int NBU = 4>
+template <int OUTS, bool STATS = false, bool POOL = false, bool FIN = false, bool VOL = false, int NBU = 4, bool FOLD = false>
 __global__ __launch_bounds__(512) void conv_wino1d_kernel(ConvArgs a, int total_tiles) {
+  static_assert(!FOLD || (POOL && !VOL && !FIN && NBU == 4), "FOLD: the pooled form, plain input, images");
+  constexpr int NBA = FOLD ? 2 : NBU;
+  constexpr int NKY = FOLD ? 4 : 3;
   extern __shared__ __align__(16) float lds[];
   unsigned* const ldsw = reinterpret_cast<unsigned*>(lds);
   const int tid = threadIdx.x;
@@ -286,7 +299,7 @@
 #pragma unroll
       for (int s = 0; s < 2; ++s) fr[c][s] = base[c * 128 + s * 64];
   };
-  const int b_lane = (j >> 4) * Y_RS + xi * 256 + h * 32 + (j & 15);
+  const int b_lane = (j >> 4) * (FOLD ? 2 : 1) * Y_RS + xi * 256 + h * 32 + (j & 15);
   [[maybe_unused]] int b_cmp[3] = {0, 0, 0};
   if constexpr (NBU == 3) {
 #pragma unroll
@@ -297,16 +310,16 @@
   }
   auto load_B = [&](uint4 (&fr)[2], const unsigned* cur, auto kyc, auto nbc) {
     constexpr int ky = decltype(kyc)::value, nb = decltype(nbc)::value;
-    const unsigned* bp = NBU == 3 ? cur + ky * Y_RS + b_cmp[nb < 3 ? nb : 0] : cur + (2 * nb + ky) * Y_RS + b_lane;
+    const unsigned* bp = NBU == 3 ? cur + ky * Y_RS + b_cmp[nb < 3 ? nb : 0] : cur + ((FOLD ? 4 : 2) * nb + ky) * Y_RS + b_lane;
 #pragma unroll
     for (int s = 0; s < 2; ++s) fr[s] = make_uint4(bp[s * 128], bp[s * 128 + 16], bp[s * 128 + 64], bp[s * 128 + 80]);
   };
 
-  f32x16 acc[2][NBU];
-#pragma unroll
-  for (int i = 0; i < 2 * NBU; ++i)
-#pragma unroll
-    for (int rr = 0; rr < 16; ++rr) acc[i / NBU][i % NBU][rr] = 0.f;
+  f32x16 acc[2][NBA];
+#pragma unroll
+  for (int i = 0; i < 2 * NBA; ++i)
+#pragma unroll
+    for (int rr = 0; rr < 16; ++rr) acc[i / NBA][i % NBA][rr] = 0.f;
 
   auto lds_barrier = [&]() {
     __builtin_amdgcn_sched_barrier(0);
@@ -373,7 +386,7 @@
           else set_fin(cur_g.b, ch + 1, cur_g.y0, cur_g.x0);
         }
         uint4 bsh[2][2];
-        __builtin_amdgcn_s_waitcnt(0x0F78);
+        __builtin_amdgcn_s_waitcnt(FOLD ? 0x0F7C : 0x0F78);
         read_items();
         load_B(bsh[0], cur, std::integral_constant<int, 0>{}, std::integral_constant<int, 0>{});
         __builtin_amdgcn_sched_barrier(0);
@@ -381,16 +394,19 @@
         issue_dma(dma_chunk);
         __builtin_amdgcn_sched_barrier(0);
         float va[4], vb[4];
-        static_for<3 * NBU>([&](auto ssc) {
+        constexpr int NSS = NKY * NBA;
+        static_for<NSS>([&](auto ssc) {
           constexpr int ss = decltype(ssc)::value;
-          constexpr int ky = ss / NBU, nb = ss % NBU;
-          constexpr int aslot = (cpar * 3 + ky) & 1;
-          if constexpr (ss < 3 * NBU - 1)
-            load_B(bsh[(ss + 1) & 1], cur, std::integral_constant<int, (ss + 1) / NBU>{}, std::integral_constant<int, (ss + 1) % NBU>{});
-          constexpr int it = ky;
-          if constexpr (nb == 0) xform_item(std::integral_constant<int, it>{}, va, vb);
-          if constexpr (nb == 1) store_item(nxt, std::integral_constant<int, it>{}, va, vb, std::integral_constant<int, 0>{}, std::integral_constant<int, 2>{});
-          if constexpr (nb == 2) store_item(nxt, std::integral_constant<int, it>{}, va, vb, std::integral_constant<int, 2>{}, std::integral_constant<int, 4>{});
+          constexpr int ky = ss / NBA, nb = ss % NBA;
+          constexpr int aslot = FOLD ? (ky & 1) : ((cpar * 3 + ky) & 1);
+          if constexpr (ss < NSS - 1)
+            load_B(bsh[(ss + 1) & 1], cur, std::integral_constant<int, (ss + 1) / NBA>{}, std::integral_constant<int, (ss + 1) % NBA>{});
+          constexpr int it = FOLD ? (ss < 6 ? ss / 3 : 2) : ky;
+          constexpr int ph = FOLD ? (ss < 6 ? ss % 3 : ss - 5) : nb;
+          constexpr bool stores = ph == 1 || ph == 2;
+          if constexpr (ph == 0 || (FOLD && ss == 6)) xform_item(std::integral_constant<int, it>{}, va, vb);
+          if constexpr (ph == 1) store_item(nxt, std::integral_constant<int, it>{}, va, vb, std::integral_constant<int, 0>{}, std::integral_constant<int, 2>{});
+          if constexpr (ph == 2) store_item(nxt, std::integral_constant<int, it>{}, va, vb, std::integral_constant<int, 2>{}, std::integral_constant<int, 4>{});
           const f16x8 bh = __builtin_bit_cast(f16x8, bsh[ss & 1][0]), bl = __builtin_bit_cast(f16x8, bsh[ss & 1][1]);
 #pragma unroll
           for (int c = 0; c < 2; ++c) {
@@ -400,17 +416,22 @@
             v = __builtin_amdgcn_mfma_f32_32x32x16_f16(__builtin_bit_cast(f16x8, afr[aslot][c][0]), bh, v, 0, 0, 0);
             acc[c][nb] = v;
           }
-          if constexpr (nb == NBU - 1) {
-            if constexpr (ky == 0) load_A(afr[aslot], 2, ch, cur_g.cob);
-            if constexpr (ky == 1) load_A(afr[aslot], 0, a_chunk, a_cob);
-            if constexpr (ky == 2) load_A(afr[aslot], 1, a_chunk, a_cob);
+          if constexpr (nb == NBA - 1) {
+            if constexpr (FOLD) {
+              if constexpr (ky < 2) load_A(afr[aslot], ky + 2, ch, cur_g.cob);
+              else load_A(afr[aslot], ky - 2, a_chunk, a_cob);
+            } else {
+              if constexpr (ky == 0) load_A(afr[aslot], 2, ch, cur_g.cob);
+              if constexpr (ky == 1) load_A(afr[aslot], 0, a_chunk, a_cob);
+              if constexpr (ky == 2) load_A(afr[aslot], 1, a_chunk, a_cob);
+            }
           }
-          if constexpr (ss < 3 * NBU - 1) __builtin_amdgcn_sched_group_barrier(0x100, 8, 0);
+          if constexpr (ss < NSS - 1) __builtin_amdgcn_sched_group_barrier(0x100, 8, 0);
 #pragma unroll
           for (int i = 0; i < 6; ++i) {
             __builtin_amdgcn_sched_group_barrier(0x008, 1, 0);
-            __builtin_amdgcn_sched_group_barrier(0x006, 4, 0);
-            if constexpr (nb == 1 || nb == 2) __builtin_amdgcn_sched_group_barrier(0x200, 1, 0);
+            __builtin_amdgcn_sched_group_barrier(0x006, (FOLD && ss == 6) ? 8 : 4, 0);
+            if constexpr (stores) __builtin_amdgcn_sched_group_barrier(0x200, 1, 0);
           }
           __builtin_amdgcn_sched_barrier(0);
         });
@@ -427,13 +448,14 @@
     float* const ms = lds + Y_S1;
     const int ecol = tid & 31, ecg = tid >> 5;
     const int co0 = cur_g.cob * Y_CO;
-    const float* const scale_p = reinterpret_cast<const float*>(wq + (VOL ? 36 : 12) * pos_stride);
+    const float* const scale_p = reinterpret_cast<const float*>(wq + (VOL ? 36 : FOLD ? 16 : 12) * pos_stride);
     const int oHW = POOL ? HW >> 2 : (VOL ? CS : HW), oW = POOL ? a.W >> 1 : a.W;
     const size_t tile_base = (((size_t)cur_g.b * a.Cout + co0) * oHW + (size_t)cur_g.z * HW + (size_t)(POOL ? cur_g.y0 >> 1 : cur_g.y0) * oW +
                               (POOL ? cur_g.x0 >> 1 : cur_g.x0)) * 4;
     const bool e_isb = pack && (ecol & 15) >= seam;
     const int e_pair = e_isb ? (ecol & 15) - seam : (ecol & 15);
-    unsigned eoff4 = 4u * (unsigned)(ecg * oHW + (POOL ? (ecol & 15) : (ecol >> 4) * oW + 2 * e_pair + (e_isb ? HW : 0)));
+    unsigned eoff4 = 4u * (unsigned)(ecg * oHW + (FOLD ? (ecol >> 4) * oW + (ecol & 15) : POOL ? (ecol & 15)
+                                                        : (ecol >> 4) * oW + 2 * e_pair + (e_isb ? HW : 0)));
     asm volatile("" : "+v"(eoff4));
     [[maybe_unused]] auto cmp_off = [&](int nb) -> unsigned {
       const int n = 32 * nb + ecol, row = n / 12, pr = n % 12;
@@ -442,11 +464,11 @@
     };
     auto boff = [&](int c, int nb, int k) -> unsigned {
       if constexpr (NBU == 3) return 4u * (unsigned)((((k >> 1) * 2 + c) * 32 + (k & 1) * 16) * oHW) + cmp_off(nb);
-      return 4u * (unsigned)((((k >> 1) * 2 + c) * 32 + (k & 1) * 16) * oHW + (POOL ? nb : 2 * nb) * oW) + eoff4;
+      return 4u * (unsigned)((((k >> 1) * 2 + c) * 32 + (k & 1) * 16) * oHW + (POOL && !FOLD ? nb : 2 * nb) * oW) + eoff4;
     };
     auto in_range = [&](int nb) {
       if constexpr (NBU == 3) return !(pack && (32 * nb + ecol) % 12 >= 6) || cur_g.z + 1 < a.D;
-      const bool row_ok = cur_g.y0 + 2 * nb + (ecol >> 4) < a.H;
+      const bool row_ok = FOLD ? cur_g.y0 + 4 * nb + 2 * (ecol >> 4) < a.H : cur_g.y0 + 2 * nb + (ecol >> 4) < a.H;
       if constexpr (VOL) {
         if (pack) return row_ok && (ecol & 15) < 2 * seam && (!e_isb || cur_g.z + 1 < a.D);
       }
@@ -464,8 +486,8 @@
     vecv resv[2][4];
     auto prefetch = [&](auto rc) {
       constexpr int rnd = decltype(rc)::value;
-      constexpr int c = rnd / NBU, nb = rnd % NBU, bf = rnd & 1;
-      const bool res_ok = has_res && in_range(nb) && (!POOL || (ecol >> 4) == 0);
+      constexpr int c = rnd / NBA, nb = rnd % NBA, bf = rnd & 1;
+      const bool res_ok = has_res && in_range(nb) && (!POOL || FOLD || (ecol >> 4) == 0);
 #pragma unroll
       for (int k = 0; k < 4; ++k) {
         const unsigned ob = res_ok ? boff(c, nb, k) : 0u;
@@ -492,9 +514,9 @@
 #else
 #define W1D_TE(k)
 #endif
-    static_for<2 * NBU>([&](auto rc) {
+    static_for<2 * NBA>([&](auto rc) {
       constexpr int rnd = decltype(rc)::value;
-      constexpr int c = rnd / NBU, nb = rnd % NBU, bf = rnd & 1;
+      constexpr int c = rnd / NBA, nb = rnd % NBA, bf = rnd & 1;
       float* const mw = ms + (rnd & 1) * Y_M;
 #pragma unroll
       for (int rr = 0; rr < 16; ++rr) {
@@ -505,8 +527,8 @@
       W1D_TE(0);
       __syncthreads();
       W1D_TE(1);
-      if constexpr (rnd < 2 * NBU - 1) prefetch(std::integral_constant<int, rnd + 1>{});
-      const bool inr = in_range(nb) && (!POOL || (ecol >> 4) == 0);
+      if constexpr (rnd < 2 * NBA - 1) prefetch(std::integral_constant<int, rnd + 1>{});
+      const bool inr = in_range(nb) && (!POOL || FOLD || (ecol >> 4) == 0);
 #pragma unroll
       for (int half = 0; half < 2; ++half) {
         float m[2][4], sc[2], bi[2];
@@ -524,9 +546,14 @@
         for (int kk = 0; kk < 2; ++kk) {
           const int k = half * 2 + kk;
           float yv[2];
-          yv[0] = __builtin_fmaf(m[kk][0] + m[kk][1] + m[kk][2], sc[kk], bi[kk]);
-          yv[1] = __builtin_fmaf(m[kk][1] - m[kk][2] - m[kk][3], sc[kk], bi[kk]);
-          if constexpr (POOL) {
+          if constexpr (FOLD) {
+            yv[0] = __builtin_fmaf(__builtin_fmaf(2.f, m[kk][1], m[kk][0]) - m[kk][3], 0.25f * sc[kk], bi[kk]);
+            yv[1] = 0.f;
+          } else {
+            yv[0] = __builtin_fmaf(m[kk][0] + m[kk][1] + m[kk][2], sc[kk], bi[kk]);
+            yv[1] = __builtin_fmaf(m[kk][1] - m[kk][2] - m[kk][3], sc[kk], bi[kk]);
+          }
+          if constexpr (POOL && !FOLD) {
             const float p0 = __shfl_xor(yv[0], 16, 64), p1 = __shfl_xor(yv[1], 16, 64);
             yv[0] = (((yv[0] + p0) + yv[1]) + p1) * 0.25f;
           }
@@ -586,7 +613,7 @@
         if constexpr (nb == 0) st_c0 = st_c1 = 0;
         st_c0 += NV * __popcll(bal & 0xffffffffull);
         st_c1 += NV * __popcll(bal >> 32);
-        if constexpr (nb == NBU - 1) {
+        if constexpr (nb == NBA - 1) {
           const float cnt = (float)(h ? st_c1 : st_c0);
           const int tb = (cur_g.y0 / Y_ROWS) * a.tiles_x + cur_g.x0 / (2 * Y_TX);
           const int n_tb = a.tiles_x * a.tiles_y;
@@ -673,7 +700,14 @@
 #define W1D_LAUNCH(O, S_, P_)                                                                                            \
   return a.coef ? ipdm_launch_lds(conv_wino1d_kernel<O, S_, P_, true>, grid, dim3(512), Y_LDS_BYTES, s, a, (int)nblk)   \
                 : ipdm_launch_lds(conv_wino1d_kernel<O, S_, P_, false>, grid, dim3(512), Y_LDS_BYTES, s, a, (int)nblk)
-  if (a.pool2) {
+#define W1D_LAUNCH_FOLD(O, S_) \
+  return ipdm_launch_lds(conv_wino1d_kernel<O, S_, true, false, false, 4, true>, grid, dim3(512), Y_LDS_BYTES, s, a, (int)nblk)
+  if (a.pool2 == 2) {
+    if (a.stats) { if (outs == 3) W1D_LAUNCH_FOLD(3, true); else W1D_LAUNCH_FOLD(1, true); }
+    else if (outs == 3) W1D_LAUNCH_FOLD(3, false);
+    else if (outs == 1) W1D_LAUNCH_FOLD(1, false);
+    else W1D_LAUNCH_FOLD(2, false);
+  } else if (a.pool2) {
     if (a.stats) { if (outs == 3) W1D_LAUNCH(3, true, true); else W1D_LAUNCH(1, true, true); }
     else if (outs == 3) W1D_LAUNCH(3, false, true);
     else if (outs == 1) W1D_LAUNCH(1, false, true);
@@ -683,16 +717,18 @@
   } else if (outs == 3) W1D_LAUNCH(3, false, false);
   else if (outs == 1) W1D_LAUNCH(1, false, false);
   else W1D_LAUNCH(2, false, false);
+#undef W1D_LAUNCH_FOLD
 #undef W1D_LAUNCH
 }
 
 int conv_wino1d_weights(const float* w, void* U, int Cout, int Cin, int npos, hipStream_t s) {
+  const bool fold = npos == 16;
   const int n_cc = (Cin + 15) / 16, n_ct = (Cout + 31) / 32;
   const int64_t total = (int64_t)npos * n_cc * n_ct * 512;
   float* inv_scale = reinterpret_cast<float*>(static_cast<char*>(U) + total * 2 * 2);
-  hipLaunchKernelGGL(wino1d_scale_kernel, dim3(n_ct * 32), dim3(256), 0, s, w, inv_scale, Cout, Cin, n_ct * 32, npos);
+  hipLaunchKernelGGL(wino1d_scale_kernel, dim3(n_ct * 32), dim3(256), 0, s, w, inv_scale, Cout, Cin, n_ct * 32, npos, fold);
   hipLaunchKernelGGL(wino1d_weight_kernel, dim3(ipdm_ew_grid(total, 256)), dim3(256), 0, s, w, (unsigned short*)U, inv_scale, Cout,
-                     Cin, n_cc, n_ct, npos);
+                     Cin, n_cc, n_ct, npos, fold);
   return ipdm_launch_status();
 }
 
@@ -708,6 +744,16 @@
 extern "C" int ipdm_conv_wino1d_pack_weight(const float* w, void* U, int Cout, int Cin, void* stream) {
   IPDM_REQUIRE(w && U && Cout > 0 && Cin > 0);
   return conv_wino1d_weights(w, U, Cout, Cin, 12, ipdm_stream(stream));
+}
+
+extern "C" int64_t ipdm_conv_wino1d_pool_weight_bytes(int Cout, int Cin) {
+  if (Cout <= 0 || Cin <= 0) return -1;
+  return (int64_t)16 * ((Cin + 15) / 16) * ((Cout + 31) / 32) * 2048 + (int64_t)((Cout + 31) / 32) * 32 * 4;
+}
+
+extern "C" int ipdm_conv_wino1d_pack_weight_pool(const float* w, void* U, int Cout, int Cin, void* stream) {
+  IPDM_REQUIRE(w && U && Cout > 0 && Cin > 0);
+  return conv_wino1d_weights(w, U, Cout, Cin, 16, ipdm_stream(stream));
 }
 
 extern "C" int ipdm_conv2d_wino1d_supported(int Cin, int Cout, int H, int W) {
@@ -723,8 +769,8 @@
   ConvArgs a = conv_launch_args(x, U, bias, residual, out, out_act, act_out, B, Cin, Cout, 1, H, W, 3, 1, 1, ext, conv_debug_stamps());
   a.coef = coef; a.act = coef ? act : IPDM_ACT_NONE;
   a.stats = stats;
-  a.pool2 = pool2 ? 1 : 0;
-  if (!wino1d_ok(a) || !wino_pairs_aligned(a)) return IPDM_EUNSUPPORTED;
+  a.pool2 = pool2 == 2 ? 2 : pool2 ? 1 : 0;
+  if (!wino1d_ok(a) || !wino_pairs_aligned(a) || (a.pool2 == 2 && coef)) return IPDM_EUNSUPPORTED;
   return conv_wino1d_launch(a, ipdm_stream(stream));
 }
 
diff --git a/inverseproblemwithdiffusionmodel_amd/ncsn/models/layers.py b/inverseproblemwithdiffusionmodel_amd/ncsn/models/layers.py
--- a/inverseproblemwithdiffusionmodel_amd/ncsn/models/layers.py
+++ b/inverseproblemwithdiffusionmodel_amd/ncsn/models/layers.py
@@ -68,6 +68,9 @@
 
     def packed_wino1d(self):
         return self._cached("wino1d", ops.conv_wino1d_weight)
+
+    def packed_wino1d_pool(self):
+        return self._cached("wino1d_pool", ops.conv_wino1d_pool_weight)
 
     def route(self, x, site="ncsn", coef=None, **call):
         return ops.conv_route(site, self.ndim, self.kernel_size, self.dilation, self.in_planes, self.out_planes, tuple(x.shape[2:]),
@@ -194,9 +197,11 @@
                                            act_out=act_out, pool2=True, want_stats=True,
                                            in_amax=getattr(coef, "_ipdm_amax_bound", None) if dyn else None,
                                            want_amax=dyn and feeds_conv, coef=coef, act=act)
-            return ops.conv2d_wino_bx3(inputs, c.packed_wino1d() if route == ops.ROUTE_WINO1D else c.packed_wino_bx3(), bias, residual,
-                                       act_out=act_out, pool2=True, want_stats=True,
-                                       in_amax=ops.in_amax_for(inputs), want_amax=dyn and feeds_conv)
+            fold = c.packed_wino1d_pool if route == ops.ROUTE_WINO1D and ops.W1D_POOLFOLD else None
+            with ops.offer_pool_form(fold):
+                return ops.conv2d_wino_bx3(inputs, c.packed_wino1d() if route == ops.ROUTE_WINO1D else c.packed_wino_bx3(), bias, residual,
+                                           act_out=act_out, pool2=True, want_stats=True,
+                                           in_amax=ops.in_amax_for(inputs), want_amax=dyn and feeds_conv)
         except _lib.IpdmUnsupported:
             return None
 
diff --git a/inverseproblemwithdiffusionmodel_amd/ops.py b/inverseproblemwithdiffusionmodel_amd/ops.py
--- a/inverseproblemwithdiffusionmodel_amd/ops.py
+++ b/inverseproblemwithdiffusionmodel_amd/ops.py
@@ -1,3 +1,4 @@
+import contextlib
 import ctypes
 import os
 
@@ -2227,6 +2228,16 @@
     return PackedBx3(blob, Cout, Cin, 12, "hx2")
 
 
+def conv_wino1d_pool_weight(w):
+    w = _gpu(w, torch.float32, "weight")
+    Cout, Cin = w.shape[:2]
+    if tuple(w.shape[2:]) != (3, 3):
+        raise ValueError(f"conv_wino1d_pool_weight: weight {tuple(w.shape)}")
+    blob = torch.empty(_lib.lib.ipdm_conv_wino1d_pool_weight_bytes(Cout, Cin), dtype=torch.uint8, device=w.device)
+    call("ipdm_conv_wino1d_pack_weight_pool", _ptr(w), _ptr(blob), Cout, Cin, _stream())
+    return PackedBx3(blob, Cout, Cin, 16, "w1dp")
+
+
 def conv_wino1d_weight3d(w):
     w = _gpu(w, torch.float32, "weight")
     Cout, Cin = w.shape[:2]
@@ -2270,6 +2281,18 @@
 WINO1D = os.environ.get("IPDM_WINO1D", "1") != "0"
 WINO1D_STATS = os.environ.get("IPDM_WINO1D_STATS", "1") != "0"
 WINO1D_FIN = os.environ.get("IPDM_WINO1D_FIN", "0") != "0"
+W1D_POOLFOLD = os.environ.get("IPDM_W1D_POOLFOLD", "1") != "0"
+_POOL_FORM_OFFER = None
+
+
+@contextlib.contextmanager
+def offer_pool_form(get):
+    global _POOL_FORM_OFFER
+    prev, _POOL_FORM_OFFER = _POOL_FORM_OFFER, get
+    try:
+        yield
+    finally:
+        _POOL_FORM_OFFER = prev
 
 
 def wino1d_pays(Cin, Cout, H, W, dilation=1):
@@ -2290,22 +2313,31 @@
                     in_amax=None, out_scale=1.0, want_amax=False, res_second=False, coef=None, act=ACT_NONE):
     x = _gpu(x, torch.float32, "x")
     B, Cin, H, W = x.shape
+    if _POOL_FORM_OFFER is not None and pool2 and U.kk == 12 and U.fmt == "hx2" and coef is None and act == ACT_NONE:
+        offered = _POOL_FORM_OFFER()
+        if (offered.fmt, offered.Cout, offered.Cin) != ("w1dp", U.Cout, U.Cin):
+            raise ValueError("conv2d_wino_bx3: the offered pool form does not match the weight blob")
+        U = offered
+    fold = U.fmt == "w1dp"
+    if fold and (not pool2 or U.kk != 16):
+        raise ValueError("conv2d_wino_bx3: the folded pool blob (conv_wino1d_pool_weight) serves pool2=True launches only")
+    fmt = "hx2" if fold else U.fmt
     amax_t = None
-    if U.fmt == "hx2" and in_amax is not None:
+    if fmt == "hx2" and in_amax is not None:
         if in_amax is True and coef is not None:
             raise ValueError("conv2d_wino_bx3: with a fused input the maxima are the coefficient kernel's bound, not max |x|")
         amax_t = absmax_per_image(x) if in_amax is True else in_amax
     bias_per_image = bias is not None and bias.dim() == 2
     if bias_per_image and (tuple(bias.shape) != (B, U.Cout) or bias.stride(1) != 1):
         raise ValueError(f"conv2d_wino_bx3: per-image bias {tuple(bias.shape)} != {(B, U.Cout)} (rows may be strided, not columns)")
-    one_d = U.kk == 12
+    one_d = U.kk == 12 or fold
     if U.kk not in (12, 16) or U.Cin != Cin:
         raise ValueError("conv2d_wino_bx3: weight blob does not match the input")
-    if one_d and (dilation != 1 or U.fmt != "hx2"):
+    if one_d and (dilation != 1 or fmt != "hx2"):
         raise ValueError("conv2d_wino_bx3: the 1-D Winograd blob serves undilated f16x2 launches only")
     if coef is not None or act != ACT_NONE:
-        if not one_d or coef is None or act != ACT_ELU:
-            raise ValueError("conv2d_wino_bx3: a fused input (coef + ACT_ELU) is the 1-D Winograd kernel's only")
+        if not one_d or fold or coef is None or act != ACT_ELU:
+            raise ValueError("conv2d_wino_bx3: a fused input (coef + ACT_ELU) is the 1-D Winograd kernel's only (12-position blob)")
         coef = _gpu(coef, torch.float32, "coef")
         if tuple(coef.shape) != (B, Cin, 3):
             raise ValueError(f"conv2d_wino_bx3: coef {tuple(coef.shape)} != {(B, Cin, 3)}")
@@ -2318,7 +2350,7 @@
     out, out_act, slot_o, slot_a = _conv_outputs(x, (B, Cout, oh, ow), raw, act_out, want_amax=want_amax)
     e0 = _trace_open()
     nb = wino_bx3_max_batch(Cin, H, W, dilation)
-    ksplit = 1 if one_d or pool2 or x.data_ptr() % 16 or (WBX3_CO32 and U.fmt == "hx2") else wino_bx3_splitk(Cin, Cout, H, W, dilation)
+    ksplit = 1 if one_d or pool2 or x.data_ptr() % 16 or (WBX3_CO32 and fmt == "hx2") else wino_bx3_splitk(Cin, Cout, H, W, dilation)
     part = None
     if ksplit == 1 and want_stats and raw and USE_STATS_EPILOGUE and x.data_ptr() % 16 == 0:
         P = (int(_lib.lib.ipdm_conv2d_wino1d_stats_partials(Cin, Cout, H, W)) if one_d else
@@ -2328,7 +2360,7 @@
     for n, cut in _chunks(B, nb):
         head = (_ptr(cut(x)), _ptr(U.blob), _ptr(cut(bias) if bias_per_image else bias))
         outs = (_ptr(cut(residual)), _ptr(cut(out)), _ptr(cut(out_act)), act_out, n, Cin, Cout, H, W)
-        ext = _conv_ext(U.fmt, cut(amax_t), cut(x), False, bias_per_image, out_scale, bias.stride(0) if bias_per_image else 0,
+        ext = _conv_ext(fmt, cut(amax_t), cut(x), False, bias_per_image, out_scale, bias.stride(0) if bias_per_image else 0,
                         cut(slot_o), cut(slot_a), res_second)
         if ksplit > 1:
             work = torch.empty((ksplit, n, Cout, H, W), dtype=torch.float32, device=x.device)
@@ -2336,7 +2368,7 @@
         elif one_d:
             stats = () if part is None else (_ptr(cut(part)),)
             call("ipdm_conv2d_wino1d_f32" if part is None else "ipdm_conv2d_wino1d_stats_f32", *head, _ptr(cut(coef)), act, *outs,
-                 int(bool(pool2)), *stats, ext, _stream())
+                 2 if fold else int(bool(pool2)), *stats, ext, _stream())
         else:
             args = head + outs + (dilation, int(bool(pool2)))
             if part is not None:
@@ -2348,9 +2380,11 @@
             call(f"ipdm_conv2d_wino_{U.fmt}_f32", *args, ext, _stream())
     if part is not None:
         out._ipdm_partials = (part, (out._version, out.data_ptr()))
-    form = dict(pool2=False, ksplit=ksplit) if ksplit > 1 else dict(pool2=bool(pool2), wino1d=one_d, stats=part is not None)
+    form = dict(pool2=False, ksplit=ksplit) if ksplit > 1 else dict(pool2=bool(pool2), wino1d=one_d and not fold, stats=part is not None)
+    if fold:
+        form["w1d_fold"] = True
     return _conv_done(e0, out, out_act, slot_o, slot_a, B=B, Cin=Cin, Cout=Cout, H=H, W=W, k=3, dil=dilation, wino=True, bx3=True,
-                      fmt=U.fmt, res=residual is not None, **form)
+                      fmt=fmt, res=residual is not None, **form)
 
 
 WBX3_CO32 = os.environ.get("IPDM_WBX3_CO32", "1") != "0"
```

New measurement: 0.1338 reconstructions/s, median of 6. 1.02x the previous value.
